# yyyyyxie/textflux

Hardware: AMD Instinct MI355X
Metric: images/sec (whole node), 1024x1024 30-step FLUX-Fill (higher is better)
Workload: dtype bf16

## Files before the change

### textflux_amd/csrc/attention.hip

```cpp
#include <atomic>
#include <type_traits>

#include "common.h"
#include "launch.h"

namespace tfx {

constexpr int KVBLK = 64, HD = 128;
#ifdef TFX_BENCH
constexpr int K_BYTES = KVBLK * HD * 2;
constexpr int ATT_LDS = 2 * 2 * K_BYTES;
constexpr int ATT_LDS2 = 2 * ATT_LDS;
constexpr int ATT_LDS_PP = 5 * K_BYTES;
#endif

typedef __attribute__((address_space(3))) s16x4 lds_s16x4;
__device__ unsigned long long* g_dbg_ptr = nullptr;

#define TFX_ATT_BARRIER()                                   \
  do {                                                      \
    __builtin_amdgcn_sched_barrier(0);                      \
    asm volatile("s_waitcnt lgkmcnt(0)" ::: "memory");      \
    __builtin_amdgcn_s_barrier();                           \
    __builtin_amdgcn_sched_barrier(0);                      \
// ... 391 lines not shown
  };
  for (int j = 0; j < nkv; j += 2) {
    tile(j, std::integral_constant<int, 0>{});
    if (j + 1 < nkv) tile(j + 1, std::integral_constant<int, 1>{});
  }

  const float inv = 1.0f / ol[0];
  if (qrow < N) {
    bf16_t* orow = Ob + (int64_t)qrow * ldo + 4 * hi;
#pragma unroll
    for (int db = 0; db < 4; ++db)
#pragma unroll
      for (int qd = 0; qd < 4; ++qd) {
        u32x2 w;
        w[0] = pack_bf2(o[db][qd * 4 + 0] * inv, o[db][qd * 4 + 1] * inv);
        w[1] = pack_bf2(o[db][qd * 4 + 2] * inv, o[db][qd * 4 + 3] * inv);
        *reinterpret_cast<u32x2*>(orow + db * 32 + qd * 8) = w;
      }
  }
}


template <bool TIMING>
__global__ __launch_bounds__(512, 2) void attn_pp_kernel(const bf16_t* Q, const bf16_t* __restrict__ Kp,
                                                         const bf16_t* __restrict__ Vp, bf16_t* O, int64_t ldq,
                                                         int64_t ldk, int64_t ldv, int64_t ldo, int64_t q_bs, int64_t k_bs,
                                                         int64_t v_bs, int64_t o_bs, int H, int N, int nqb,
                                                         float scale_log2e, unsigned long long* dbg) {
  extern __shared__ __attribute__((aligned(16))) char smem[];
  const int tid = threadIdx.x, lane = tid & 63;
  const int wave = __builtin_amdgcn_readfirstlane(tid >> 6);
  const int g = wave >> 2;
  unsigned long long t_pa = 0, t_b1 = 0, t_pb = 0, t_b2 = 0, tmark = 0;
#define ATM() do { if (TIMING) tmark = __builtin_readcyclecounter(); } while (0)
#define ATA(x) do { if (TIMING) { unsigned long long n_ = __builtin_readcyclecounter(); x += n_ - tmark; tmark = n_; } } while (0)
  const int hi = lane >> 5, l31 = lane & 31;
  int bid = blockIdx.x;
  {
    const int nwg = gridDim.x, q = nwg >> 3, r = nwg & 7, xcd = bid & 7, k = bid >> 3;
    bid = (xcd < r ? xcd * (q + 1) : r * (q + 1) + (xcd - r) * q) + k;
  }
  const int qb = bid % nqb;
  bid /= nqb;
  const int h = bid % H;
  const int b = bid / H;
  const bf16_t* Qb = Q + b * q_bs + h * HD;
  const bf16_t* Kb = Kp + b * k_bs + h * HD;
  const bf16_t* Vb = Vp + b * v_bs + h * HD;
  bf16_t* Ob = O + b * o_bs + h * HD;

  const int qrow = qb * 256 + wave * 32 + l31;
  const int qrow_c = qrow < N ? qrow : N - 1;
  bf16x8 qf[8];
#pragma unroll
  for (int s = 0; s < 8; ++s) qf[s] = *reinterpret_cast<const bf16x8*>(Qb + (int64_t)qrow_c * ldq + s * 16 + hi * 8);

  const int nkv = (N + KVBLK - 1) / KVBLK;
  char* kbuf = smem;
  char* vbuf = smem + 2 * K_BYTES;
  u32x4 kreg[2], vreg[2];
  auto opaque_tid = [&]() { int t_ = tid; asm volatile("" : "+v"(t_)); return t_; };
  auto load_rows = [&](const bf16_t* base, int64_t ld, int t, u32x4* reg) {
    const int te = opaque_tid();
#pragma unroll
    for (int i = 0; i < 2; ++i) {
      const int c = te + i * 512;
      int key = t * KVBLK + (c >> 4);
      if (key > N - 1) key = N - 1;
      reg[i] = *reinterpret_cast<const u32x4*>(base + (int64_t)key * ld + (c & 15) * 8);
    }
  };
  auto write_k = [&](int t) {
    char* kd = kbuf + (t & 1) * K_BYTES;
    const int te = opaque_tid();
#pragma unroll
    for (int i = 0; i < 2; ++i) {
      const int c = te + i * 512, key = c >> 4, ch = c & 15;
      *reinterpret_cast<u32x4*>(kd + key * 256 + ((ch ^ (key & 15)) << 4)) = kreg[i];
    }
  };
  auto write_v = [&](int t) {
    char* vd = vbuf + (t % 3) * K_BYTES;
    const int te = opaque_tid();
#pragma unroll
    for (int i = 0; i < 2; ++i) {
      const int c = te + i * 512, key = c >> 4, ch = c & 15;
      *reinterpret_cast<u32x4*>(vd + key * 256 + ((((ch >> 2) ^ (key & 3)) << 6) | ((ch & 3) << 4))) = vreg[i];
    }
  };

  uint32_t koff[8];
#pragma unroll
  for (int s = 0; s < 8; ++s) koff[s] = l31 * 256 + (((2 * s + hi) ^ (lane & 15)) << 4);
  const int vi = lane & 15;
  const uint32_t vrow = (4 * hi + (vi >> 2)) * 256 + 32 * ((lane >> 4) & 1) + (vi & 3) * 8;
  uint32_t voff[4];
#pragma unroll
  for (int db = 0; db < 4; ++db) voff[db] = vrow + ((db ^ ((vi >> 2) & 3)) << 6);

  f32x16 o[4], s0, s1;
#pragma unroll
  for (int db = 0; db < 4; ++db)
#pragma unroll
    for (int r = 0; r < 16; ++r) o[db][r] = 0.f;
  float m_run = -INFINITY, l_run = 0.f;
  bf16x8 pf[4];
  typedef __attribute__((ext_vector_type(8))) short s16x8;

  auto ldvf = [&](const char* vt, int i) -> bf16x8 {
    const char* va = vt + voff[i & 3] + (i >> 2) * 16 * 256;
    const s16x4 lo = __builtin_amdgcn_ds_read_tr16_b64_v4i16((lds_s16x4*)(va));
    const s16x4 hi4 = __builtin_amdgcn_ds_read_tr16_b64_v4i16((lds_s16x4*)(va + 8 * 256));
    return __builtin_bit_cast(bf16x8, (s16x8)__builtin_shufflevector(lo, hi4, 0, 1, 2, 3, 4, 5, 6, 7));
  };

  load_rows(Kb, ldk, 0, kreg);
  load_rows(Vb, ldv, 0, vreg);
  write_k(0);
  write_v(0);
  if (nkv > 1) {
    load_rows(Kb, ldk, 1, kreg);
    load_rows(Vb, ldv, 1, vreg);
    write_k(1);
    write_v(1);
    if (nkv > 2) {
      load_rows(Kb, ldk, 2, kreg);
      load_rows(Vb, ldv, 2, vreg);
    }
  }
  __syncthreads();
  {
#pragma unroll
    for (int r = 0; r < 16; ++r) { s0[r] = 0.f; s1[r] = 0.f; }
#pragma unroll
    for (int s = 0; s < 8; ++s) {
      const bf16x8 k0 = *reinterpret_cast<const bf16x8*>(kbuf + koff[s]);
      const bf16x8 k1 = *reinterpret_cast<const bf16x8*>(kbuf + koff[s] + 32 * 256);
      s0 = __builtin_amdgcn_mfma_f32_32x32x16_bf16(k0, qf[s], s0, 0, 0, 0);
      s1 = __builtin_amdgcn_mfma_f32_32x32x16_bf16(k1, qf[s], s1, 0, 0, 0);
    }
  }
  TFX_ATT_BARRIER();
  if (g == 1) TFX_ATT_BARRIER();

  int vslot = 0;
  for (int u = 0; u < nkv; ++u) {
    ATM();
    bf16x8 vf[16];
    {
      const char* vt = vbuf + vslot * K_BYTES;
#pragma unroll
      for (int i = 0; i < 16; ++i) vf[i] = ldvf(vt, i);
    }
    if (u == nkv - 1 && (N & (KVBLK - 1))) {
      const int kbase = u * KVBLK + 4 * hi;
#pragma unroll
      for (int r = 0; r < 16; ++r) {
        const int key = kbase + (r & 3) + 8 * (r >> 2);
        if (key >= N) s0[r] = -INFINITY;
        if (key + 32 >= N) s1[r] = -INFINITY;
      }
    }
    {
      float mx = s0[0];
#pragma unroll
      for (int r = 1; r < 16; ++r) mx = fmaxf(mx, s0[r]);
#pragma unroll
      for (int r = 0; r < 16; ++r) mx = fmaxf(mx, s1[r]);
      mx = fmaxf(mx, __shfl_xor(mx, 32, 64));
      const float m_new = fmaxf(m_run, mx);
      const float mc = m_new * scale_log2e;
      const float alpha = __builtin_amdgcn_exp2f(m_run * scale_log2e - mc);
      m_run = m_new;
      float psum = 0.f;
#pragma unroll
      for (int r = 0; r < 16; ++r) {
        s0[r] = __builtin_amdgcn_exp2f(s0[r] * scale_log2e - mc);
        s1[r] = __builtin_amdgcn_exp2f(s1[r] * scale_log2e - mc);
        psum += s0[r] + s1[r];
      }
      l_run = l_run * alpha + psum;
#pragma unroll
      for (int e = 0; e < 8; ++e) {
        pf[0][e] = (__bf16)s0[e];
        pf[1][e] = (__bf16)s0[8 + e];
        pf[2][e] = (__bf16)s1[e];
        pf[3][e] = (__bf16)s1[8 + e];
      }
      if (!__all(alpha == 1.0f)) {
#pragma unroll
        for (int db = 0; db < 4; ++db)
#pragma unroll
          for (int r = 0; r < 16; ++r) o[db][r] *= alpha;
      }
    }
    ATA(t_pa);
    TFX_ATT_BARRIER();
    ATA(t_b1);
    const char* kt = kbuf + ((u + 1) & 1) * K_BYTES;
    bf16x8 kf[8][2];
    uint32_t kofs[8];
    {
      int le = lane;
      asm volatile("" : "+v"(le));
#pragma unroll
      for (int s = 0; s < 8; ++s) kofs[s] = (le & 31) * 256 + (((2 * s + (le >> 5)) ^ (le & 15)) << 4);
    }
    __builtin_amdgcn_s_setprio(1);
#pragma unroll
    for (int ks = 0; ks < 4; ++ks) {
#pragma unroll
      for (int db = 0; db < 4; ++db) o[db] = __builtin_amdgcn_mfma_f32_32x32x16_bf16(vf[ks * 4 + db], pf[ks], o[db], 0, 0, 0);
      __builtin_amdgcn_sched_barrier(0);
#pragma unroll
      for (int s = 2 * ks; s < 2 * ks + 2; ++s) {
        kf[s][0] = *reinterpret_cast<const bf16x8*>(kt + kofs[s]);
        kf[s][1] = *reinterpret_cast<const bf16x8*>(kt + kofs[s] + 32 * 256);
      }
      __builtin_amdgcn_sched_barrier(0);
    }
#pragma unroll
    for (int db = 0; db < 4; ++db) asm volatile("" : "+v"(o[db]));
#pragma unroll
    for (int r = 0; r < 16; ++r) { s0[r] = 0.f; s1[r] = 0.f; }
#pragma unroll
    for (int s = 0; s < 8; ++s) {
      s0 = __builtin_amdgcn_mfma_f32_32x32x16_bf16(kf[s][0], qf[s], s0, 0, 0, 0);
      s1 = __builtin_amdgcn_mfma_f32_32x32x16_bf16(kf[s][1], qf[s], s1, 0, 0, 0);
    }
    asm volatile("" : "+v"(s0), "+v"(s1));
    __builtin_amdgcn_sched_barrier(0);
    __builtin_amdgcn_s_setprio(0);
    if (u + 2 < nkv) {
      write_k(u + 2);
      write_v(u + 2);
      if (u + 3 < nkv) {
        load_rows(Kb, ldk, u + 3, kreg);
        load_rows(Vb, ldv, u + 3, vreg);
      }
    }
    vslot = vslot == 2 ? 0 : vslot + 1;
    ATA(t_pb);
    TFX_ATT_BARRIER();
    ATA(t_b2);
  }
  if (g == 0) TFX_ATT_BARRIER();
  if (TIMING && lane == 0 && dbg) {
    unsigned long long* d = dbg + ((size_t)blockIdx.x * 8 + wave) * 4;
    d[0] = t_pa; d[1] = t_b1; d[2] = t_pb; d[3] = t_b2;
  }
#undef ATM
#undef ATA

  const float l_tot = l_run + __shfl_xor(l_run, 32, 64);
  const float inv = 1.0f / l_tot;
  if (qrow < N) {
    bf16_t* orow = Ob + (int64_t)qrow * ldo + 4 * hi;
#pragma unroll
    for (int db = 0; db < 4; ++db)
#pragma unroll
      for (int qd = 0; qd < 4; ++qd) {
        u32x2 w;
        w[0] = pack_bf2(o[db][qd * 4 + 0] * inv, o[db][qd * 4 + 1] * inv);
        w[1] = pack_bf2(o[db][qd * 4 + 2] * inv, o[db][qd * 4 + 3] * inv);
        *reinterpret_cast<u32x2*>(orow + db * 32 + qd * 8) = w;
      }
  }
}

#endif

static int g_attn_bound = 1;
void set_attention_use_bound(int v) { g_attn_bound = v; }
static std::atomic<int64_t> g_attn_mode_count[9];
void attention_note_streamk() { ++g_attn_mode_count[8]; }
int attention_mode_counts(int64_t* counts, int n, int reset) {
  n = n < 0 ? 0 : n > 9 ? 9 : n;
  for (int i = 0; i < n; ++i) counts[i] = g_attn_mode_count[i].load(std::memory_order_relaxed);
  if (reset) for (int i = 0; i < 9; ++i) g_attn_mode_count[i].store(0, std::memory_order_relaxed);
  return n;
}
static bool attn_bound_admissible(float score_bound, int N) {
  return score_bound > 0.f && score_bound * 1.4426950408889634f + log2f((float)N) + 24.0f <= 126.0f;
}
static int g_attn_waves = 30;
static unsigned long long* g_attn_dbg = nullptr;
void set_attention_debug(void* p) {
  g_attn_dbg = (unsigned long long*)p;
  (void)hipMemcpyToSymbol(HIP_SYMBOL(g_dbg_ptr), &p, sizeof(p));
}
static int g_attn_abl = 0;
void set_attention_ablation(int a) { g_attn_abl = a; }
void set_attention_waves(int nw) {
  if (nw == 0) { g_attn_waves = 30; return; }
  g_attn_waves = (nw == 4 || nw == 8 || nw == 9 || nw == 10 || nw == 12 || nw == 20 || (nw >= 30 && nw <= 34) || nw == 40) ? nw : 16;
}

int joint_attention(const AttnArgs& a, hipStream_t st) {
  if (a.B <= 0 || a.H <= 0 || a.N <= 0) return 0;
  if ((a.ldq | a.ldk | a.ldv | a.q_bstride | a.k_bstride | a.v_bstride) % 8 || (a.ldo | a.o_bstride) % 4)
    return fail("attention: strides must be multiples of 8 elements (q,k,v) / 4 (o)");
  if (((uintptr_t)a.q | (uintptr_t)a.k | (uintptr_t)a.v) % 16 || (uintptr_t)a.o % 8)
    return fail("attention: q/k/v must be 16-byte aligned, o 8-byte aligned");
#ifdef TFX_BENCH
  if (g_attn_waves == 20 && !g_attn_abl) {
    const bool prof = prof_on(st);
    if (prof) prof_begin(1, 4.0 * a.B * a.H * (double)a.N * a.N * HD, st);
    const int rc = joint_attention_hp(a, st);
    if (prof) prof_end(1, st);
    ++g_attn_mode_count[5];
    return rc ? rc : check_launch("joint_attention");
  }
#endif
  const uint64_t w4_rows = (uint64_t)((a.N + 63) / 64 + 3) * 64;
  const bool w4_ok = (a.ldo | a.o_bstride) % 8 == 0 && w4_rows * (uint64_t)a.ldk * 2 + 256 < (1ull << 32) &&
                     w4_rows * (uint64_t)a.ldv * 2 + 256 < (1ull << 32);
#ifdef TFX_BENCH
  if (g_attn_waves == 40 && w4_ok) {
    const bool prof = prof_on(st);
    if (prof) prof_begin(1, 4.0 * a.B * a.H * (double)a.N * a.N * HD, st);
    const int rc = joint_attention_w16(a, st);
    if (prof) prof_end(1, st);
    ++g_attn_mode_count[6];
    return rc ? rc : check_launch("joint_attention");
  }
#endif
#ifdef TFX_BENCH
  if (((g_attn_waves >= 30 && g_attn_waves <= 34) || g_attn_waves == 40) && w4_ok) {
#else
  if ((g_attn_waves == 30 || g_attn_waves == 34) && w4_ok) {
#endif
    const bool prof = prof_on(st);
    if (prof) prof_begin(1, 4.0 * a.B * a.H * (double)a.N * a.N * HD, st);
    const bool bounded = attn_bound_admissible(a.score_bound, a.N);
#ifdef TFX_BENCH
    const int mode = g_attn_waves == 34 ? (bounded ? 4 : 3) : g_attn_waves == 30 ? (bounded && g_attn_bound ? 4 : 0)
                   : g_attn_waves >= 31 && g_attn_waves <= 33 ? g_attn_waves - 30 : 0;
#else
    const int mode = bounded && (g_attn_bound || g_attn_waves == 34) ? 4 : 0;
#endif
    const int rc = joint_attention_w4(a, st, mode);
    if (prof) prof_end(1, st);
    ++g_attn_mode_count[mode];
    return rc ? rc : check_launch("joint_attention");
  }
#ifndef TFX_BENCH
  if (g_attn_waves != 30 && g_attn_waves != 34)
    return fail("attention: kernel variant %d is a bench-only schedule (libtextflux_hip_bench.so, `make bench`)", g_attn_waves);
  return fail("attention: output rows must be 16-byte aligned (ldo and o_bstride multiples of 8 elements) and one head's K / V rows "
              "addressable in 32 bits; got ldo %lld, o_bstride %lld, N %d, ldk %lld, ldv %lld", (long long)a.ldo, (long long)a.o_bstride,
              a.N, (long long)a.ldk, (long long)a.ldv);
#else
  const int NW = (g_attn_waves == 16 || g_attn_waves == 9 || g_attn_waves == 10 || g_attn_waves >= 30) ? 8 : g_attn_waves == 12 ? 4 : g_attn_waves;
  const int qblk = NW * 32;
  static bool attr_set = false;
  if (!attr_set) {
    const void* fns[] = {(const void*)attn_kernel<8>, (const void*)attn_mx_kernel<8>,
#ifdef TFX_BENCH
                         (const void*)attn_kernel<4>, (const void*)attn_mx_kernel<4>,
#endif
    };
    for (const void* fn : fns) {
      hipFuncAttributes fa;
      (void)hipFuncGetAttributes(&fa, fn);
      (void)hipGetLastError();
      if (hipFuncSetAttribute(fn, hipFuncAttributeMaxDynamicSharedMemorySize, ATT_LDS) != hipSuccess)
        return fail("attention: cannot raise dynamic LDS limit");
    }
#ifdef TFX_BENCH
    hipFuncAttributes fa;
    (void)hipFuncGetAttributes(&fa, (const void*)attn_kernel<8, 0, 2>);
    (void)hipFuncGetAttributes(&fa, (const void*)attn_pp_kernel<false>);
    (void)hipGetLastError();
    if (hipFuncSetAttribute((const void*)attn_kernel<8, 0, 2>, hipFuncAttributeMaxDynamicSharedMemorySize, ATT_LDS2) != hipSuccess ||
        hipFuncSetAttribute((const void*)attn_pp_kernel<false>, hipFuncAttributeMaxDynamicSharedMemorySize, ATT_LDS_PP) != hipSuccess)
      return fail("attention: cannot raise dynamic LDS limit (bench variants)");
#endif
    attr_set = true;
  }
  const int nqb = (a.N + qblk - 1) / qblk;
  const unsigned grid = (unsigned)(a.B * a.H * nqb);
  const bool prof = prof_on(st);
  if (prof) prof_begin(1, 4.0 * a.B * a.H * (double)a.N * a.N * HD, st);
  const float sl2 = a.scale * 1.4426950408889634f;
#define ATT_ARGS (const bf16_t*)a.q, (const bf16_t*)a.k, (const bf16_t*)a.v, (bf16_t*)a.o, a.ldq, a.ldk, a.ldv, a.ldo, a.q_bstride, \
                 a.k_bstride, a.v_bstride, a.o_bstride, a.H, a.N, nqb, sl2
#ifdef TFX_BENCH
  if (g_attn_abl) {
    (void)hipFuncSetAttribute((const void*)attn_kernel<8, 1>, hipFuncAttributeMaxDynamicSharedMemorySize, ATT_LDS);
    (void)hipFuncSetAttribute((const void*)attn_kernel<8, 2>, hipFuncAttributeMaxDynamicSharedMemorySize, ATT_LDS);
    (void)hipFuncSetAttribute((const void*)attn_kernel<8, 4>, hipFuncAttributeMaxDynamicSharedMemorySize, ATT_LDS);
    (void)hipFuncSetAttribute((const void*)attn_kernel<8, 8>, hipFuncAttributeMaxDynamicSharedMemorySize, ATT_LDS);
    (void)hipFuncSetAttribute((const void*)attn_kernel<8, 15>, hipFuncAttributeMaxDynamicSharedMemorySize, ATT_LDS);
    (void)hipFuncSetAttribute((const void*)attn_kernel<8, 16>, hipFuncAttributeMaxDynamicSharedMemorySize, ATT_LDS);
    switch (g_attn_abl) {
      case 1: attn_kernel<8, 1><<<grid, 512, ATT_LDS, st>>>(ATT_ARGS); break;
      case 2: attn_kernel<8, 2><<<grid, 512, ATT_LDS, st>>>(ATT_ARGS); break;
      case 4: attn_kernel<8, 4><<<grid, 512, ATT_LDS, st>>>(ATT_ARGS); break;
      case 8: attn_kernel<8, 8><<<grid, 512, ATT_LDS, st>>>(ATT_ARGS); break;
      case 16: attn_kernel<8, 16><<<grid, 512, ATT_LDS, st>>>(ATT_ARGS); break;
      default: attn_kernel<8, 15><<<grid, 512, ATT_LDS, st>>>(ATT_ARGS); break;
    }
  } else if (g_attn_waves == 16) {
    if (g_attn_dbg) {
      (void)hipFuncSetAttribute((const void*)attn_pp_kernel<true>, hipFuncAttributeMaxDynamicSharedMemorySize, ATT_LDS_PP);
      attn_pp_kernel<true><<<grid, 512, ATT_LDS_PP, st>>>(ATT_ARGS, g_attn_dbg);
    } else {
      attn_pp_kernel<false><<<grid, 512, ATT_LDS_PP, st>>>(ATT_ARGS, nullptr);
    }
  } else if (g_attn_waves == 12) {
    attn_mx_kernel<4><<<grid, 256, ATT_LDS, st>>>(ATT_ARGS);
  } else if (g_attn_waves == 9) {
    attn_kernel<8, 0, 2><<<grid, 512, ATT_LDS2, st>>>(ATT_ARGS);
  } else if (g_attn_waves == 4) {
    attn_kernel<4><<<grid, 256, ATT_LDS, st>>>(ATT_ARGS);
  } else
#endif
  if (g_attn_waves == 10 || (g_attn_waves >= 30 && g_attn_waves <= 34))
    attn_mx_kernel<8><<<grid, 512, ATT_LDS, st>>>(ATT_ARGS);
  else
    attn_kernel<8><<<grid, 512, ATT_LDS, st>>>(ATT_ARGS);
#undef ATT_ARGS
  if (prof) prof_end(1, st);
  ++g_attn_mode_count[7];
  return check_launch("joint_attention");
#endif
}

}
```

### textflux_amd/csrc/attention_w4.hip

```cpp
#include <mutex>
#include <type_traits>

#include "common.h"
#include "launch.h"

namespace tfx {

namespace {
constexpr int W4_KV = 64, W4_HD = 128;
constexpr int W4_VT = W4_KV * 256;
constexpr int W4_KROW = 272;
constexpr int W4_KT = W4_KV * W4_KROW;
constexpr int W4_NBUF = 3;
constexpr int W4_KBASE = W4_NBUF * W4_VT;
constexpr int W4_PROW = 132;
__device__ __forceinline__ int w4_part_off(int r, int col) {
  return ((((r >> 5) * 4 + (col >> 5)) * 4 + ((col >> 3) & 3)) * 64 + ((col >> 2) & 1) * 32 + (r & 31)) * 4;
}
constexpr int W4_PART_LM = 256 * 128;
constexpr float W4_THR = 4.0f;
constexpr float W4_BIG = 64.0f;
typedef __attribute__((address_space(3))) s16x4 lds_s16x4;
typedef __attribute__((ext_vector_type(8))) short s16x8;
typedef __attribute__((ext_vector_type(2))) __bf16 bf2_t;
template <int V>
using IC = std::integral_constant<int, V>;
}

constexpr int ATT_LDS_W4 = W4_NBUF * (W4_VT + W4_KT);

#define W4_GAP() __builtin_amdgcn_sched_barrier(0)
#ifndef W4_ABL
#define W4_ABL 0
#endif
#define W4_DRAIN_MFMA()                                                                                                 \
  asm volatile("s_nop 15\n\ts_nop 15\n\ts_nop 15\n\ts_nop 15\n\ts_nop 15\n\ts_nop 15\n\ts_nop 15\n\ts_nop 15\n\t"      \
               "s_nop 15\n\ts_nop 15\n\ts_nop 15\n\ts_nop 15\n\ts_nop 15\n\ts_nop 15\n\ts_nop 15\n\ts_nop 15\n\t"      \
               "s_nop 15\n\ts_nop 15\n\ts_nop 15\n\ts_nop 15\n\ts_nop 15\n\ts_nop 15\n\ts_nop 15\n\ts_nop 15" ::: "memory")

#ifndef W4_NO_TOUCH
#define W4_TOUCH(acc)                                                                  \
  do {                                                                                 \
    const int t_ = __builtin_amdgcn_readfirstlane(__float_as_int((acc)[0]));           \
    asm volatile("" ::"s"(t_));                                                        \
  } while (0)
#else
#define W4_TOUCH(acc) do { } while (0)
#endif

__device__ __forceinline__ void w4_mfma_s0(f32x16& d, const bf16x8& k, const bf16x8& q) {
  f32x16 z;
#pragma unroll
  for (int r = 0; r < 16; ++r) z[r] = 0.f;
  d = __builtin_amdgcn_mfma_f32_32x32x16_bf16(k, q, z, 0, 0, 0);
}
__device__ __forceinline__ void w4_mfma_s(f32x16& d, const bf16x8& k, const bf16x8& q) {
  d = __builtin_amdgcn_mfma_f32_32x32x16_bf16(k, q, d, 0, 0, 0);
}
__device__ __forceinline__ void w4_mfma_o(f32x16& d, const bf16x8& v, const u32x4& p) {
  d = __builtin_amdgcn_mfma_f32_32x32x16_bf16(v, __builtin_bit_cast(bf16x8, p), d, 0, 0, 0);
}
__device__ __forceinline__ void w4_mfma_l(f32x16& d, const bf16x8& ones, const u32x4& p) {
  d = __builtin_amdgcn_mfma_f32_32x32x16_bf16(ones, __builtin_bit_cast(bf16x8, p), d, 0, 0, 0);
}
__device__ __forceinline__ float w4_max7(float a, float b, float c, float d, float e, float f, float g) {
  float r;
  asm("v_max3_f32 %0, %1, %2, %3\n\tv_max3_f32 %0, %0, %4, %5\n\tv_max3_f32 %0, %0, %6, %7"
      : "=&v"(r) : "v"(a), "v"(b), "v"(c), "v"(d), "v"(e), "v"(f), "v"(g));
  return r;
}
__device__ __forceinline__ float w4_max4(float a, float b, float c, float d) {
  float r;
  asm("v_max3_f32 %0, %1, %2, %3\n\tv_max_f32 %0, %0, %4" : "=&v"(r) : "v"(a), "v"(b), "v"(c), "v"(d));
  return r;
}
__device__ __forceinline__ float w4_max(float a, float b) {
  float r;
  asm("v_max_f32 %0, %1, %2" : "=v"(r) : "v"(a), "v"(b));
  return r;
}
__device__ __forceinline__ void w4_dot2c(float& l, uint32_t p) {
  asm volatile("v_dot2c_f32_bf16 %0, 0x3f803f80, %1" : "+v"(l) : "v"(p));
}
__device__ __forceinline__ uint32_t w4_cvt_pk(float lo, float hi) {
  uint32_t r;
  asm volatile("v_cvt_pk_bf16_f32 %0, %1, %2" : "=v"(r) : "v"(lo), "v"(hi));
  return r;
}
#ifdef TFX_BENCH
__device__ unsigned long long* g_w4_timers = nullptr;
#define W4_STAMP(i) do { if (wave == 0) w4_stamp[i] = __builtin_amdgcn_s_memtime(); } while (0)
#else
#define W4_STAMP(i) ((void)0)
#endif
constexpr int W4_SK_MIN = 4;
__host__ __device__ __forceinline__ int w4_sk_bound(int c, int group, int share, int nkv, int total) {
  if (c >= group) return total;
  int p = c * share;
  if (p >= total) return total;
  const int r = p % nkv;
  if (r < W4_SK_MIN) p -= r;
  else if (r > nkv - W4_SK_MIN) p += nkv - r;
  return p < total ? p : total;
}

template <int MODE>
__global__ __launch_bounds__(256, 1) void attn_w4_kernel(const bf16_t* Q, const bf16_t* __restrict__ Kp,
                                                         const bf16_t* __restrict__ Vp, bf16_t* O, int64_t ldq, int64_t ldk,
                                                         int64_t ldv, int64_t ldo, int64_t q_bs, int64_t k_bs, int64_t v_bs,
                                                         int64_t o_bs, int H, int N, int nqb, float scale_log2e, int nfull,
                                                         int nparts, int nsplit, int xsplit, float* part, int T_items, int sk_group,
                                                         int sk_share) {
  extern __shared__ __attribute__((aligned(16))) char smem[];
  constexpr bool LV = MODE == 1 || MODE == 2, LZ = MODE >= 2, NOREF = MODE == 4, FT = LV || NOREF;
  const int tid = threadIdx.x, lane = tid & 63;
  const int wave = __builtin_amdgcn_readfirstlane(tid >> 6);
  const int hi = lane >> 5, l31 = lane & 31;
  int bid = blockIdx.x;
  int kpart = -1, ptile = 0, qblk, h, b;
  int item = 0, item_step = 0, item_end = 0;
  int sk_lo = 0, sk_hi = 0, sk_base = 0, sk_slot0 = 0, sk_u = 0, sk_nunits = 0, sk_nwhole = 0, sk_full = 0, sk_cu = 0, sk_tfirst = 0;
  const int nkv_all = (N + W4_KV - 1) / W4_KV;
  auto sk_unit = [&](int u, int& it, int& ts, int& te) __attribute__((always_inline)) {
    if (u < sk_nwhole) {
      it = sk_base + sk_cu + u * sk_group; ts = 0; te = nkv_all;
    } else {
      const int ti = sk_tfirst + (u - sk_nwhole);
      it = sk_base + sk_full + ti; ts = max(sk_lo - ti * nkv_all, 0); te = min(sk_hi - ti * nkv_all, nkv_all);
    }
  };
  int ts = 0, te = nkv_all;
  if (sk_share > 0) {
    const int L = (bid & 7) * (gridDim.x >> 3) + (bid >> 3);
    const int sample = L / sk_group;
    sk_cu = L - sample * sk_group;
    if (sample >= nfull) return;
    sk_full = (T_items / sk_group) * sk_group;
    sk_nwhole = sk_full / sk_group;
    const int total = (T_items - sk_full) * nkv_all;
    sk_lo = w4_sk_bound(sk_cu, sk_group, sk_share, nkv_all, total);
    sk_hi = w4_sk_bound(sk_cu + 1, sk_group, sk_share, nkv_all, total);
    sk_tfirst = sk_lo / nkv_all;
    sk_nunits = sk_nwhole + (sk_hi > sk_lo ? (sk_hi - 1) / nkv_all - sk_tfirst + 1 : 0);
    if (sk_nunits == 0) return;
    sk_base = sample * T_items;
    sk_slot0 = 2 * L;
    sk_unit(0, item, ts, te);
    qblk = item % nqb;
    h = (item / nqb) % H;
    b = item / (nqb * H);
  } else if (T_items > 0) {
    const int nwg = gridDim.x, q = T_items >> 3, r = T_items & 7, xcd = bid & 7, slot = bid >> 3;
    const int xs = xcd < r ? xcd * (q + 1) : r * (q + 1) + (xcd - r) * q, xc = q + (xcd < r ? 1 : 0);
    if (slot >= xc) return;
    item = xs + slot;
    item_step = nwg >> 3;
    item_end = xs + xc;
    qblk = item % nqb;
    h = (item / nqb) % H;
    b = item / (nqb * H);
  } else if (nsplit > 1) {
    const int fpad = (nfull + 7) & ~7, pf = H * nqb - xsplit;
    int pair;
    if (bid < fpad) {
      const int q = nfull >> 3, r = nfull & 7, xcd = bid & 7, k = bid >> 3;
      if (k >= q + (xcd < r ? 1 : 0)) return;
      const int fid = (xcd < r ? xcd * (q + 1) : r * (q + 1) + (xcd - r) * q) + k;
      b = fid / pf;
      pair = fid % pf;
    } else {
      const int pi = bid - fpad;
      if (pi >= nparts) return;
      kpart = pi % nsplit;
      ptile = pi / nsplit;
      b = ptile / xsplit;
      pair = pf + ptile % xsplit;
    }
    h = pair / nqb;
    qblk = pair % nqb;
  } else {
    const int nwg = gridDim.x, q = nwg >> 3, r = nwg & 7, xcd = bid & 7, k = bid >> 3;
    bid = (xcd < r ? xcd * (q + 1) : r * (q + 1) + (xcd - r) * q) + k;
    qblk = bid % nqb;
    bid /= nqb;
    h = bid % H;
    b = bid / H;
  }
  bf16x8 qn[2][8];
  bool have_pref = false;
  u32x4 kreg[4], vreg[4];
#ifdef TFX_BENCH
  unsigned long long w4_stamp[4] = {0, 0, 0, 0}, w4_sum[4] = {0, 0, 0, 0};
#endif
  for (;;) {
  W4_STAMP(0);
  bool has_next = item + item_step < item_end;
  int item2 = item + item_step, ts2 = 0;
  if (sk_share > 0) {
    int te2;
    has_next = sk_u + 1 < sk_nunits;
    if (has_next) sk_unit(sk_u + 1, item2, ts2, te2);
  }
  const int qblk2 = item2 % nqb, h2 = (item2 / nqb) % H, b2 = item2 / (nqb * H);
  const bf16_t* Qb = Q + b * q_bs + h * W4_HD;
  const bf16_t* Kb = Kp + b * k_bs + h * W4_HD;
  const bf16_t* Vb = Vp + b * v_bs + h * W4_HD;
  bf16_t* Ob = O + b * o_bs + h * W4_HD;
  int Nk = N;
  if (kpart >= 0) {
    const int nkv_all = (N + W4_KV - 1) / W4_KV;
    const int t0 = kpart * nkv_all / nsplit, t1 = (kpart + 1) * nkv_all / nsplit;
    Nk = min(N, t1 * W4_KV) - t0 * W4_KV;
    Kb += (int64_t)t0 * W4_KV * ldk;
    Vb += (int64_t)t0 * W4_KV * ldv;
  }
  int pslot = -1;
  if (sk_share > 0) {
    if (ts > 0) pslot = sk_slot0;
    else if (te < nkv_all) pslot = sk_slot0 + 1;
    Nk = min(N, te * W4_KV) - ts * W4_KV;
    Kb += (int64_t)ts * W4_KV * ldk;
    Vb += (int64_t)ts * W4_KV * ldv;
  }

  int qrow[2];
  bf16x8 qf[2][8];
#pragma unroll
  for (int qb = 0; qb < 2; ++qb) {
    qrow[qb] = qblk * 256 + wave * 64 + qb * 32 + l31;
    const int rc = qrow[qb] < N ? qrow[qb] : N - 1;
    if (have_pref) {
#pragma unroll
      for (int s = 0; s < 8; ++s) qf[qb][s] = qn[qb][s];
    } else {
#pragma unroll
      for (int s = 0; s < 8; ++s) qf[qb][s] = *reinterpret_cast<const bf16x8*>(Qb + (int64_t)rc * ldq + s * 16 + hi * 8);
    }
  }
  auto load_qn = [&]() __attribute__((always_inline)) {
    const bf16_t* Qb2 = Q + b2 * q_bs + h2 * W4_HD;
#pragma unroll
    for (int qb = 0; qb < 2; ++qb) {
      const int r2 = qblk2 * 256 + wave * 64 + qb * 32 + l31;
      const int rc = r2 < N ? r2 : N - 1;
#pragma unroll
      for (int s = 0; s < 8; ++s) qn[qb][s] = *reinterpret_cast<const bf16x8*>(Qb2 + (int64_t)rc * ldq + s * 16 + hi * 8);
    }
  };
  __builtin_amdgcn_sched_barrier(0);
  auto convert_q = [&]() __attribute__((always_inline)) {
    if constexpr (W4_ABL & 1024) {
      float cc = scale_log2e, sn = scale_log2e * 0.5f;
      uint32_t wlo = 0x3f80u, whi = 0x3f800000u;
      asm volatile("" : "+v"(cc), "+v"(sn), "+v"(wlo), "+v"(whi));
#pragma unroll
      for (int qb = 0; qb < 2; ++qb) {
        float ss = 0.f;
#pragma unroll
        for (int s = 0; s < 8; ++s) {
          const u32x4 pk = __builtin_bit_cast(u32x4, qf[qb][s]);
#pragma unroll
          for (int i = 0; i < 4; ++i) {
            const uint32_t pi = pk[i];
            ss = __builtin_amdgcn_fdot2_f32_bf16(__builtin_bit_cast(bf2_t, pi), __builtin_bit_cast(bf2_t, pi), ss, false);
          }
        }
        const auto sw = __builtin_amdgcn_permlane32_swap(__float_as_uint(ss), __float_as_uint(ss), false, false);
        const float rinv = rsqrtf((__uint_as_float(sw[0]) + __uint_as_float(sw[1])) * (1.0f / 128.0f) + 1e-6f);
#pragma unroll
        for (int s = 0; s < 8; ++s) {
          u32x4 pk = __builtin_bit_cast(u32x4, qf[qb][s]);
#pragma unroll
          for (int i = 0; i < 4; ++i) {
            const uint32_t a = pack_bf2(__uint_as_float(pk[i] << 16) * rinv, __uint_as_float(pk[i] & 0xffff0000u) * rinv);
            float y0, y1;
            y0 = __builtin_amdgcn_fdot2_f32_bf16(__builtin_bit_cast(bf2_t, a), __builtin_bit_cast(bf2_t, wlo), 0.0f, false);
            y1 = __builtin_amdgcn_fdot2_f32_bf16(__builtin_bit_cast(bf2_t, a), __builtin_bit_cast(bf2_t, whi), 0.0f, false);
            const uint32_t yp = pack_bf2(y0, y1);
            y0 = __uint_as_float(yp << 16);
            y1 = __uint_as_float(yp & 0xffff0000u);
            pk[i] = pack_bf2(y0 * cc + (-y1) * sn, y1 * cc + y0 * sn);
          }
          qf[qb][s] = __builtin_bit_cast(bf16x8, pk);
        }
      }
    }
#pragma unroll
    for (int qb = 0; qb < 2; ++qb)
#pragma unroll
      for (int s = 0; s < 8; ++s) {
#pragma unroll
        for (int e = 0; e < 8; ++e) qf[qb][s][e] = (__bf16)((float)qf[qb][s][e] * scale_log2e);
        asm volatile("" : "+a"(qf[qb][s]));
      }
  };

  const int nkv = (Nk + W4_KV - 1) / W4_KV;
  const int ldk2 = (int)ldk * 2, ldv2 = (int)ldv * 2;
  const auto rsK = __builtin_amdgcn_make_buffer_rsrc((void*)Kb, 0, (int)((uint32_t)(Nk - 1) * (uint32_t)ldk2 + 256u), 0x00020000);
  const auto rsV = __builtin_amdgcn_make_buffer_rsrc((void*)Vb, 0, (int)((uint32_t)(Nk - 1) * (uint32_t)ldv2 + 256u), 0x00020000);
  const auto rsK2 = __builtin_amdgcn_make_buffer_rsrc((void*)(Kp + b2 * k_bs + h2 * W4_HD + (int64_t)ts2 * W4_KV * ldk), 0,
                                                      (int)((uint32_t)(N - 1 - ts2 * W4_KV) * (uint32_t)ldk2 + 256u), 0x00020000);
  const auto rsV2 = __builtin_amdgcn_make_buffer_rsrc((void*)(Vp + b2 * v_bs + h2 * W4_HD + (int64_t)ts2 * W4_KV * ldv), 0,
                                                      (int)((uint32_t)(N - 1 - ts2 * W4_KV) * (uint32_t)ldv2 + 256u), 0x00020000);
  auto rsKs = rsK, rsVs = rsV;
  auto load_piece = [&](int j, int ko, int vo, auto Ic, bool k_side) __attribute__((always_inline)) {
    constexpr int i = decltype(Ic)::value;
    if (W4_ABL & 32) j = 0;
    if constexpr (W4_ABL & 256) {
      typedef __attribute__((address_space(3))) void lds_void_;
      __builtin_amdgcn_raw_ptr_buffer_load_lds(k_side ? rsKs : rsVs, (lds_void_*)(smem + ATT_LDS_W4 + (tid >> 6) * 1024), 16, k_side ? ko : vo,
                                               (j * W4_KV + 16 * i) * (k_side ? ldk2 : ldv2), 0, 0);
      return;
    }
    if (k_side)
      kreg[i] = __builtin_bit_cast(u32x4, __builtin_amdgcn_raw_buffer_load_b128(rsKs, ko, (j * W4_KV + 16 * i) * ldk2, 0));
    else
      vreg[i] = __builtin_bit_cast(u32x4, __builtin_amdgcn_raw_buffer_load_b128(rsVs, vo, (j * W4_KV + 16 * i) * ldv2, 0));
  };
  auto stage_offsets = [&](int& ko, int& vo) __attribute__((always_inline)) {
    int te = tid;
    asm volatile("" : "+v"(te));
    ko = (int)__umul24(te >> 4, ldk2) + (te & 15) * 16;
    vo = (int)__umul24(te >> 4, ldv2) + (te & 15) * 16;
  };
  auto load_tile = [&](int j) __attribute__((always_inline)) {
    int ko, vo;
    stage_offsets(ko, vo);
    load_piece(j, ko, vo, IC<0>{}, true); load_piece(j, ko, vo, IC<0>{}, false); load_piece(j, ko, vo, IC<1>{}, true); load_piece(j, ko, vo, IC<1>{}, false);
    load_piece(j, ko, vo, IC<2>{}, true); load_piece(j, ko, vo, IC<2>{}, false); load_piece(j, ko, vo, IC<3>{}, true); load_piece(j, ko, vo, IC<3>{}, false);
  };
  auto write_piece = [&](int buf, auto Ic, bool k_side) __attribute__((always_inline)) {
    constexpr int i = decltype(Ic)::value;
    const int kr = tid >> 4, ch = tid & 15;
    if (k_side)
      *reinterpret_cast<u32x4*>(smem + W4_KBASE + buf * W4_KT + kr * W4_KROW + ch * 16 + i * 16 * W4_KROW) = kreg[i];
    else
      *reinterpret_cast<u32x4*>(smem + buf * W4_VT + kr * 256 + ((((ch >> 2) ^ (kr & 3)) << 6) | ((ch & 3) << 4)) + i * 16 * 256) = vreg[i];
  };
  auto write_tile = [&](int buf) __attribute__((always_inline)) {
    write_piece(buf, IC<0>{}, true); write_piece(buf, IC<0>{}, false); write_piece(buf, IC<1>{}, true); write_piece(buf, IC<1>{}, false);
    write_piece(buf, IC<2>{}, true); write_piece(buf, IC<2>{}, false); write_piece(buf, IC<3>{}, true); write_piece(buf, IC<3>{}, false);
  };
  const char* rK = smem + W4_KBASE + l31 * W4_KROW + hi * 16;
  const int vi = lane & 15;
  const char* rV[4];
#pragma unroll
  for (int db = 0; db < 4; ++db)
    rV[db] = smem + (4 * hi + (vi >> 2)) * 256 + 32 * ((lane >> 4) & 1) + (vi & 3) * 8 + ((db ^ ((vi >> 2) & 3)) << 6);
  auto kread = [&](int koff, int s) __attribute__((always_inline)) -> bf16x8 {
    return *reinterpret_cast<const bf16x8*>(rK + koff + s * 32);
  };
  auto vread = [&](int voff, int ks, int db) __attribute__((always_inline)) -> bf16x8 {
    const char* va = rV[db] + voff + ks * 16 * 256;
    if constexpr (W4_ABL & 512) return *reinterpret_cast<const bf16x8*>(rK + voff + ks * 16 * 256 + db * 64);
    const s16x4 lo = __builtin_amdgcn_ds_read_tr16_b64_v4i16((lds_s16x4*)(va));
    const s16x4 hi4 = __builtin_amdgcn_ds_read_tr16_b64_v4i16((lds_s16x4*)(va + 8 * 256));
    return __builtin_bit_cast(bf16x8, (s16x8)__builtin_shufflevector(lo, hi4, 0, 1, 2, 3, 4, 5, 6, 7));
  };

  f32x16 o[2][4], ol[2], sc[2];
#pragma unroll
  for (int qb = 0; qb < 2; ++qb)
#pragma unroll
    for (int r = 0; r < 16; ++r) {
      ol[qb][r] = 0.f;
#pragma unroll
      for (int db = 0; db < 4; ++db) o[qb][db][r] = 0.f;
    }
  bf16x8 kone, vone, qm[2], kf[8], vf[2][4];
  u32x4 pf[2][2];
#pragma unroll
  for (int e = 0; e < 8; ++e) {
    kone[e] = (__bf16)0.f;
    vone[e] = (__bf16)1.0f;
    qm[0][e] = qm[1][e] = (__bf16)0.f;
  }
  if (hi == 0) kone[0] = (__bf16)1.0f;
  asm volatile("" : "+a"(kone), "+a"(vone));
  float m_ref[2] = {0.f, 0.f};
  float lsum[2] = {0.f, 0.f};
  bool any_ref = false;

#ifdef W4_DEBUG_CLEAR_LDS
  for (int i = tid * 16; i < ATT_LDS_W4; i += 256 * 16) *reinterpret_cast<u32x4*>(smem + i) = u32x4{0, 0, 0, 0};
  __syncthreads();
#endif
  if (!have_pref) load_tile(0);
  u32x4 k1[4], v1[4];
  {
    int ko, vo;
    stage_offsets(ko, vo);
#pragma unroll
    for (int i = 0; i < 4; ++i) {
      k1[i] = __builtin_bit_cast(u32x4, __builtin_amdgcn_raw_buffer_load_b128(rsK, ko, (W4_KV + 16 * i) * ldk2, 0));
      v1[i] = __builtin_bit_cast(u32x4, __builtin_amdgcn_raw_buffer_load_b128(rsV, vo, (W4_KV + 16 * i) * ldv2, 0));
    }
  }
  __builtin_amdgcn_sched_barrier(0);
  convert_q();
  __builtin_amdgcn_sched_barrier(0);
  write_tile(0);
  load_tile(2);
  {
    const int kr = tid >> 4, ch = tid & 15;
#pragma unroll
    for (int i = 0; i < 4; ++i) {
      *reinterpret_cast<u32x4*>(smem + W4_KBASE + W4_KT + kr * W4_KROW + ch * 16 + i * 16 * W4_KROW) = k1[i];
      *reinterpret_cast<u32x4*>(smem + W4_VT + kr * 256 + ((((ch >> 2) ^ (kr & 3)) << 6) | ((ch & 3) << 4)) + i * 16 * 256) = v1[i];
    }
  }
  __syncthreads();
#pragma unroll
  for (int s = 0; s < 8; ++s) kf[s] = kread(0, s);
  W4_GAP();
  if constexpr (LZ) {
    w4_mfma_s0(sc[0], kf[0], qf[0][0]);
#pragma unroll
    for (int s = 1; s < 8; ++s) w4_mfma_s(sc[0], kf[s], qf[0][s]);
  } else {
    w4_mfma_s0(sc[0], kone, qm[0]);
#pragma unroll
    for (int s = 0; s < 8; ++s) w4_mfma_s(sc[0], kf[s], qf[0][s]);
  }
#ifdef W4_KEEP_DRAINS
  W4_DRAIN_MFMA();
#endif
  W4_GAP();

  auto step = [&](auto QBc, auto PVc, auto FIRSTc, auto KNc, auto VNc, auto STGc, int jst, bool rag, int kb_abs) __attribute__((always_inline)) {
    constexpr int QB = decltype(QBc)::value, OQ = 1 - QB;
    constexpr bool EVEN = QB == 0, PV = decltype(PVc)::value != 0, FIRST = decltype(FIRSTc)::value != 0;
    constexpr int KN = decltype(KNc)::value, VN = decltype(VNc)::value, STG = decltype(STGc)::value;
    f32x16& cur = sc[QB];
    f32x16& nxt = sc[OQ];
    if (__builtin_expect_with_probability(rag, 0, 1.0)) {
      int kbase = kb_abs + 4 * hi;
      asm volatile("" : "+v"(kbase));
#pragma unroll
      for (int r = 0; r < 16; ++r)
        if (kbase + (r & 3) + 8 * (r >> 2) >= Nk) cur[r] = -INFINITY;
    }
    auto S = [&](auto Ic) __attribute__((always_inline)) {
      constexpr int i = decltype(Ic)::value;
      if constexpr (i == 0) {
        w4_mfma_s0(nxt, kone, qm[OQ]);
      } else if constexpr (i == 1 && LZ) {
        w4_mfma_s0(nxt, kf[0], qf[OQ][0]);
        if constexpr (!NOREF) {
          if (__builtin_expect_with_probability(any_ref, 0, 1.0)) w4_mfma_s(nxt, kone, qm[OQ]);
        }
      } else {
        w4_mfma_s(nxt, kf[i - 1], qf[OQ][i - 1]);
        if constexpr (EVEN && i >= 2 && !(W4_ABL & 2)) kf[i - 2] = kread(KN, i - 2);
      }
    };
    auto PL = [&](auto Ic) __attribute__((always_inline)) {
      constexpr int i = decltype(Ic)::value, ks = i / 4, db = i % 4;
      if constexpr (PV) w4_mfma_o(o[OQ][db], vf[ks][db], pf[OQ][ks]);
      if constexpr (EVEN && i >= 1 && !(W4_ABL & 2)) vf[(i - 1) / 4][(i - 1) % 4] = vread(VN, (i - 1) / 4, (i - 1) % 4);
    };
    auto RL = [&]() __attribute__((always_inline)) {
      if constexpr (EVEN && !(W4_ABL & 2)) {
        vf[1][3] = vread(VN, 1, 3);
        kf[7] = kread(KN, 7);
      }
    };
    auto DL = [&](auto Ic) __attribute__((always_inline)) {
      constexpr int c = decltype(Ic)::value;
      if constexpr (PV && !(W4_ABL & 1)) w4_dot2c(lsum[OQ], pf[OQ][c >> 2][c & 3]);
    };
    auto P = [&](auto Ic) __attribute__((always_inline)) {
      constexpr int i = decltype(Ic)::value, ks = i / 5, db = i % 5;
      if constexpr (PV) {
        if constexpr (db == 4) {
          w4_mfma_l(ol[OQ], vone, pf[OQ][ks]);
        } else {
          w4_mfma_o(o[OQ][db], vf[ks][db], pf[OQ][ks]);
        }
      }
      if constexpr (EVEN && i >= 1 && (i - 1) % 5 < 4 && !(W4_ABL & 2)) vf[(i - 1) / 5][(i - 1) % 5] = vread(VN, (i - 1) / 5, (i - 1) % 5);
      if constexpr (EVEN && i == 9 && !(W4_ABL & 2)) kf[7] = kread(KN, 7);
    };
    auto F = [&](auto Ic) __attribute__((always_inline)) {
      constexpr int k = decltype(Ic)::value;
      if constexpr (W4_ABL & 1) return;
      constexpr bool is_c = FT ? (k >= 22 || (k >= 3 && k <= 18 && k % 3 == 0)) : ((k == 23) || (k >= 3 && k < 22 && k % 3 == 0));
      if constexpr (is_c) {
        constexpr int c = FT ? (k >= 22 ? k - 16 : k / 3 - 1) : (k == 23 ? 7 : k / 3 - 1);
        pf[QB][c >> 2][c & 3] = w4_cvt_pk(cur[2 * c], cur[2 * c + 1]);
      } else {
        constexpr int e = FT ? (k < 3 ? k : k >= 19 ? k - 6 : k - (k / 3))
                             : (k < 3 ? k : k == 22 ? 15 : k - (k / 3));
        cur[e] = __builtin_amdgcn_exp2f(cur[e]);
      }
    };
    int stg_ko = 0, stg_vo = 0;
    if constexpr ((STG & 3) == 1 && !(W4_ABL & 4)) stage_offsets(stg_ko, stg_vo);
    auto G = [&](auto Ic) __attribute__((always_inline)) {
      constexpr int n = decltype(Ic)::value;
      if constexpr ((STG & 3) == 1 && !(W4_ABL & 4)) {
        constexpr bool is_w = n == 0 || n == 1 || (n < 15 && (n & 1));
        constexpr int g = n < 2 ? n : is_w ? (n + 1) / 2 : n == 15 ? 7 : n / 2 - 1;
        if constexpr (is_w) { if constexpr (!(W4_ABL & 64)) write_piece(STG >> 2, IC<g / 2>{}, (g & 1) == 0); }
        else { if constexpr (!(W4_ABL & 128)) load_piece(jst, stg_ko, stg_vo, IC<g / 2>{}, (g & 1) == 0); }
      }
    };
    float mx = 0.f;
    auto MX = [&](auto Ic) __attribute__((always_inline)) {
      constexpr int i = decltype(Ic)::value;
      if constexpr (W4_ABL & 8) return;
      if constexpr (i == 0) mx = w4_max7(cur[0], cur[1], cur[2], cur[3], cur[4], cur[5], cur[6]);
      if constexpr (i == 1) mx = w4_max7(mx, cur[7], cur[8], cur[9], cur[10], cur[11], cur[12]);
      if constexpr (i == 2) mx = w4_max4(mx, cur[13], cur[14], cur[15]);
      if constexpr (i == 3) {
        const auto sw = __builtin_amdgcn_permlane32_swap(__float_as_uint(mx), __float_as_uint(mx), false, false);
        mx = w4_max(__uint_as_float(sw[0]), __uint_as_float(sw[1]));
      }
    };
    auto MOVE = [&]() __attribute__((always_inline)) {
      bool take;
      if constexpr (LZ) take = !(W4_ABL & 8) && !__all(FIRST ? fabsf(mx) <= W4_BIG : mx <= W4_BIG);
      else take = FIRST || (!(W4_ABL & 8) && !__all(mx <= W4_THR));
      if (__builtin_expect_with_probability(take, FIRST && !LZ, 1.0)) {
        float m_new;
        if constexpr (LZ) {
          const bool mv = FIRST ? fabsf(mx) > W4_BIG : mx > W4_BIG;
          m_new = mv ? round_bf(m_ref[QB] + mx) : m_ref[QB];
        } else {
          m_new = round_bf(m_ref[QB] + (FIRST ? mx : fmaxf(mx, 0.f)));
        }
        const float d = m_new - m_ref[QB];
        m_ref[QB] = m_new;
        qm[QB][0] = (__bf16)(hi == 0 ? -m_new : 0.f);
        if constexpr (LZ) any_ref = __any(m_ref[0] != 0.f || m_ref[1] != 0.f);
#pragma unroll
        for (int r = 0; r < 16; ++r) cur[r] -= d;
        if constexpr (!FIRST) {
          const float f = __builtin_amdgcn_exp2f(-d);
          if constexpr (LV) lsum[QB] *= f;
#pragma unroll
          for (int r = 0; r < 16; ++r) {
            if constexpr (!LV) ol[QB][r] *= f;
#pragma unroll
            for (int db = 0; db < 4; ++db) o[QB][db][r] *= f;
          }
        }
      }
    };
    if constexpr (MODE == 0) {
    S(IC<0>{});
    W4_TOUCH(cur);
    MX(IC<0>{});
    W4_GAP();
    S(IC<1>{});
    MX(IC<1>{});
    W4_GAP();
    P(IC<0>{});
    MX(IC<2>{});
    W4_GAP();
    S(IC<2>{});
    MX(IC<3>{});
    W4_GAP();
    P(IC<1>{});
    W4_GAP();
    MOVE();
    W4_GAP();
    S(IC<3>{}); F(IC<0>{}); F(IC<1>{}); G(IC<0>{});
    W4_GAP();
    P(IC<2>{}); F(IC<2>{}); F(IC<3>{}); G(IC<1>{});
    W4_GAP();
    S(IC<4>{}); F(IC<4>{}); F(IC<5>{}); G(IC<2>{});
    W4_GAP();
    P(IC<3>{}); F(IC<6>{}); F(IC<7>{}); G(IC<3>{});
    W4_GAP();
    S(IC<5>{}); F(IC<8>{}); F(IC<9>{}); G(IC<4>{});
    W4_GAP();
    P(IC<4>{}); F(IC<10>{}); F(IC<11>{}); G(IC<5>{});
    W4_GAP();
    S(IC<6>{}); F(IC<12>{}); F(IC<13>{}); G(IC<6>{});
    W4_GAP();
    P(IC<5>{}); F(IC<14>{}); F(IC<15>{}); G(IC<7>{});
    W4_GAP();
    S(IC<7>{}); F(IC<16>{}); F(IC<17>{}); G(IC<8>{});
    W4_GAP();
    P(IC<6>{}); F(IC<18>{}); F(IC<19>{}); G(IC<9>{});
    W4_GAP();
    S(IC<8>{}); F(IC<20>{}); F(IC<21>{}); G(IC<10>{});
#ifdef W4_HAZARD_SELFTEST
    { const float t_ = w4_max(nxt[0], nxt[1]); asm volatile("" ::"v"(t_)); }
#endif
    W4_GAP();
    P(IC<7>{}); F(IC<22>{}); G(IC<11>{});
    W4_GAP();
    P(IC<8>{}); G(IC<12>{}); G(IC<13>{});
    W4_GAP();
    P(IC<9>{}); G(IC<14>{}); G(IC<15>{});
    W4_GAP();
    F(IC<23>{});
    W4_GAP();
    } else if constexpr (MODE == 1) {
    S(IC<0>{}); W4_TOUCH(cur); MX(IC<0>{}); G(IC<0>{});
    W4_GAP();
    S(IC<1>{}); MX(IC<1>{}); DL(IC<0>{}); G(IC<1>{});
    W4_GAP();
    PL(IC<0>{}); MX(IC<2>{}); DL(IC<1>{}); DL(IC<2>{}); G(IC<2>{});
    W4_GAP();
    S(IC<2>{}); MX(IC<3>{}); DL(IC<3>{}); DL(IC<4>{}); G(IC<3>{});
    W4_GAP();
    PL(IC<1>{}); DL(IC<5>{}); DL(IC<6>{}); DL(IC<7>{}); G(IC<4>{});
    W4_GAP();
    MOVE();
    W4_GAP();
    S(IC<3>{}); F(IC<0>{}); F(IC<1>{}); G(IC<5>{});
    W4_GAP();
    PL(IC<2>{}); F(IC<2>{}); F(IC<3>{}); G(IC<6>{});
    W4_GAP();
    S(IC<4>{}); F(IC<4>{}); F(IC<5>{}); G(IC<7>{});
    W4_GAP();
    PL(IC<3>{}); F(IC<6>{}); F(IC<7>{}); G(IC<8>{});
    W4_GAP();
    S(IC<5>{}); F(IC<8>{}); F(IC<9>{}); G(IC<9>{});
    W4_GAP();
    PL(IC<4>{}); F(IC<10>{}); F(IC<11>{}); G(IC<10>{});
    W4_GAP();
    S(IC<6>{}); F(IC<12>{}); F(IC<13>{}); G(IC<11>{});
    W4_GAP();
    PL(IC<5>{}); F(IC<14>{}); F(IC<15>{}); G(IC<12>{});
    W4_GAP();
    S(IC<7>{}); F(IC<16>{}); F(IC<17>{}); G(IC<13>{});
    W4_GAP();
    PL(IC<6>{}); F(IC<18>{}); F(IC<19>{}); G(IC<14>{});
    W4_GAP();
    S(IC<8>{}); F(IC<20>{}); F(IC<21>{}); G(IC<15>{});
#ifdef W4_HAZARD_SELFTEST
    { const float t_ = w4_max(nxt[0], nxt[1]); asm volatile("" ::"v"(t_)); }
#endif
    W4_GAP();
    PL(IC<7>{}); F(IC<22>{}); RL(); F(IC<23>{});
    W4_GAP();
    } else if constexpr (MODE == 3) {
    S(IC<1>{}); W4_TOUCH(cur); MX(IC<0>{});
    W4_GAP();
    P(IC<0>{}); MX(IC<1>{});
    W4_GAP();
    S(IC<2>{}); MX(IC<2>{});
    W4_GAP();
    P(IC<1>{}); MX(IC<3>{});
    W4_GAP();
    MOVE();
    W4_GAP();
    S(IC<3>{}); F(IC<0>{}); F(IC<1>{}); G(IC<0>{});
    W4_GAP();
    P(IC<2>{}); F(IC<2>{}); F(IC<3>{}); G(IC<1>{});
    W4_GAP();
    S(IC<4>{}); F(IC<4>{}); F(IC<5>{}); G(IC<2>{});
    W4_GAP();
    P(IC<3>{}); F(IC<6>{}); F(IC<7>{}); G(IC<3>{});
    W4_GAP();
    S(IC<5>{}); F(IC<8>{}); F(IC<9>{}); G(IC<4>{});
    W4_GAP();
    P(IC<4>{}); F(IC<10>{}); F(IC<11>{}); G(IC<5>{});
    W4_GAP();
    S(IC<6>{}); F(IC<12>{}); F(IC<13>{}); G(IC<6>{});
    W4_GAP();
    P(IC<5>{}); F(IC<14>{}); F(IC<15>{}); G(IC<7>{});
    W4_GAP();
    S(IC<7>{}); F(IC<16>{}); F(IC<17>{}); G(IC<8>{});
    W4_GAP();
    P(IC<6>{}); F(IC<18>{}); F(IC<19>{}); G(IC<9>{});
    W4_GAP();
    S(IC<8>{}); F(IC<20>{}); F(IC<21>{}); G(IC<10>{});
#ifdef W4_HAZARD_SELFTEST
    { const float t_ = w4_max(nxt[0], nxt[1]); asm volatile("" ::"v"(t_)); }
#endif
    W4_GAP();
    P(IC<7>{}); F(IC<22>{}); G(IC<11>{});
    W4_GAP();
    P(IC<8>{}); G(IC<12>{}); G(IC<13>{});
    W4_GAP();
    P(IC<9>{}); G(IC<14>{}); G(IC<15>{});
    W4_GAP();
    F(IC<23>{});
    W4_GAP();
    } else if constexpr (MODE == 4) {
    auto E = [&](auto Ic) __attribute__((always_inline)) {
      constexpr int e = decltype(Ic)::value;
      if constexpr (!(W4_ABL & 1)) cur[e] = __builtin_amdgcn_exp2f(cur[e]);
    };
    auto C2 = [&](auto Ic) __attribute__((always_inline)) {
      constexpr int c = decltype(Ic)::value;
      if constexpr (!(W4_ABL & 1)) pf[QB][c >> 2][c & 3] = w4_cvt_pk(cur[2 * c], cur[2 * c + 1]);
    };
    S(IC<1>{}); W4_TOUCH(cur); E(IC<0>{}); E(IC<1>{}); G(IC<0>{});
    W4_GAP();
    P(IC<0>{}); E(IC<2>{}); G(IC<1>{});
    W4_GAP();
    S(IC<2>{}); E(IC<3>{}); G(IC<2>{});
    W4_GAP();
    P(IC<1>{}); C2(IC<0>{}); E(IC<4>{}); G(IC<3>{});
    W4_GAP();
    S(IC<3>{}); E(IC<5>{}); G(IC<4>{});
    W4_GAP();
    P(IC<2>{}); C2(IC<1>{}); E(IC<6>{}); G(IC<5>{});
    W4_GAP();
    S(IC<4>{}); E(IC<7>{}); G(IC<6>{});
    W4_GAP();
    P(IC<3>{}); C2(IC<2>{}); E(IC<8>{}); G(IC<7>{});
    W4_GAP();
    S(IC<5>{}); E(IC<9>{}); G(IC<8>{});
    W4_GAP();
    P(IC<4>{}); C2(IC<3>{}); E(IC<10>{}); G(IC<9>{});
    W4_GAP();
    S(IC<6>{}); E(IC<11>{}); G(IC<10>{});
    W4_GAP();
    P(IC<5>{}); C2(IC<4>{}); E(IC<12>{}); G(IC<11>{});
    W4_GAP();
    S(IC<7>{}); E(IC<13>{}); G(IC<12>{});
    W4_GAP();
    P(IC<6>{}); C2(IC<5>{}); E(IC<14>{}); G(IC<13>{});
    W4_GAP();
    S(IC<8>{}); E(IC<15>{}); G(IC<14>{});
#ifdef W4_HAZARD_SELFTEST
    { const float t_ = w4_max(nxt[0], nxt[1]); asm volatile("" ::"v"(t_)); }
#endif
    W4_GAP();
    P(IC<7>{}); C2(IC<6>{}); G(IC<15>{});
    W4_GAP();
    P(IC<8>{});
    W4_GAP();
    P(IC<9>{}); C2(IC<7>{});
    W4_GAP();
    } else {
    S(IC<1>{}); W4_TOUCH(cur); MX(IC<0>{}); G(IC<0>{});
    W4_GAP();
    PL(IC<0>{}); MX(IC<1>{}); DL(IC<0>{}); G(IC<1>{});
    W4_GAP();
    S(IC<2>{}); MX(IC<2>{}); DL(IC<1>{}); DL(IC<2>{}); G(IC<2>{});
    W4_GAP();
    PL(IC<1>{}); MX(IC<3>{}); DL(IC<3>{}); DL(IC<4>{}); G(IC<3>{});
    W4_GAP();
    S(IC<3>{}); DL(IC<5>{}); DL(IC<6>{}); DL(IC<7>{}); G(IC<4>{});
    W4_GAP();
    MOVE();
    W4_GAP();
    PL(IC<2>{}); F(IC<0>{}); F(IC<1>{}); G(IC<5>{});
    W4_GAP();
    S(IC<4>{}); F(IC<2>{}); F(IC<3>{}); G(IC<6>{});
    W4_GAP();
    PL(IC<3>{}); F(IC<4>{}); F(IC<5>{}); G(IC<7>{});
    W4_GAP();
    S(IC<5>{}); F(IC<6>{}); F(IC<7>{}); G(IC<8>{});
    W4_GAP();
    PL(IC<4>{}); F(IC<8>{}); F(IC<9>{}); G(IC<9>{});
    W4_GAP();
    S(IC<6>{}); F(IC<10>{}); F(IC<11>{}); G(IC<10>{});
    W4_GAP();
    PL(IC<5>{}); F(IC<12>{}); F(IC<13>{}); G(IC<11>{});
    W4_GAP();
    S(IC<7>{}); F(IC<14>{}); F(IC<15>{}); G(IC<12>{});
    W4_GAP();
    PL(IC<6>{}); F(IC<16>{}); F(IC<17>{}); G(IC<13>{});
    W4_GAP();
    S(IC<8>{}); F(IC<18>{}); F(IC<19>{}); G(IC<14>{});
#ifdef W4_HAZARD_SELFTEST
    { const float t_ = w4_max(nxt[0], nxt[1]); asm volatile("" ::"v"(t_)); }
#endif
    W4_GAP();
    PL(IC<7>{}); F(IC<20>{}); F(IC<21>{}); G(IC<15>{}); RL();
    W4_GAP();
    F(IC<22>{}); F(IC<23>{});
    W4_GAP();
    }
  };

  const int j_rag = (Nk & (W4_KV - 1)) ? nkv - 1 : -1;
  auto tile = [&](int j, auto Bc, auto FIRSTc) __attribute__((always_inline)) {
    constexpr int B = decltype(Bc)::value, NB = (B + 1) % 3, WB = (B + 2) % 3;
    constexpr int FIRST = decltype(FIRSTc)::value;
    const bool rag = j == j_rag;
    step(IC<0>{}, IC<!FIRST>{}, IC<FIRST>{}, IC<B * W4_KT + 32 * W4_KROW>{}, IC<B * W4_VT>{}, IC<0>{}, 0, rag, j * W4_KV);
    step(IC<1>{}, IC<1>{}, IC<FIRST>{}, IC<0>{}, IC<0>{}, IC<1 + 4 * WB>{}, j + 3, rag, j * W4_KV);
    step(IC<0>{}, IC<1>{}, IC<0>{}, IC<NB * W4_KT>{}, IC<B * W4_VT + 2 * 16 * 256>{}, IC<0>{}, 0, rag, j * W4_KV + 32);
    step(IC<1>{}, IC<1>{}, IC<0>{}, IC<0>{}, IC<0>{}, IC<0>{}, 0, rag, j * W4_KV + 32);
    __builtin_amdgcn_sched_barrier(0);
    asm volatile("s_waitcnt lgkmcnt(0)" ::: "memory");
    if (!(W4_ABL & 16)) __builtin_amdgcn_s_barrier();
    __builtin_amdgcn_sched_barrier(0);
  };
  W4_STAMP(1);
  tile(0, IC<0>{}, IC<1>{});
  for (int j = 1; j < nkv; j += 3) {
    tile(j, IC<1>{}, IC<0>{});
    if (j + 1 < nkv) tile(j + 1, IC<2>{}, IC<0>{});
    if (j + 2 < nkv) tile(j + 2, IC<0>{}, IC<0>{});
  }
  W4_STAMP(2);
  asm volatile("s_waitcnt vmcnt(0)" ::: "memory");
  if (has_next) load_qn();
#pragma unroll
  for (int ks = 0; ks < 2; ++ks) {
#pragma unroll
    for (int db = 0; db < 4; ++db) w4_mfma_o(o[1][db], vf[ks][db], pf[1][ks]);
    if constexpr (!LV) w4_mfma_l(ol[1], vone, pf[1][ks]);
  }
  float ltot[2];
  if constexpr (LV) {
#pragma unroll
    for (int c = 0; c < 8; ++c) w4_dot2c(lsum[1], pf[1][c >> 2][c & 3]);
#pragma unroll
    for (int qb = 0; qb < 2; ++qb) ltot[qb] = lsum[qb] + __shfl_xor(lsum[qb], 32, 64);
  }
#ifdef W4_KEEP_DRAINS
  W4_DRAIN_MFMA();
#endif
  if constexpr (!LV) {
    ltot[0] = ol[0][0];
    ltot[1] = ol[1][0];
  }

  if (kpart >= 0 || pslot >= 0) {
    float* pp = part + (kpart >= 0 ? (int64_t)ptile * nsplit + kpart : (int64_t)pslot) * (256 * W4_PROW);
#pragma unroll
    for (int qb = 0; qb < 2; ++qb) {
      float* pr = pp + (wave * 2 + qb) * (16 * 256) + lane * 4;
#pragma unroll
      for (int db = 0; db < 4; ++db)
#pragma unroll
        for (int qd = 0; qd < 4; ++qd)
          *reinterpret_cast<f32x4*>(pr + (db * 4 + qd) * 256) =
              f32x4{o[qb][db][qd * 4 + 0], o[qb][db][qd * 4 + 1], o[qb][db][qd * 4 + 2], o[qb][db][qd * 4 + 3]};
      if (hi == 0) *reinterpret_cast<float2*>(pp + W4_PART_LM + (wave * 64 + qb * 32 + l31) * 2) = float2{ltot[qb], m_ref[qb]};
    }
    if (kpart >= 0) return;
  } else {
  constexpr int OROW = 272;
  char* ot = smem + wave * (64 * OROW);
#pragma unroll
  for (int qb = 0; qb < 2; ++qb) {
    const float inv = 1.0f / ltot[qb];
    char* orow = ot + (qb * 32 + l31) * OROW + 8 * hi;
#pragma unroll
    for (int db = 0; db < 4; ++db)
#pragma unroll
      for (int qd = 0; qd < 4; ++qd) {
        u32x2 w;
        w[0] = pack_bf2(o[qb][db][qd * 4 + 0] * inv, o[qb][db][qd * 4 + 1] * inv);
        w[1] = pack_bf2(o[qb][db][qd * 4 + 2] * inv, o[qb][db][qd * 4 + 3] * inv);
        *reinterpret_cast<u32x2*>(orow + db * 64 + qd * 16) = w;
      }
  }
  __builtin_amdgcn_fence(__ATOMIC_RELEASE, "wavefront");
  asm volatile("s_waitcnt lgkmcnt(0)" ::: "memory");
  const int row0 = qblk * 256 + wave * 64;
#pragma unroll
  for (int i = 0; i < 16; ++i) {
    const int c = lane + 64 * i, row = c >> 4, ch = c & 15;
    const u32x4 v = *reinterpret_cast<const u32x4*>(ot + row * OROW + ch * 16);
    if (row0 + row < N) *reinterpret_cast<u32x4*>(Ob + (int64_t)(row0 + row) * ldo + ch * 8) = v;
  }
  }
#ifdef TFX_BENCH
  W4_STAMP(3);
  w4_sum[0] += w4_stamp[1] - w4_stamp[0]; w4_sum[1] += w4_stamp[2] - w4_stamp[1]; w4_sum[2] += w4_stamp[3] - w4_stamp[2]; w4_sum[3] += 1;
  if (!has_next && g_w4_timers && tid == 0)
    for (int i = 0; i < 4; ++i) atomicAdd(g_w4_timers + i, w4_sum[i]);
#endif
  if (!has_next) break;
  rsKs = rsK2;
  rsVs = rsV2;
  load_tile(0);
  item = item2; b = b2; h = h2; qblk = qblk2;
  if (sk_share > 0) { ++sk_u; int it_; sk_unit(sk_u, it_, ts, te); }
  have_pref = true;
  __builtin_amdgcn_sched_barrier(0);
  asm volatile("s_waitcnt lgkmcnt(0)" ::: "memory");
  __builtin_amdgcn_s_barrier();
  __builtin_amdgcn_sched_barrier(0);
  }
}

__global__ __launch_bounds__(256) void attn_w4_merge_kernel(const float* part, bf16_t* O, int64_t ldo, int64_t o_bs, int H, int N,
                                                            int nqb, int xsplit, int nsplit) {
  const int rg = blockIdx.x * 8 + (threadIdx.x >> 5), c = (threadIdx.x & 31) * 4;
  const int ptile = rg >> 8, r = rg & 255;
  const int pair = H * nqb - xsplit + ptile % xsplit, b = ptile / xsplit, h = pair / nqb, qblk = pair % nqb;
  const int row = qblk * 256 + r;
  if (row >= N) return;
  const float* pr = part + (int64_t)ptile * nsplit * (256 * W4_PROW);
  const int po = w4_part_off(r, c), lo = W4_PART_LM + r * 2;
  float m = -INFINITY;
  for (int k = 0; k < nsplit; ++k) m = fmaxf(m, pr[(int64_t)k * 256 * W4_PROW + lo + 1]);
  f32x4 acc = {0.f, 0.f, 0.f, 0.f};
  float l = 0.f;
  for (int k = 0; k < nsplit; ++k) {
    const float* pk = pr + (int64_t)k * 256 * W4_PROW;
    const float w = __builtin_amdgcn_exp2f(pk[lo + 1] - m);
    const f32x4 v = *reinterpret_cast<const f32x4*>(pk + po);
    acc += v * w;
    l += pk[lo] * w;
  }
  const float inv = 1.0f / l;
  u32x2 o2;
  o2[0] = pack_bf2(acc[0] * inv, acc[1] * inv);
  o2[1] = pack_bf2(acc[2] * inv, acc[3] * inv);
  *reinterpret_cast<u32x2*>(O + b * o_bs + (int64_t)row * ldo + h * W4_HD + c) = o2;
}

__global__ __launch_bounds__(256) void attn_w4_merge_sk_kernel(const float* part, bf16_t* O, int64_t ldo, int64_t o_bs, int H, int N, int nqb,
                                                               int group, int share, int Tp) {
  __shared__ __attribute__((aligned(16))) unsigned short sm[32][128 + 8];
  const int bi = blockIdx.x >> 3, wq = blockIdx.x & 7;
  const int sample = bi / group, c = bi - sample * group;
  if (c == 0) return;
  const int nkv = (N + W4_KV - 1) / W4_KV, full = (Tp / group) * group, total = (Tp - full) * nkv;
  const int p = w4_sk_bound(c, group, share, nkv, total);
  if (p >= total || p % nkv == 0) return;
  const int il = p / nkv, istart = il * nkv, iend = istart + nkv;
  if (w4_sk_bound(c - 1, group, share, nkv, total) > istart) return;
  const int gi = full + il, h = gi / nqb, qblk = gi - h * nqb;
  if (qblk * 256 + wq * 32 >= N) return;
  int slots[8], np = 0;
  slots[np++] = 2 * (sample * group + c - 1) + 1;
  for (int j = c; j < group && np < 8; ++j) {
    const int lo = w4_sk_bound(j, group, share, nkv, total), hi = w4_sk_bound(j + 1, group, share, nkv, total);
    if (lo >= iend || lo >= total) break;
    if (hi > lo) slots[np++] = 2 * (sample * group + j);
  }
  const int tid = threadIdx.x, lane = tid & 63, w = tid >> 6, l31 = lane & 31, hi = lane >> 5;
  const int lmo = W4_PART_LM + (wq * 32 + l31) * 2, vo = ((wq * 4 + w) * 4 * 64 + lane) * 4;
  float2 lm[8];
  float m = -INFINITY;
#pragma unroll
  for (int k = 0; k < 8; ++k) {
    lm[k] = float2{0.f, -INFINITY};
    if (k < np) lm[k] = *reinterpret_cast<const float2*>(part + (int64_t)slots[k] * (256 * W4_PROW) + lmo);
  }
#pragma unroll
  for (int k = 0; k < 8; ++k) m = fmaxf(m, lm[k].y);
  f32x4 acc[4] = {{0.f, 0.f, 0.f, 0.f}, {0.f, 0.f, 0.f, 0.f}, {0.f, 0.f, 0.f, 0.f}, {0.f, 0.f, 0.f, 0.f}};
  float l = 0.f;
#pragma unroll
  for (int k = 0; k < 8; ++k)
    if (k < np) {
      const float* pk = part + (int64_t)slots[k] * (256 * W4_PROW) + vo;
      f32x4 v[4];
#pragma unroll
      for (int qd = 0; qd < 4; ++qd) v[qd] = *reinterpret_cast<const f32x4*>(pk + qd * 256);
      const float wgt = __builtin_amdgcn_exp2f(lm[k].y - m);
#pragma unroll
      for (int qd = 0; qd < 4; ++qd) acc[qd] += v[qd] * wgt;
      l += lm[k].x * wgt;
    }
  const float inv = 1.0f / l;
#pragma unroll
  for (int qd = 0; qd < 4; ++qd) {
    u32x2 o2;
    o2[0] = pack_bf2(acc[qd][0] * inv, acc[qd][1] * inv);
    o2[1] = pack_bf2(acc[qd][2] * inv, acc[qd][3] * inv);
    *reinterpret_cast<u32x2*>(&sm[l31][w * 32 + qd * 8 + hi * 4]) = o2;
  }
  __syncthreads();
  const int orow = tid >> 3, och = tid & 7, row = qblk * 256 + wq * 32 + orow;
  if (row < N) {
    bf16_t* dst = O + sample * o_bs + (int64_t)row * ldo + h * W4_HD + och * 16;
    *reinterpret_cast<u32x4*>(dst) = *reinterpret_cast<const u32x4*>(&sm[orow][och * 16]);
    *reinterpret_cast<u32x4*>(dst + 8) = *reinterpret_cast<const u32x4*>(&sm[orow][och * 16 + 8]);
  }
}

static constexpr int W4_PART_TILES = 1024;
static constexpr int W4_PART_SLOTS = 8;
struct W4Scratch { int dev; hipStream_t st; float* part; int cus; };
static W4Scratch g_w4_scr[W4_PART_SLOTS];
static int g_w4_nscr = 0;
static std::mutex g_w4_mu;
static int g_w4_split = 0;
void set_attention_tail_split(int v) { g_w4_split = v; }

static const W4Scratch* w4_scratch(hipStream_t st, bool may_alloc) {
  int dev = 0;
  (void)hipGetDevice(&dev);
  std::lock_guard<std::mutex> lk(g_w4_mu);
  for (int i = 0; i < g_w4_nscr; ++i)
    if (g_w4_scr[i].dev == dev && g_w4_scr[i].st == st) return &g_w4_scr[i];
  if (!may_alloc || g_w4_nscr == W4_PART_SLOTS) return nullptr;
  W4Scratch s{dev, st, nullptr, 256};
  if (hipDeviceGetAttribute(&s.cus, hipDeviceAttributeMultiprocessorCount, dev) != hipSuccess || s.cus < 8) s.cus = 256;
  if (hipMalloc((void**)&s.part, (size_t)W4_PART_TILES * 256 * W4_PROW * sizeof(float)) != hipSuccess) {
    (void)hipGetLastError();
    return nullptr;
  }
  g_w4_scr[g_w4_nscr] = s;
  return &g_w4_scr[g_w4_nscr++];
}

int attention_w4_release() {
  std::lock_guard<std::mutex> lk(g_w4_mu);
  if (g_w4_nscr == 0) return 0;
  (void)hipDeviceSynchronize();
  int cur = 0;
  (void)hipGetDevice(&cur);
  for (int i = 0; i < g_w4_nscr; ++i) {
    (void)hipSetDevice(g_w4_scr[i].dev);
    (void)hipDeviceSynchronize();
    (void)hipFree(g_w4_scr[i].part);
  }
  (void)hipSetDevice(cur);
  (void)hipGetLastError();
  g_w4_nscr = 0;
  return 0;
}

int attention_w4_prepare(hipStream_t st) {
  if (!g_w4_split) return 0;
  return w4_scratch(st, true) ? 0 : fail("attention: cannot allocate the tail-split scratch");
}

static int g_w4_streamk = 1;
void set_attention_streamk(int v) { g_w4_streamk = v; }
static int g_w4_persist = 1;
void set_attention_persistent(int v) { g_w4_persist = v; }
static int g_w4_grid() {
  static int grid = 0;
  if (!grid) {
    int dev = 0, cus = 0;
    (void)hipGetDevice(&dev);
    if (hipDeviceGetAttribute(&cus, hipDeviceAttributeMultiprocessorCount, dev) != hipSuccess || cus < 8) cus = 256;
    grid = cus & ~7;
  }
  return grid;
}

#ifdef TFX_BENCH
extern "C" void tfx_bench_attn_timers(unsigned long long* dev) {
  (void)hipMemcpyToSymbol(HIP_SYMBOL(g_w4_timers), &dev, sizeof(dev));
}
#endif

template <int MODE>
static int w4_launch(const AttnArgs& a, hipStream_t st, unsigned grid, int nqb, int nfull, int nparts, int nsplit, int xsplit, float* part,
                     int sk_group, int sk_share) {
  static bool attr_set = false;
  const void* fn = (const void*)attn_w4_kernel<MODE>;
  if (!attr_set) {
    hipFuncAttributes fa;
    if (hipFuncGetAttributes(&fa, fn) != hipSuccess) return fail("attention: no attn_w4_kernel<%d> in this build", MODE);
    (void)hipGetLastError();
    if (fa.localSizeBytes != 0)
      return fail("attention: attn_w4_kernel<%d> spills %zu bytes per lane -- attention_w4.hip must be compiled with "
                  "-mllvm -amdgpu-mfma-vgpr-form", MODE, (size_t)fa.localSizeBytes);
    if (hipFuncSetAttribute(fn, hipFuncAttributeMaxDynamicSharedMemorySize, ATT_LDS_W4 + ((W4_ABL & 256) ? 4096 : 0)) != hipSuccess)
      return fail("attention: cannot raise dynamic LDS limit to %d bytes", ATT_LDS_W4);
    attr_set = true;
  }
  int T_items = 0;
  if (sk_share > 0) {
    T_items = a.H * nqb;
    nfull = a.B;
    grid = (unsigned)g_w4_grid();
  } else if (g_w4_persist && nsplit == 1 && (int)grid > g_w4_grid()) {
    T_items = (int)grid;
    grid = (unsigned)g_w4_grid();
  }
  attn_w4_kernel<MODE><<<grid, 256, ATT_LDS_W4 + ((W4_ABL & 256) ? 4096 : 0), st>>>((const bf16_t*)a.q, (const bf16_t*)a.k, (const bf16_t*)a.v, (bf16_t*)a.o, a.ldq,
                                                       a.ldk, a.ldv, a.ldo, a.q_bstride, a.k_bstride, a.v_bstride, a.o_bstride, a.H,
                                                       a.N, nqb, a.scale * 1.4426950408889634f, nfull, nparts, nsplit, xsplit, part, T_items, sk_group, sk_share);
  return 0;
}

int joint_attention_w4(const AttnArgs& a, hipStream_t st, int mode) {
  const int nqb = (a.N + 255) / 256;
  const int T = a.B * a.H * nqb;
  int nfull = T, nsplit = 1, nparts = 0, xsplit = 0;
  float* part = nullptr;
  if (g_w4_split) {
    hipStreamCaptureStatus cs = hipStreamCaptureStatusNone;
    const bool capturing = !(hipStreamIsCapturing(st, &cs) == hipSuccess && cs == hipStreamCaptureStatusNone);
    (void)hipGetLastError();
    if (const W4Scratch* sc = w4_scratch(st, !capturing)) {
      const int C = sc->cus, tail = T % C, nkv = (a.N + W4_KV - 1) / W4_KV;
      const int m = (tail + a.B - 1) / a.B;
      if (tail && T >= C && m * a.B * 2 <= C + 8 && nkv >= 48 && m < a.H * nqb && m * a.B * 2 <= W4_PART_TILES) {
        xsplit = m; nsplit = 2; nfull = T - m * a.B; nparts = m * a.B * 2; part = sc->part;
      }
    }
  }
  int sk_group = 0, sk_share = 0;
  if (g_w4_streamk && g_w4_persist && nsplit == 1 && a.workspace && a.B <= g_w4_grid()) {
    const int C = g_w4_grid(), nkv = (a.N + W4_KV - 1) / W4_KV, Tp = a.H * nqb, group = C / a.B;
    const int full = (Tp / group) * group, R = Tp - full;
    const int share = R ? (R * nkv + group - 1) / group : 0;
    const int64_t need = (int64_t)2 * a.B * group * 256 * W4_PROW * (int64_t)sizeof(float);
    const float F = 7.f, M = 20.f;
    const float t_whole = (float)(full / group) * ((float)nkv + F);
    const float t_now = t_whole + (float)nkv + F, t_sk = t_whole + (float)share + ((float)share / (float)nkv + 1.f) * F + M;
    if (R > 0 && nkv >= 16 && share * 6 >= nkv && share >= 8 && need <= a.workspace_bytes && ((uintptr_t)a.workspace & 15) == 0 &&
        (g_w4_streamk >= 2 || t_sk < 0.99f * t_now)) {
      sk_group = group; sk_share = share; part = (float*)a.workspace;
    }
  }
  const unsigned grid = nsplit > 1 ? (unsigned)(((nfull + 7) & ~7) + nparts) : (unsigned)T;
#ifdef TFX_BENCH
  const int rc = mode == 4 ? w4_launch<4>(a, st, grid, nqb, nfull, nparts, nsplit, xsplit, part, sk_group, sk_share)
               : mode == 3 ? w4_launch<3>(a, st, grid, nqb, nfull, nparts, nsplit, xsplit, part, sk_group, sk_share)
               : mode == 2 ? w4_launch<2>(a, st, grid, nqb, nfull, nparts, nsplit, xsplit, part, sk_group, sk_share)
               : mode == 1 ? w4_launch<1>(a, st, grid, nqb, nfull, nparts, nsplit, xsplit, part, sk_group, sk_share)
                           : w4_launch<0>(a, st, grid, nqb, nfull, nparts, nsplit, xsplit, part, sk_group, sk_share);
#else
  if (mode != 4 && mode != 0) return fail("attention: attn_w4_kernel<%d> is bench-only (libtextflux_hip_bench.so)", mode);
  const int rc = mode == 4 ? w4_launch<4>(a, st, grid, nqb, nfull, nparts, nsplit, xsplit, part, sk_group, sk_share)
                           : w4_launch<0>(a, st, grid, nqb, nfull, nparts, nsplit, xsplit, part, sk_group, sk_share);
#endif
  if (rc) return rc;
  if (sk_share > 0) attention_note_streamk();
  if (sk_share > 0)
    attn_w4_merge_sk_kernel<<<(unsigned)(a.B * sk_group * 8), 256, 0, st>>>(part, (bf16_t*)a.o, a.ldo, a.o_bstride, a.H, a.N, nqb, sk_group,
                                                                             sk_share, a.H * nqb);
  if (nsplit > 1)
    attn_w4_merge_kernel<<<(unsigned)(xsplit * a.B * 32), 256, 0, st>>>(part, (bf16_t*)a.o, a.ldo, a.o_bstride, a.H, a.N, nqb,
                                                                              xsplit, nsplit);
  return 0;
}

}
```

### textflux_amd/csrc/capi.cpp

```cpp
#include "../../include/textflux_hip.h"

#include <cstring>

#include "launch.h"

using namespace tfx;

namespace {

inline hipStream_t S(tfx_stream s) { return (hipStream_t)s; }
inline const uint16_t* bf(const void* p) { return (const uint16_t*)p; }
inline uint16_t* bf(void* p) { return (uint16_t*)p; }

#define TRY(x)            \
  do {                    \
    if (int _e = (x)) return _e; \
  } while (0)

struct LoraCtx { const tfx_dit_desc* d; };
thread_local const LoraCtx* g_lora = nullptr;

struct Gemm {
  GemmArgs a;
  const tfx_linear* lin;
  const tfx_linear* lin2 = nullptr;
  Gemm(const void* A, int64_t lda, int64_t abs_, const tfx_linear& l, int64_t ldw, void* C, int64_t ldc, int64_t cbs,
       int M, int N, int K, int batch) : lin(&l) {
    a = GemmArgs();
    a.A = A; a.lda = lda; a.a_bstride = abs_;
    a.W = l.w; a.ldw = l.ldw > 0 ? l.ldw : ldw; a.bias = l.b;
    a.C = C; a.ldc = ldc; a.c_bstride = cbs;
    a.M = M; a.N = N; a.K = K; a.batch = batch;
    a.epilogue = EPI_BIAS;
  }
  Gemm& gelu(int from_col) { a.epilogue = EPI_BIAS_GELU; a.gelu_from_col = from_col; return *this; }
  Gemm& gate_res(const void* gate, int64_t gbs, const void* res, int64_t ldr, int64_t rbs) {
    a.epilogue = EPI_BIAS_GATE_RES; a.gate = gate; a.gate_bstride = gbs; a.res = res; a.ldr = ldr; a.r_bstride = rbs;
    return *this;
  }
  Gemm& scratch(void* ws, int64_t bytes) { a.workspace = ws; a.workspace_bytes = bytes; return *this; }
  Gemm& rowsplit(int split_row, const tfx_linear& l2, const void* gate2 = nullptr) {
    a.split_row = split_row; a.W2 = l2.w; a.bias2 = l2.b; a.gate2 = gate2; lin2 = &l2;
    return *this;
  }
  Gemm& qknorm2(const void* wq2, const void* wk2) { a.qkn_wq2 = wq2; a.qkn_wk2 = wk2; return *this; }
  bool rowsplit_ok() const { return gemm_rowsplit_ok(a); }
  Gemm& qknorm(const void* wq, const void* wk, const float* cs, int pos0, int D, float eps) {
    a.qkn_wq = wq; a.qkn_wk = wk; a.qkn_rope_cs = cs; a.qkn_pos0 = pos0;
    a.qkn_k0 = 0; a.qkn_k1 = D; a.qkn_q0 = 2 * D; a.qkn_q1 = 3 * D; a.qkn_eps = eps;
    if (a.epilogue == EPI_BIAS) { a.epilogue = EPI_BIAS_GELU; a.gelu_from_col = 1 << 30; }
    return *this;
  }
  bool qknorm_ok(const void* wq, const void* wk, const float* cs, int pos0, int D, float eps, bool fp8 = false) const {
    Gemm t = *this;
    t.qknorm(wq, wk, cs, pos0, D, eps);
    if (t.a.split_row > 0 && !(t.a.qkn_wq2 && t.a.qkn_wk2)) return false;
    return fp8 ? gemm_fp8_qkn_ok(t.a) : gemm_qkn_ok(t.a);
  }
  bool adapted() const { return lin->lora_a || (a.split_row > 0 && lin2 && lin2->lora_a); }
  int run_lora(hipStream_t st) const {
    if (!g_lora) return fail("dit_forward: adapted Linear outside a forward");
    const tfx_dit_desc& d = *g_lora->d;
    if (!d.lora_t_xn || !d.lora_t_y || !d.lora_scale)
      return fail("dit_forward: a block Linear carries a runtime LoRA adapter but lora_t_xn / lora_t_y / lora_scale are null");
    const tfx_linear* l2 = a.split_row > 0 ? lin2 : nullptr;
    const tfx_linear& ref = lin->lora_a ? *lin : *l2;
    const int R = ref.lora_r, nseg = ref.lora_nseg;
    if (R <= 0 || nseg <= 0 || nseg > 4) return fail("dit_forward: bad lora_r / lora_nseg on an adapted Linear");
    if (l2 && (l2->ldw != lin->ldw || (l2->lora_a && lin->lora_a && (l2->lora_r != R || l2->lora_nseg != nseg))))
      return fail("dit_forward: the [img; txt] Linears of a joint launch must share ldw, lora_r and lora_nseg");
    const int64_t hid_elems = (int64_t)d.B * (d.S + d.T) * d.D;
    const char* A = (const char*)a.A;
    const bool in_xn = A >= (const char*)d.xn && A < (const char*)d.xn + hid_elems * 2;
    const bool in_y = A >= (const char*)d.y && A < (const char*)d.y + hid_elems * 14;
    if (!in_xn && !in_y) return fail("dit_forward: adapted Linear whose input is neither xn nor y");
    char* T = const_cast<char*>(A) + (in_xn ? (const char*)d.lora_t_xn - (const char*)d.xn : (const char*)d.lora_t_y - (const char*)d.y);
    const bool planes = (int64_t)nseg * R > a.lda;
    if (planes && (!in_xn || d.D >= 1024)) return fail("dit_forward: lora_nseg * lora_r exceeds the input's row pitch");
    auto down = [&](const tfx_linear& l, int row0, int rows) -> int {
      if (!l.lora_a || rows <= 0) return 0;
      GemmArgs g = GemmArgs();
      g.A = A + (int64_t)row0 * a.lda * 2; g.lda = a.lda; g.a_bstride = a.a_bstride;
      g.ldw = a.K; g.bias = nullptr;
      g.ldc = a.lda; g.c_bstride = a.a_bstride;
      g.M = rows; g.K = a.K; g.batch = a.batch;
      g.epilogue = EPI_COLSCALE;
      g.workspace = a.workspace; g.workspace_bytes = a.workspace_bytes;
      for (int s = 0; s < (planes ? nseg : 1); ++s) {
        if (planes && !((l.lora_mask >> s) & 1)) continue;
        g.W = (const char*)l.lora_a + (int64_t)s * R * a.K * 2;
        g.C = T + (int64_t)row0 * a.lda * 2 + (int64_t)s * hid_elems * 2;
        g.N = planes ? R : nseg * R;
        g.cscale = d.lora_scale + l.lora_scale_off + s * R;
        if (int e = gemm_bf16(g, st)) return e;
      }
      return 0;
    };
    if (l2) {
      TRY(down(*l2, 0, a.split_row));
      TRY(down(*lin, a.split_row, a.M - a.split_row));
    } else {
      TRY(down(*lin, 0, a.M));
    }
    LoraArgs la{T, (const char*)a.W + (int64_t)a.K * 2, R, nseg > 1 ? d.D : a.N, nseg,
                (uint32_t)lin->lora_mask | (l2 ? (uint32_t)l2->lora_mask << 8 : 0u), planes ? hid_elems : 0};
    return gemm_bf16_lora(a, la, st);
  }
  int run(hipStream_t st) const { return adapted() ? run_lora(st) : gemm_bf16(a, st); }
  bool fp8_ready() const { return lin->w8 && lin->w8_scale && a.K % 256 == 0; }
  int run_pre(hipStream_t st, const void* q, int64_t qld, int64_t qbs, const float* qs, int64_t qs_bs) const {
    if (adapted()) return fail("dit_forward: runtime LoRA adapters and fp8 linears (flags bit 2) cannot be combined");
    GemmArgs f = a;
    f.A = q; f.lda = qld; f.a_bstride = qbs;
    f.W = lin->w8;
    f.a_scale = qs; f.a_scale_bstride = qs_bs; f.w_scale = lin->w8_scale;
    return gemm_fp8(f, st);
  }
  int run(hipStream_t st, void* q8, float* q8_scale) const {
    if (adapted()) return q8 ? fail("dit_forward: runtime LoRA adapters and fp8 linears (flags bit 2) cannot be combined") : run_lora(st);
    if (!q8 || !lin->w8 || !lin->w8_scale || a.K % 256) return gemm_bf16(a, st);
    if (int e = quantize_rows_fp8(a.A, a.lda, a.a_bstride, q8, a.K, (int64_t)a.M * a.K, q8_scale, a.M, a.M, a.batch, a.K, st))
      return e;
    GemmArgs f = a;
    f.A = q8; f.lda = a.K; f.a_bstride = (int64_t)a.M * a.K;
    f.W = lin->w8; f.ldw = a.ldw;
    f.a_scale = q8_scale; f.a_scale_bstride = a.M; f.w_scale = lin->w8_scale;
    return gemm_fp8(f, st);
  }
};

static int g_fp8_fuse_qkn = 1;
static int g_ln_joint = 1;
static int g_group_streams = 1;

int dit_forward(const tfx_dit_desc& d, hipStream_t st) {
  const int D = d.D, H = d.H, B = d.B, Sn = d.S, T = d.T, N = Sn + T;
  if (D != H * 128) return fail("dit_forward: inner dim %d != heads %d * 128", D, H);
  if (B <= 0 || Sn <= 0 || T < 0) return fail("dit_forward: bad B/S/T");
  const int64_t D7 = 7ll * D;
  const int64_t hid_bs = (int64_t)N * D, y_bs = (int64_t)N * D7;
  uint16_t* hid = bf(d.hid);
  uint16_t* xn = bf(d.xn);
  uint16_t* y = bf(d.y);
  uint16_t* hid_img = hid + (int64_t)T * D;
  uint16_t* xn_img = xn + (int64_t)T * D;
  uint16_t* y_img = y + (int64_t)T * D7;
  const uint16_t* mod = bf(d.mod);
  const int64_t mbs = d.mod_bstride;
  const float eps = 1e-6f;
  const float att_scale = 0.08838834764831845f;
  const int nblk = d.n_double + d.n_single;
  const int first = d.first_block < 0 ? 0 : d.first_block;
  const int last = (d.last_block < 0 || d.last_block > nblk) ? nblk : d.last_block;
  void* q8 = (d.flags & 4) ? d.q8 : nullptr;
  float* q8s = (d.flags & 4) ? d.q8_scale : nullptr;
  if ((d.flags & 4) && (!d.q8 || !d.q8_scale)) return fail("dit_forward: fp8 flag set but the q8 workspace is null");
  const LoraCtx lora_ctx{&d};
  struct LoraScope { LoraScope(const LoraCtx* c) { g_lora = c; } ~LoraScope() { g_lora = nullptr; } } lora_scope(&lora_ctx);

  if (!(d.flags & 1)) {
    TRY(Gemm(d.xin, d.in_channels, (int64_t)Sn * d.in_channels, d.x_embedder, d.in_channels, hid_img, D, hid_bs, Sn, D,
             d.in_channels, B).run(st));
    if (T > 0) TRY(copy_rows(d.ctx0, D, (int64_t)T * D, hid, D, hid_bs, T, D, B, st));
  }

  auto norm_rope_rows = [&](int row0, int rows, const void* nq, const void* nk) -> int {
    if (rows <= 0) return 0;
    return rmsnorm_rope(y + (int64_t)row0 * D7, D7, y_bs, 2 * D, 0, H, rows, 0, B, nq, nk, nq, nk, d.cos_tab + (int64_t)row0 * 128,
                        d.sin_tab + (int64_t)row0 * 128, eps, st);
  };
  auto attention = [&](float block_bound) -> int {
    AttnArgs a;
    a.q = y + 2 * D; a.k = y; a.v = y + D; a.o = y + 2 * D;
    a.ldq = a.ldk = a.ldv = a.ldo = D7;
    a.q_bstride = a.k_bstride = a.v_bstride = a.o_bstride = y_bs;
    a.B = B; a.H = H; a.N = N; a.scale = att_scale; a.score_bound = block_bound > 0.f ? block_bound : d.attn_score_bound;
    a.workspace = d.gemm_workspace; a.workspace_bytes = d.gemm_workspace_bytes;
    return joint_attention(a, st);
  };

  const bool may_fuse = d.rope_cs != nullptr;
  auto fused_here = [&](const Gemm& gm, int row0, const void* nq, const void* nk) -> bool {
    if (gm.adapted()) return may_fuse;
    Gemm t = gm;
    t.scratch(d.gemm_workspace, d.gemm_workspace_bytes);
    const bool f8 = q8 && gm.fp8_ready();
    if (f8 && !g_fp8_fuse_qkn) return false;
    return may_fuse && t.qknorm_ok(nq, nk, d.rope_cs, row0, D, eps, f8);
  };
  auto norm_gemm = [&](const uint16_t* src, int row0, int rows, const uint16_t* shift, const uint16_t* scale, Gemm gm) -> int {
    gm.scratch(d.gemm_workspace, d.gemm_workspace_bytes);
    if (q8 && gm.fp8_ready()) {
      uint8_t* q = (uint8_t*)q8 + (int64_t)row0 * D;
      float* qs = q8s + row0;
      TRY(ln_modulate_fp8(src, q, qs, shift, scale, mbs, rows, B, D, D, hid_bs, D, hid_bs, N, eps, st));
      return gm.run_pre(st, q, D, hid_bs, qs, N);
    }
    TRY(ln_modulate(src, xn + (int64_t)row0 * D, shift, scale, mbs, rows, B, D, D, hid_bs, D, hid_bs, eps, st));
    return gm.run(st, q8, q8s);
  };

  for (int blk = first; blk < last; ++blk) {
    if (blk < d.n_double) {
      const tfx_double_block& w = d.dbl[blk];
      const uint16_t* mi = mod + (int64_t)blk * 12 * D;
      const uint16_t* mt = mi + 6 * D;
      Gemm jq(xn, D, hid_bs, w.qkv_img, D, y, D7, y_bs, N, 3 * D, D, B);
      jq.rowsplit(T, w.qkv_txt).qknorm2(w.norm_added_q, w.norm_added_k).scratch(d.gemm_workspace, d.gemm_workspace_bytes);
      Gemm jo(y + 2 * D, D7, y_bs, w.out_img, D, hid, D, hid_bs, N, D, D, B);
      jo.gate_res(mi + 2 * D, mbs, hid, D, hid_bs).rowsplit(T, w.out_txt, mt + 2 * D).scratch(d.gemm_workspace, d.gemm_workspace_bytes);
      Gemm j1(xn, D, hid_bs, w.ff1_img, D, y + 3 * D, D7, y_bs, N, 4 * D, D, B);
      j1.gelu(0).rowsplit(T, w.ff1_txt).scratch(d.gemm_workspace, d.gemm_workspace_bytes);
      Gemm j2(y + 3 * D, D7, y_bs, w.ff2_img, 4 * D, hid, D, hid_bs, N, D, 4 * D, B);
      j2.gate_res(mi + 5 * D, mbs, hid, D, hid_bs).rowsplit(T, w.ff2_txt, mt + 5 * D).scratch(d.gemm_workspace, d.gemm_workspace_bytes);
      const bool joint = g_group_streams && T > 0 && !q8 && jq.rowsplit_ok() && jo.rowsplit_ok() && j1.rowsplit_ok() && j2.rowsplit_ok();
      if (joint) {
        if (g_ln_joint) {
          TRY(ln_modulate_split(hid, xn, mi, mi + D, mt, mt + D, T, mbs, N, B, D, D, hid_bs, D, hid_bs, eps, st));
        } else {
          TRY(ln_modulate(hid_img, xn_img, mi, mi + D, mbs, Sn, B, D, D, hid_bs, D, hid_bs, eps, st));
          TRY(ln_modulate(hid, xn, mt, mt + D, mbs, T, B, D, D, hid_bs, D, hid_bs, eps, st));
        }
        const bool fj = may_fuse && (jq.adapted() || jq.qknorm_ok(w.norm_q, w.norm_k, d.rope_cs, 0, D, eps));
        if (fj) jq.qknorm(w.norm_q, w.norm_k, d.rope_cs, 0, D, eps);
        TRY(jq.run(st));
        if (!fj)
          TRY(rmsnorm_rope(y, D7, y_bs, 2 * D, 0, H, N, T, B, w.norm_q, w.norm_k, w.norm_added_q, w.norm_added_k, d.cos_tab, d.sin_tab, eps, st));
        TRY(attention(w.attn_score_bound));
        TRY(jo.run(st));
        if (g_ln_joint) {
          TRY(ln_modulate_split(hid, xn, mi + 3 * D, mi + 4 * D, mt + 3 * D, mt + 4 * D, T, mbs, N, B, D, D, hid_bs, D, hid_bs, eps, st));
        } else {
          TRY(ln_modulate(hid_img, xn_img, mi + 3 * D, mi + 4 * D, mbs, Sn, B, D, D, hid_bs, D, hid_bs, eps, st));
          TRY(ln_modulate(hid, xn, mt + 3 * D, mt + 4 * D, mbs, T, B, D, D, hid_bs, D, hid_bs, eps, st));
        }
        TRY(j1.run(st));
        TRY(j2.run(st));
        continue;
      }
      {
        Gemm gi(xn_img, D, hid_bs, w.qkv_img, D, y_img, D7, y_bs, Sn, 3 * D, D, B);
        const bool fi = fused_here(gi, T, w.norm_q, w.norm_k);
        if (fi) gi.qknorm(w.norm_q, w.norm_k, d.rope_cs, T, D, eps);
        TRY(norm_gemm(hid_img, T, Sn, mi, mi + D, gi));
        if (!fi) TRY(norm_rope_rows(T, Sn, w.norm_q, w.norm_k));
        if (T > 0) {
          Gemm gt(xn, D, hid_bs, w.qkv_txt, D, y, D7, y_bs, T, 3 * D, D, B);
          const bool ft = fused_here(gt, 0, w.norm_added_q, w.norm_added_k);
          if (ft) gt.qknorm(w.norm_added_q, w.norm_added_k, d.rope_cs, 0, D, eps);
          TRY(norm_gemm(hid, 0, T, mt, mt + D, gt));
          if (!ft) TRY(norm_rope_rows(0, T, w.norm_added_q, w.norm_added_k));
        }
      }
      TRY(attention(w.attn_score_bound));
      TRY(Gemm(y_img + 2 * D, D7, y_bs, w.out_img, D, hid_img, D, hid_bs, Sn, D, D, B)
              .gate_res(mi + 2 * D, mbs, hid_img, D, hid_bs).scratch(d.gemm_workspace, d.gemm_workspace_bytes).run(st, q8, q8s));
      if (T > 0)
        TRY(Gemm(y + 2 * D, D7, y_bs, w.out_txt, D, hid, D, hid_bs, T, D, D, B)
                .gate_res(mt + 2 * D, mbs, hid, D, hid_bs).scratch(d.gemm_workspace, d.gemm_workspace_bytes).run(st, q8, q8s));
      TRY(norm_gemm(hid_img, T, Sn, mi + 3 * D, mi + 4 * D,
                    Gemm(xn_img, D, hid_bs, w.ff1_img, D, y_img + 3 * D, D7, y_bs, Sn, 4 * D, D, B).gelu(0)));
      if (T > 0)
        TRY(norm_gemm(hid, 0, T, mt + 3 * D, mt + 4 * D, Gemm(xn, D, hid_bs, w.ff1_txt, D, y + 3 * D, D7, y_bs, T, 4 * D, D, B).gelu(0)));
      TRY(Gemm(y_img + 3 * D, D7, y_bs, w.ff2_img, 4 * D, hid_img, D, hid_bs, Sn, D, 4 * D, B)
              .gate_res(mi + 5 * D, mbs, hid_img, D, hid_bs).scratch(d.gemm_workspace, d.gemm_workspace_bytes).run(st, q8, q8s));
      if (T > 0)
        TRY(Gemm(y + 3 * D, D7, y_bs, w.ff2_txt, 4 * D, hid, D, hid_bs, T, D, 4 * D, B)
                .gate_res(mt + 5 * D, mbs, hid, D, hid_bs).scratch(d.gemm_workspace, d.gemm_workspace_bytes).run(st, q8, q8s));
    } else {
      const int j = blk - d.n_double;
      const tfx_single_block& w = d.sgl[j];
      const uint16_t* ms = mod + (int64_t)d.n_double * 12 * D + (int64_t)j * 3 * D;
      {
        Gemm gs = Gemm(xn, D, hid_bs, w.qkv_mlp, D, y, D7, y_bs, N, 7 * D, D, B).gelu(3 * D);
        const bool fs = fused_here(gs, 0, w.norm_q, w.norm_k);
        if (fs) gs.qknorm(w.norm_q, w.norm_k, d.rope_cs, 0, D, eps);
        TRY(norm_gemm(hid, 0, N, ms, ms + D, gs));
        if (!fs) TRY(norm_rope_rows(0, N, w.norm_q, w.norm_k));
      }
      TRY(attention(w.attn_score_bound));
      TRY(Gemm(y + 2 * D, D7, y_bs, w.proj_out, 5 * D, hid, D, hid_bs, N, D, 5 * D, B)
              .gate_res(ms + 2 * D, mbs, hid, D, hid_bs).scratch(d.gemm_workspace, d.gemm_workspace_bytes).run(st, q8, q8s));
    }
  }

  if (!(d.flags & 2)) {
    const uint16_t* mo = mod + (int64_t)d.n_double * 12 * D + (int64_t)d.n_single * 3 * D;
    TRY(ln_modulate(hid_img, xn_img, mo + D, mo, mbs, Sn, B, D, D, hid_bs, D, hid_bs, eps, st));
    if (d.euler_gate) {
      void* lat = const_cast<void*>(d.xin);
      const int64_t xbs = (int64_t)Sn * d.in_channels;
      TRY(Gemm(xn_img, D, hid_bs, d.proj_out, D, lat, d.in_channels, xbs, Sn, d.out_channels, D, B)
              .gate_res(d.euler_gate, d.euler_gate_bstride, lat, d.in_channels, xbs).run(st));
    } else {
      TRY(Gemm(xn_img, D, hid_bs, d.proj_out, D, d.out, d.out_channels, (int64_t)Sn * d.out_channels, Sn, d.out_channels,
               D, B).run(st));
    }
  }
  return 0;
}

}

extern "C" {

const char* tfx_version(void) { return "textflux_hip 0.1 (gfx950)"; }
const char* tfx_last_error(void) { return last_error(); }
int tfx_abi_info(int32_t* out, int n) {
  const int32_t v[7] = {TFX_ABI_VERSION, (int32_t)sizeof(tfx_gemm_args), (int32_t)sizeof(tfx_attn_args), (int32_t)sizeof(tfx_dit_desc),
                        (int32_t)sizeof(tfx_step_desc), (int32_t)sizeof(tfx_double_block), (int32_t)sizeof(tfx_single_block)};
  for (int i = 0; i < 7 && i < n; ++i) out[i] = v[i];
  return 7;
}

int tfx_query_arch(char* buf, int buflen) {
  int dev = 0;
  if (hipGetDevice(&dev) != hipSuccess) return fail("tfx_query_arch: no HIP device");
  hipDeviceProp_t prop;
  if (hipGetDeviceProperties(&prop, dev) != hipSuccess) return fail("tfx_query_arch: hipGetDeviceProperties failed");
  if (buf && buflen > 0) {
    std::strncpy(buf, prop.gcnArchName, buflen - 1);
    buf[buflen - 1] = 0;
  }
  return 0;
}

#ifdef TFX_BENCH
static struct { const void* wq; const void* wk; const float* cs; int D; } g_bench_qkn = {nullptr, nullptr, nullptr, 0};
extern "C" void tfx_bench_gemm_qkn(const void* wq, const void* wk, const float* cs, int D) { g_bench_qkn = {wq, wk, cs, D}; }
#endif

int tfx_gemm_bf16(const tfx_gemm_args* g, int variant, tfx_stream stream) {
  if (!g) return fail("tfx_gemm_bf16: null args");
  GemmArgs a;
  a.A = g->A; a.lda = g->lda; a.a_bstride = g->a_bstride;
  a.W = g->W; a.ldw = g->ldw; a.bias = g->bias; a.w_bstride = g->w_bstride;
  a.C = g->C; a.ldc = g->ldc; a.c_bstride = g->c_bstride;
  a.M = g->M; a.N = g->N; a.K = g->K; a.batch = g->batch;
  a.epilogue = g->epilogue; a.gelu_from_col = g->gelu_from_col;
  a.gate = g->gate; a.gate_bstride = g->gate_bstride;
  a.res = g->res; a.ldr = g->ldr; a.r_bstride = g->r_bstride;
  a.workspace = g->workspace; a.workspace_bytes = g->workspace_bytes;
  a.cscale = g->cscale;
  if (!a.A || !a.W || !a.C) return fail("tfx_gemm_bf16: null matrix pointer");
#ifdef TFX_BENCH
  if (g_bench_qkn.cs) {
    const int D = g_bench_qkn.D;
    a.qkn_wq = g_bench_qkn.wq; a.qkn_wk = g_bench_qkn.wk; a.qkn_rope_cs = g_bench_qkn.cs; a.qkn_pos0 = 0;
    a.qkn_k0 = 0; a.qkn_k1 = D; a.qkn_q0 = 2 * D; a.qkn_q1 = 3 * D; a.qkn_eps = 1e-6f;
    if (!gemm_qkn_ok(a)) return fail("tfx_bench_gemm_qkn: shape cannot carry the fused epilogue");
  }
#endif
  return variant < 0 ? gemm_bf16(a, S(stream)) : gemm_bf16_variant(a, variant, S(stream));
}

int tfx_gemm_bf16_qkn(const tfx_gemm_args* g, const tfx_qkn_args* q, tfx_stream stream) {
  if (!g || !q) return fail("tfx_gemm_bf16_qkn: null args");
  if (!g->A || !g->W || !g->C) return fail("tfx_gemm_bf16_qkn: null matrix pointer");
  if (!q->norm_q || !q->norm_k || !q->rope_cs) return fail("tfx_gemm_bf16_qkn: norm weights and the rotary table are required");
  if ((uintptr_t)q->norm_q % 16 || (uintptr_t)q->norm_k % 16 || (uintptr_t)q->rope_cs % 16)
    return fail("tfx_gemm_bf16_qkn: norm weights and the rotary table must be 16-byte aligned");
  if (q->q0 < 0 || q->q1 < q->q0 || q->q1 > g->N || q->k0 < 0 || q->k1 < q->k0 || q->k1 > g->N || q->pos0 < 0)
    return fail("tfx_gemm_bf16_qkn: column ranges outside [0, N)");
  GemmArgs a;
  a.A = g->A; a.lda = g->lda; a.a_bstride = g->a_bstride;
  a.W = g->W; a.ldw = g->ldw; a.bias = g->bias; a.w_bstride = g->w_bstride;
  a.C = g->C; a.ldc = g->ldc; a.c_bstride = g->c_bstride;
  a.M = g->M; a.N = g->N; a.K = g->K; a.batch = g->batch;
  if (g->epilogue != EPI_BIAS && g->epilogue != EPI_BIAS_GELU) return fail("tfx_gemm_bf16_qkn: epilogue must be 0 (bias) or 1 (bias + GELU from a column)");
  a.epilogue = EPI_BIAS_GELU;
  a.gelu_from_col = g->epilogue == EPI_BIAS_GELU ? g->gelu_from_col : (g->N + 255) / 256 * 256;
  a.gate = nullptr; a.gate_bstride = 0; a.res = nullptr; a.ldr = 0; a.r_bstride = 0;
  a.workspace = g->workspace; a.workspace_bytes = g->workspace_bytes;
  a.qkn_wq = q->norm_q; a.qkn_wk = q->norm_k; a.qkn_rope_cs = q->rope_cs; a.qkn_pos0 = q->pos0;
  a.qkn_q0 = q->q0; a.qkn_q1 = q->q1; a.qkn_k0 = q->k0; a.qkn_k1 = q->k1; a.qkn_eps = q->eps;
  return gemm_bf16(a, S(stream));
}

int tfx_gemm_bf16_lora(const tfx_gemm_args* g, const tfx_qkn_args* q, const tfx_lora_args* l, tfx_stream stream) {
  if (!g || !l) return fail("tfx_gemm_bf16_lora: null args");
  if (!g->A || !g->W || !g->C) return fail("tfx_gemm_bf16_lora: null matrix pointer");
  if (!l->T || !l->Bm) return fail("tfx_gemm_bf16_lora: null adapter operand (T / Bm)");
  GemmArgs a;
  a.A = g->A; a.lda = g->lda; a.a_bstride = g->a_bstride;
  a.W = g->W; a.ldw = g->ldw; a.bias = g->bias; a.w_bstride = g->w_bstride;
  a.C = g->C; a.ldc = g->ldc; a.c_bstride = g->c_bstride;
  a.M = g->M; a.N = g->N; a.K = g->K; a.batch = g->batch;
  a.epilogue = g->epilogue; a.gelu_from_col = g->gelu_from_col;
  a.gate = g->gate; a.gate_bstride = g->gate_bstride;
  a.res = g->res; a.ldr = g->ldr; a.r_bstride = g->r_bstride;
  if (q) {
    if (!q->norm_q || !q->norm_k || !q->rope_cs) return fail("tfx_gemm_bf16_lora: norm weights and the rotary table are required");
    if ((uintptr_t)q->norm_q % 16 || (uintptr_t)q->norm_k % 16 || (uintptr_t)q->rope_cs % 16)
      return fail("tfx_gemm_bf16_lora: norm weights and the rotary table must be 16-byte aligned");
    if (q->q0 < 0 || q->q1 < q->q0 || q->q1 > g->N || q->k0 < 0 || q->k1 < q->k0 || q->k1 > g->N || q->pos0 < 0)
      return fail("tfx_gemm_bf16_lora: column ranges outside [0, N)");
    if (g->epilogue != EPI_BIAS && g->epilogue != EPI_BIAS_GELU) return fail("tfx_gemm_bf16_lora: with q/k norm the epilogue must be 0 (bias) or 1 (bias + GELU from a column)");
    a.epilogue = EPI_BIAS_GELU;
    a.gelu_from_col = g->epilogue == EPI_BIAS_GELU ? g->gelu_from_col : (g->N + 255) / 256 * 256;
    a.gate = nullptr; a.gate_bstride = 0; a.res = nullptr; a.ldr = 0; a.r_bstride = 0;
    a.qkn_wq = q->norm_q; a.qkn_wk = q->norm_k; a.qkn_rope_cs = q->rope_cs; a.qkn_pos0 = q->pos0;
    a.qkn_q0 = q->q0; a.qkn_q1 = q->q1; a.qkn_k0 = q->k0; a.qkn_k1 = q->k1; a.qkn_eps = q->eps;
  }
  if (l->split_row > 0) {
    if (!l->W2) return fail("tfx_gemm_bf16_lora: row-split weights need W2");
    if (q && ((uintptr_t)l->norm_q2 % 16 || (uintptr_t)l->norm_k2 % 16)) return fail("tfx_gemm_bf16_lora: norm_q2 / norm_k2 must be 16-byte aligned");
    a.split_row = l->split_row; a.W2 = l->W2; a.bias2 = l->bias2; a.gate2 = l->gate2; a.qkn_wq2 = l->norm_q2; a.qkn_wk2 = l->norm_k2;
  } else if (l->split_row < 0) {
    return fail("tfx_gemm_bf16_lora: split_row must not be negative");
  }
  if (l->t_seg_stride < 0) return fail("tfx_gemm_bf16_lora: t_seg_stride must not be negative");
  LoraArgs la{l->T, l->Bm, l->R, l->seg_cols, l->nseg, l->seg_mask, l->t_seg_stride};
  return gemm_bf16_lora(a, la, S(stream));
}

int tfx_gemm_bf16_f32(const tfx_gemm_args* g, tfx_stream stream) {
  if (!g) return fail("tfx_gemm_bf16_f32: null args");
  if (!g->A || !g->W || !g->C) return fail("tfx_gemm_bf16_f32: null matrix pointer");
  GemmArgs a;
  a.A = g->A; a.lda = g->lda; a.a_bstride = g->a_bstride;
  a.W = g->W; a.ldw = g->ldw; a.bias = g->bias; a.w_bstride = g->w_bstride;
  a.C = g->C; a.ldc = g->ldc; a.c_bstride = g->c_bstride;
  a.M = g->M; a.N = g->N; a.K = g->K; a.batch = g->batch;
  a.epilogue = g->epilogue; a.gelu_from_col = 0;
  a.gate = nullptr; a.gate_bstride = 0; a.res = nullptr; a.ldr = 0; a.r_bstride = 0;
  return gemm_bf16_f32out(a, S(stream));
}

int tfx_gemm_fp8(const tfx_gemm_args* g, const float* a_scale, int64_t a_scale_bstride, const float* w_scale,
                 tfx_stream stream) {
  if (!g) return fail("tfx_gemm_fp8: null args");
  GemmArgs a;
  a.A = g->A; a.lda = g->lda; a.a_bstride = g->a_bstride;
  a.W = g->W; a.ldw = g->ldw; a.bias = g->bias; a.w_bstride = g->w_bstride;
  a.C = g->C; a.ldc = g->ldc; a.c_bstride = g->c_bstride;
  a.M = g->M; a.N = g->N; a.K = g->K; a.batch = g->batch;
  a.epilogue = g->epilogue; a.gelu_from_col = g->gelu_from_col;
  a.gate = g->gate; a.gate_bstride = g->gate_bstride;
  a.res = g->res; a.ldr = g->ldr; a.r_bstride = g->r_bstride;
  a.a_scale = a_scale; a.a_scale_bstride = a_scale_bstride; a.w_scale = w_scale;
  a.workspace = g->workspace; a.workspace_bytes = g->workspace_bytes;
  if (!a.A || !a.W || !a.C) return fail("tfx_gemm_fp8: null matrix pointer");
  return gemm_fp8(a, S(stream));
}

int tfx_quantize_rows_fp8(const void* x, int64_t ldx, int64_t x_bstride, void* out, int64_t ldo, int64_t o_bstride,
                          float* scale, int64_t s_bstride, int32_t rows, int32_t batch, int32_t K, tfx_stream stream) {
  if (!x || !out || !scale) return fail("tfx_quantize_rows_fp8: null pointer");
  return quantize_rows_fp8(x, ldx, x_bstride, out, ldo, o_bstride, scale, s_bstride, rows, batch, K, S(stream));
}

int tfx_ln_modulate_fp8(const void* x, int64_t ldx, int64_t x_bstride, void* q8, int64_t ldq, int64_t q_bstride,
                        float* q8_scale, int64_t s_bstride, const void* shift, const void* scale, int64_t mod_bstride,
                        int32_t rows_per_batch, int32_t batch, int32_t D, float eps, tfx_stream stream) {
  if (!x || !q8 || !q8_scale || !shift || !scale) return fail("tfx_ln_modulate_fp8: null pointer");
  return ln_modulate_fp8(x, q8, q8_scale, shift, scale, mod_bstride, rows_per_batch, batch, D, ldx, x_bstride, ldq,
                         q_bstride, s_bstride, eps, S(stream));
}

int tfx_ln_modulate(const void* x, int64_t ldx, int64_t x_bstride, void* out, int64_t ldo, int64_t o_bstride,
                    const void* shift, const void* scale, int64_t mod_bstride, int32_t rows_per_batch, int32_t batch,
                    int32_t D, float eps, tfx_stream stream) {
  if (!x || !out || !shift || !scale) return fail("tfx_ln_modulate: null pointer");
  return ln_modulate(x, out, shift, scale, mod_bstride, rows_per_batch, batch, D, ldx, x_bstride, ldo, o_bstride, eps,
                     S(stream));
}

int tfx_layernorm(const void* x, int64_t ldx, void* out, int64_t ldo, const void* gamma, const void* beta, int64_t rows,
                  int32_t D, float eps, tfx_stream stream) {
  if (!x || !out || !gamma || !beta) return fail("tfx_layernorm: null pointer");
  if (ldx % 8 || ldo % 8) return fail("tfx_layernorm: row strides must be multiples of 8 elements");
  return layernorm_affine(x, out, gamma, beta, rows, D, ldx, ldo, eps, S(stream));
}

int tfx_rmsnorm_rope(void* buf, int64_t ld, int64_t bstride, int32_t q_off, int32_t k_off, int32_t H, int32_t Ntok,
                     int32_t T, int32_t B, const void* wq_img, const void* wk_img, const void* wq_txt,
                     const void* wk_txt, const float* cos_tab, const float* sin_tab, float eps, tfx_stream stream) {
  if (!buf || !wq_img || !wk_img || !wq_txt || !wk_txt || !cos_tab || !sin_tab) return fail("tfx_rmsnorm_rope: null pointer");
  if (ld % 8 || bstride % 8 || q_off % 8 || k_off % 8) return fail("tfx_rmsnorm_rope: offsets/strides must be multiples of 8");
  return rmsnorm_rope(buf, ld, bstride, q_off, k_off, H, Ntok, T, B, wq_img, wk_img, wq_txt, wk_txt, cos_tab, sin_tab,
                      eps, S(stream));
}

int tfx_rmsnorm_rope_qk(void* buf, int64_t ld, int64_t bstride, int32_t q_off, int32_t k_off, int32_t H, int32_t Ntok,
                        int32_t T, int32_t B, const void* wq_img, const void* wk_img, const void* wq_txt,
                        const void* wk_txt, const float* cos_tab, const float* sin_tab, float eps, tfx_stream stream) {
  return tfx_rmsnorm_rope(buf, ld, bstride, q_off, k_off, H, Ntok, T, B, wq_img, wk_img, wq_txt, wk_txt, cos_tab, sin_tab, eps, stream);
}

int tfx_gate_residual(const void* x, int64_t ldx, int64_t x_bstride, const void* gate, int64_t gate_bstride, const void* res,
                      int64_t ldr, int64_t r_bstride, void* out, int64_t ldo, int64_t o_bstride, int32_t rows_per_batch,
                      int32_t batch, int32_t D, tfx_stream stream) {
  if (!x || !gate || !res || !out) return fail("tfx_gate_residual: null pointer");
  if (D <= 0 || D % 8 || (ldx | x_bstride | ldr | r_bstride | ldo | o_bstride | gate_bstride) % 8)
    return fail("tfx_gate_residual: D and every stride must be multiples of 8 elements");
  if (((uintptr_t)x | (uintptr_t)gate | (uintptr_t)res | (uintptr_t)out) % 16) return fail("tfx_gate_residual: pointers must be 16-byte aligned");
  if (rows_per_batch < 0 || batch < 0) return fail("tfx_gate_residual: negative extent");
  return gate_residual(x, ldx, x_bstride, gate, gate_bstride, res, ldr, r_bstride, out, ldo, o_bstride, rows_per_batch, batch, D, S(stream));
}

int tfx_blend_edge_nhwc(const void* a, int64_t a_bstride, int64_t a_tstride, int64_t a_ustride, void* b, int64_t b_bstride,
                        int64_t b_tstride, int64_t b_ustride, int32_t batch, int32_t extent, int32_t len, int32_t C, tfx_stream stream) {
  if (!a || !b) return fail("tfx_blend_edge_nhwc: null pointer");
  if (C <= 0 || C % 8 || (a_bstride | a_tstride | a_ustride | b_bstride | b_tstride | b_ustride) % 8)
    return fail("tfx_blend_edge_nhwc: C and every stride must be multiples of 8 elements");
  if (((uintptr_t)a | (uintptr_t)b) % 16) return fail("tfx_blend_edge_nhwc: pointers must be 16-byte aligned");
  if (batch < 0 || extent < 0 || len < 0) return fail("tfx_blend_edge_nhwc: negative extent");
  return blend_edge(a, a_bstride, a_tstride, a_ustride, b, b_bstride, b_tstride, b_ustride, batch, extent, len, C, S(stream));
}

int tfx_release_scratch(void) { return attention_w4_release(); }

int tfx_attention_mode_counts(int64_t* counts, int32_t n, int32_t reset) {
  if (!counts && n > 0) return fail("tfx_attention_mode_counts: null pointer");
  return attention_mode_counts(counts, n, reset);
}

int tfx_joint_attention(const tfx_attn_args* g, tfx_stream stream) {
  if (!g || !g->q || !g->k || !g->v || !g->o) return fail("tfx_joint_attention: null pointer");
  AttnArgs a;
  a.q = g->q; a.k = g->k; a.v = g->v; a.o = g->o;
  a.ldq = g->ldq; a.ldk = g->ldk; a.ldv = g->ldv; a.ldo = g->ldo;
  a.q_bstride = g->q_bstride; a.k_bstride = g->k_bstride; a.v_bstride = g->v_bstride; a.o_bstride = g->o_bstride;
  a.B = g->B; a.H = g->H; a.N = g->N; a.scale = g->scale; a.score_bound = g->score_bound;
  a.workspace = g->workspace; a.workspace_bytes = g->workspace ? g->workspace_bytes : 0;
  return joint_attention(a, S(stream));
}

int tfx_euler_step(const void* v, void* x, void* xin, int64_t ldxin, int32_t C, int64_t rows, const float* coef,
                   const int32_t* step_ptr, int32_t step, tfx_stream stream) {
  if (!v || !x || !coef) return fail("tfx_euler_step: null pointer");
  return sched_step(false, v, x, xin, ldxin, C, rows, coef, step_ptr, step, nullptr, S(stream));
}
int tfx_amo_step(const void* v, void* x, void* xin, int64_t ldxin, int32_t C, int64_t rows, const float* coef,
                 const int32_t* step_ptr, int32_t step, const float* noise, tfx_stream stream) {
  if (!v || !x || !coef) return fail("tfx_amo_step: null pointer");
  return sched_step(true, v, x, xin, ldxin, C, rows, coef, step_ptr, step, noise, S(stream));
}

int tfx_timestep_embedding(const float* t, void* out, int32_t n, tfx_stream stream) {
  if (!t || !out) return fail("tfx_timestep_embedding: null pointer");
  return timestep_embedding(t, out, n, S(stream));
}
int tfx_silu(const void* a, void* out, int64_t n, tfx_stream stream) {
  if (!a || !out) return fail("tfx_silu: null pointer");
  return silu_bf16(a, out, n, S(stream));
}
int tfx_add(const void* a, const void* b, void* out, int64_t n, tfx_stream stream) {
  if (!a || !b || !out) return fail("tfx_add: null pointer");
  return add_bf16(a, b, out, n, S(stream));
}
int tfx_scatter_cols(const void* src, void* dst, int64_t rows, int32_t C, int64_t ld, int32_t col0, tfx_stream stream) {
  if (!src || !dst) return fail("tfx_scatter_cols: null pointer");
  return scatter_cols(src, dst, rows, C, ld, col0, S(stream));
}
int tfx_copy_rows(const void* src, int64_t src_ld, int64_t src_bstride, void* dst, int64_t dst_ld, int64_t dst_bstride,
                  int32_t rows, int32_t cols, int32_t batch, tfx_stream stream) {
  if (!src || !dst) return fail("tfx_copy_rows: null pointer");
  return copy_rows(src, src_ld, src_bstride, dst, dst_ld, dst_bstride, rows, cols, batch, S(stream));
}
int tfx_select_step(const void* table, void* cur, int64_t per_step_elems, int32_t* step_ptr, tfx_stream stream) {
  if (!table || !cur || !step_ptr) return fail("tfx_select_step: null pointer");
  return select_step(table, cur, per_step_elems, step_ptr, S(stream));
}
int tfx_advance_step(int32_t* step_ptr, tfx_stream stream) {
  if (!step_ptr) return fail("tfx_advance_step: null pointer");
  return advance_step(step_ptr, S(stream));
}

int tfx_conv3x3_nhwc(const void* x, int32_t B, int32_t inH, int32_t inW, int32_t Cin, const void* w, const void* bias,
                     void* out, int32_t H, int32_t W, int32_t Cout, int32_t stride, int32_t up, int32_t pad_lo,
                     const void* res, const void* zero_page, int variant, tfx_stream stream) {
  if (!x || !w || !out || !zero_page) return fail("tfx_conv3x3_nhwc: null pointer");
  if (up != 1 && up != 2) return fail("tfx_conv3x3_nhwc: up must be 1 or 2");
  GemmArgs a;
  std::memset(&a, 0, sizeof(a));
  const int K = Cin < 64 ? (9 * Cin + 63) / 64 * 64 : 9 * Cin;
  a.A = x; a.lda = Cin; a.W = w; a.ldw = K; a.bias = bias;
  a.C = out; a.ldc = Cout; a.M = B * H * W; a.N = Cout; a.K = K; a.batch = 1;
  a.epilogue = res ? EPI_BIAS_RES : EPI_BIAS;
  a.res = res; a.ldr = Cout;
  a.conv_cin = Cin; a.conv_inH = inH; a.conv_inW = inW; a.conv_H = H; a.conv_W = W;
  a.conv_stride = stride; a.conv_up_shift = up == 2 ? 1 : 0; a.conv_pad_lo = pad_lo; a.zero_page = zero_page;
  a.conv_kw = 3; a.conv_stride_x = 0; a.qkn_eps = 1e-6f;
  return variant < 0 ? gemm_bf16(a, S(stream)) : gemm_bf16_variant(a, variant, S(stream));
}

int tfx_conv3x3_pair_nhwc(const void* x, int32_t B, int32_t H, int32_t W, int32_t Cin, const void* w_pair, const void* bias_pair,
                          void* out, int32_t Cout, const void* res, const void* zero_page, tfx_stream stream) {
  if (!x || !w_pair || !out || !zero_page) return fail("tfx_conv3x3_pair_nhwc: null pointer");
  if (W % 2 || Cin % 64 || Cout % 4) return fail("tfx_conv3x3_pair_nhwc: W must be even, Cin a multiple of 64, Cout of 4");
  GemmArgs a;
  std::memset(&a, 0, sizeof(a));
  const int K = 12 * Cin;
  a.A = x; a.lda = Cin; a.W = w_pair; a.ldw = K; a.bias = bias_pair;
  a.C = out; a.ldc = 2 * Cout; a.M = B * H * (W / 2); a.N = 2 * Cout; a.K = K; a.batch = 1;
  a.epilogue = res ? EPI_BIAS_RES : EPI_BIAS;
  a.res = res; a.ldr = 2 * Cout;
  a.conv_cin = Cin; a.conv_inH = H; a.conv_inW = W; a.conv_H = H; a.conv_W = W / 2;
  a.conv_stride = 1; a.conv_up_shift = 0; a.conv_pad_lo = 1; a.zero_page = zero_page;
  a.conv_kw = 4; a.conv_stride_x = 2;
  return gemm_bf16(a, S(stream));
}

int tfx_groupnorm_nhwc(const void* x, void* out, const void* gamma, const void* beta, float* workspace, int32_t B,
                       int64_t HW, int32_t C, int32_t groups, float eps, int32_t silu, tfx_stream stream) {
  if (!x || !out || !gamma || !beta || !workspace) return fail("tfx_groupnorm_nhwc: null pointer");
  return groupnorm_silu_nhwc(x, out, gamma, beta, workspace, B, HW, C, groups, eps, silu != 0, S(stream));
}

int tfx_any_negative(const void* x, int32_t dtype, int64_t n, int32_t* flag, tfx_stream stream) {
  if (!x || !flag) return fail("tfx_any_negative: null pointer");
  return any_negative(x, dtype, n, flag, S(stream));
}
int tfx_prep_image(const void* img, int32_t img_dtype, const void* mask, int32_t mask_dtype, void* out, int32_t B, int32_t C,
                   int32_t H, int32_t W, int32_t mask_batch, int32_t norm_mode, int32_t binarize, const int32_t* neg_flag,
                   tfx_stream stream) {
  if (!img || !out) return fail("tfx_prep_image: null pointer");
  return prep_image(img, img_dtype, mask, mask_dtype, out, B, C, H, W, mask_batch, norm_mode, binarize, neg_flag, S(stream));
}
int tfx_compose_canvas(const void* glyph, const void* scene, const void* scene_mask_rgb, void* canvas, void* cmask, int32_t B,
                       int32_t gh, int32_t gw, int32_t sh, int32_t sw, int32_t direction, int32_t mask_rgb, tfx_stream stream) {
  if (!glyph || !scene || !scene_mask_rgb || !canvas || !cmask) return fail("tfx_compose_canvas: null pointer");
  return compose_canvas(glyph, scene, scene_mask_rgb, canvas, cmask, B, gh, gw, sh, sw, direction, mask_rgb, S(stream));
}
int tfx_rgb_to_grey_u8(const void* rgb, void* out, int64_t pixels, tfx_stream stream) {
  if (!rgb || !out) return fail("tfx_rgb_to_grey_u8: null pointer");
  return rgb_to_grey(rgb, out, pixels, S(stream));
}
int tfx_resample_u8(const void* in, void* out, const int32_t* bounds, const int32_t* coeffs, int32_t ksize, int64_t outer,
                    int32_t in_len, int32_t out_len, int32_t inner, tfx_stream stream) {
  if (!in || !out || !bounds || !coeffs) return fail("tfx_resample_u8: null pointer");
  return resample_u8(in, out, bounds, coeffs, ksize, outer, in_len, out_len, inner, S(stream));
}
int tfx_pack_mask(const void* mask, int32_t mask_dtype, void* out, int32_t B, int32_t H, int32_t W, int32_t mask_batch,
                  int32_t binarize, int64_t ld, int32_t col0, tfx_stream stream) {
  if (!mask || !out) return fail("tfx_pack_mask: null pointer");
  return pack_mask(mask, mask_dtype, out, B, H, W, mask_batch, binarize, ld, col0, S(stream));
}
int tfx_vae_sample_pack(const void* moments, const void* eps, int32_t eps_dtype, void* out, int32_t B, int32_t h, int32_t w,
                        int32_t L, float shift, float scale, int64_t ld, int32_t col0, tfx_stream stream) {
  if (!moments || !out) return fail("tfx_vae_sample_pack: null pointer");
  return sample_pack(moments, eps, eps_dtype, out, B, h, w, L, shift, scale, ld, col0, S(stream));
}
int tfx_unpack_latents(const void* latents, int64_t ld, void* out, int32_t B, int32_t h, int32_t w, int32_t L, float shift,
                       float scale, tfx_stream stream) {
  if (!latents || !out) return fail("tfx_unpack_latents: null pointer");
  return unpack_latents(latents, ld, out, B, h, w, L, shift, scale, S(stream));
}
int tfx_postprocess(const void* x, void* out, int32_t B, int32_t H, int32_t W, int32_t Cs, int32_t C, int32_t mode, int32_t denorm,
                    int32_t y0, int32_t x0, int32_t Hc, int32_t Wc, tfx_stream stream) {
  if (!x || !out) return fail("tfx_postprocess: null pointer");
  return postprocess(x, out, B, H, W, Cs, C, mode, denorm, y0, x0, Hc, Wc, S(stream));
}
int tfx_transpose(const void* in, int64_t ldi, int64_t in_bstride, void* out, int64_t ldo, int64_t out_bstride, int32_t N,
                  int32_t C, int32_t batch, tfx_stream stream) {
  if (!in || !out) return fail("tfx_transpose: null pointer");
  return transpose_bf16(in, ldi, in_bstride, out, ldo, out_bstride, N, C, batch, S(stream));
}
int tfx_row_softmax(const float* s, int64_t lds, void* p, int64_t ldp, int32_t rows, int32_t N, float scale, tfx_stream stream) {
  if (!s || !p) return fail("tfx_row_softmax: null pointer");
  return row_softmax(s, lds, p, ldp, rows, N, scale, S(stream));
}

int tfx_attention64(const tfx_attn_args* g, const float* rel_bias, int32_t causal, tfx_stream stream) {
  if (!g || !g->q || !g->k || !g->v || !g->o) return fail("tfx_attention64: null pointer");
  AttnArgs a;
  a.q = g->q; a.k = g->k; a.v = g->v; a.o = g->o;
  a.ldq = g->ldq; a.ldk = g->ldk; a.ldv = g->ldv; a.ldo = g->ldo;
  a.q_bstride = g->q_bstride; a.k_bstride = g->k_bstride; a.v_bstride = g->v_bstride; a.o_bstride = g->o_bstride;
  a.B = g->B; a.H = g->H; a.N = g->N; a.scale = g->scale;
  return attention64(a, rel_bias, causal, S(stream));
}
int tfx_rmsnorm(const void* x, int32_t x_dtype, int64_t ldx, const void* w, void* out, int64_t ldo, int64_t rows, int32_t D,
                float eps, tfx_stream stream) {
  if (!x || !w || !out) return fail("tfx_rmsnorm: null pointer");
  return rmsnorm(x, x_dtype, ldx, w, out, ldo, rows, D, eps, S(stream));
}
int tfx_gather_rows(const void* table, const int64_t* ids, void* out, int64_t n, int32_t D, int64_t vocab, tfx_stream stream) {
  if (!table || !ids || !out) return fail("tfx_gather_rows: null pointer");
  return gather_rows(table, ids, out, n, D, vocab, S(stream));
}
int tfx_add_into_f32(float* x, const void* y, int64_t n, int32_t mode, tfx_stream stream) {
  if (!x || !y) return fail("tfx_add_into_f32: null pointer");
  return add_into_f32(x, y, n, mode, S(stream));
}
int tfx_mul_act(const void* a, int64_t lda, const void* b, int64_t ldb, void* out, int64_t ldo, int64_t rows, int32_t cols,
                int32_t mode, tfx_stream stream) {
  if (!a || !out) return fail("tfx_mul_act: null pointer");
  return mul_act(a, lda, b, ldb, out, ldo, rows, cols, mode, S(stream));
}

int tfx_set_option(const char* name, int value) {
  if (!name) return fail("tfx_set_option: null name");
  if (!std::strcmp(name, "attention_waves")) {
    if (value == 0) { set_attention_waves(0); return 0; }
    if (value != 4 && value != 8 && value != 9 && value != 10 && value != 12 && value != 16 && value != 20 && !(value >= 30 && value <= 34) && value != 40)
      return fail("tfx_set_option: attention_waves must be 4, 8, 9 (128 keys per barrier), 10 / 12 (matrix-pipe softmax, 8 / 4 waves), 16 (ping-pong), 20 (half-tile pipelined), 30 .. 34 (one wave per SIMD, 32x32x16 MFMA: 30 bookkeeping on the matrix pipe -- or no reference at all when the call carries an admissible score bound -- / 31 row sums on the VALU / 32 = 31 + lazy reference offset / 33 = 30 + lazy reference offset / 34 = no reference with a score bound, else 33) or 40 (one wave per SIMD, 16x16x32 MFMA)");
#ifndef TFX_BENCH
    if (value != 30 && value != 34)
      return fail("tfx_set_option: attention_waves %d is a bench-only kernel (libtextflux_hip_bench.so, `make bench`); the product library "
                  "carries 30 (the default) and 34", value);
#endif
    set_attention_waves(value);
    return 0;
  }
  if (!std::strcmp(name, "gemm_group_m")) { set_gemm_group_m(value); return 0; }
  if (!std::strcmp(name, "attention_tail_split")) { set_attention_tail_split(value); return 0; }
  if (!std::strcmp(name, "attention_use_bound")) { set_attention_use_bound(value); return 0; }
  if (!std::strcmp(name, "attention_persistent")) { set_attention_persistent(value); return 0; }
  if (!std::strcmp(name, "attention_streamk")) { set_attention_streamk(value); return 0; }
  if (!std::strcmp(name, "gemm_place")) { set_gemm_place(value); return 0; }
  if (!std::strcmp(name, "gemm_waves")) {
#ifndef TFX_BENCH
    if (value != 8 && value != 0) return fail("tfx_set_option: gemm_waves 4 (gemm4w_kernel) is bench-only (libtextflux_hip_bench.so, `make bench`)");
#endif
    set_gemm_waves(value);
    return 0;
  }
  if (!std::strcmp(name, "gemm_group_streams")) { g_group_streams = value; return 0; }
  if (!std::strcmp(name, "ln_joint")) { g_ln_joint = value; return 0; }
  if (!std::strcmp(name, "ln_prefetch")) { set_ln_prefetch(value); return 0; }
  if (!std::strcmp(name, "fp8_fuse_qkn")) { g_fp8_fuse_qkn = value; return 0; }
  if (!std::strcmp(name, "gemm_splitk")) { set_gemm_splitk(value); return 0; }
  if (!std::strcmp(name, "attention_ablation")) { set_attention_ablation(value); return 0; }
  return fail("tfx_set_option: unknown option '%s'", name);
}

int tfx_debug_attention_timing(void* buf) { set_attention_debug(buf); return 0; }

int tfx_mfma_peak_probe(const void* operands, int64_t operand_bytes, int32_t fp8, int32_t ktiles, double* flops, tfx_stream stream) {
  return mfma_peak_probe(operands, operand_bytes, fp8, ktiles, flops, S(stream));
}

int tfx_prof_enable(int on) { prof_enable(on); return 0; }
int tfx_prof_collect(int kind, double* total_ms, double* total_flops, int* launches) {
  if (kind < 0 || kind > 2) return fail("tfx_prof_collect: kind must be 0 (gemm), 1 (attention) or 2 (fp8 gemm)");
  return prof_collect(kind, total_ms, total_flops, launches);
}

static inline int64_t align256(int64_t v) { return (v + 255) & ~(int64_t)255; }
int tfx_workspace_layout(int32_t B, int32_t Sn, int32_t T, int32_t D, int32_t flags, int64_t* off, int64_t* gemm_ws_bytes) {
  if (B <= 0 || Sn <= 0 || T < 0 || D <= 0 || !off) return fail("tfx_workspace_layout: bad arguments");
  const int64_t N = (int64_t)Sn + T, hid = align256(B * N * D * 2), y = align256(B * N * 7 * (int64_t)D * 2);
  const bool fp8 = (flags & 4) != 0;
  const int64_t q8 = fp8 ? align256(B * N * 5 * (int64_t)D) : 0, q8s = fp8 ? align256(B * N * 4) : 0, gws = 128ll << 20;
  int64_t o = 0;
  off[0] = o; o += hid;
  off[1] = o; o += hid;
  off[2] = o; o += y;
  off[3] = fp8 ? o : -1; o += q8;
  off[4] = fp8 ? o : -1; o += q8s;
  off[5] = o;
  if (flags & 8) {
    o += gws;
    off[6] = o; o += (D >= 1024 ? 1 : 4) * hid;
    off[7] = o;
  }
  if (gemm_ws_bytes) *gemm_ws_bytes = gws;
  return 0;
}
int64_t tfx_workspace_bytes(int32_t B, int32_t Sn, int32_t T, int32_t D, int32_t flags) {
  int64_t off[8], gws = 0;
  if (tfx_workspace_layout(B, Sn, T, D, flags, off, &gws)) return -1;
  if (flags & 8) return off[7] + ((off[3] >= 0 ? off[3] : off[5]) - off[2]);
  return off[5] + gws;
}

namespace {
struct StepGraph { hipGraph_t graph; hipGraphExec_t exec; };

int step_check(const tfx_step_desc* s) {
  if (!s) return fail("tfx_dit_step: null descriptor");
  if (!s->mod_table || !s->mod_cur || !s->step_ptr) return fail("tfx_dit_step: null pointer in descriptor");
  if (s->dit.mod != s->mod_cur) return fail("tfx_dit_step: dit.mod must point at mod_cur (the rows the step selects)");
  if (s->sampler < 0 || s->sampler > 2) return fail("tfx_dit_step: sampler must be 0 (Euler), 1 (AMO) or 2 (Euler fused into proj_out)");
  if (s->sampler == 2) {
    const char* g = (const char*)s->dit.euler_gate;
    if (!g || g < (const char*)s->mod_cur || g >= (const char*)s->mod_cur + s->mod_step_elems * 2)
      return fail("tfx_dit_step: sampler 2 needs dit.euler_gate inside mod_cur (the step's dsigma row is selected with its modulation rows)");
    return 0;
  }
  if (s->dit.euler_gate) return fail("tfx_dit_step: dit.euler_gate is set but sampler is not 2");
  if (!s->latents || !s->coef) return fail("tfx_dit_step: null pointer in descriptor");
  if (s->sampler == 1 && !s->noise) return fail("tfx_dit_step: the AMO sampler needs a noise buffer");
  if (!s->dit.out) return fail("tfx_dit_step: dit.out is null");
  return 0;
}

int step_enqueue(const tfx_step_desc& s, hipStream_t st) {
  TRY(select_step(s.mod_table, s.mod_cur, s.mod_step_elems, s.step_ptr, st));
  TRY(tfx_dit_forward(&s.dit, (tfx_stream)st));
  if (s.sampler == 2) return advance_step(s.step_ptr, st);
  const int64_t rows = (int64_t)s.dit.B * s.dit.S;
  TRY(sched_step(s.sampler == 1, s.dit.out, s.latents, const_cast<void*>(s.dit.xin), s.dit.in_channels, s.dit.out_channels, rows,
                 s.coef, s.step_ptr, 0, s.noise, st));
  return advance_step(s.step_ptr, st);
}
}

int tfx_dit_step_run(const tfx_step_desc* s, tfx_stream stream) {
  TRY(step_check(s));
  return step_enqueue(*s, S(stream));
}

int tfx_dit_step_capture(const tfx_step_desc* s, tfx_stream stream, tfx_graph* out) {
  TRY(step_check(s));
  if (!out) return fail("tfx_dit_step_capture: null output handle");
  if (!stream) return fail("tfx_dit_step_capture: the NULL stream cannot be captured; pass a created stream");
  hipStream_t st = S(stream);
  (void)attention_w4_prepare(st);
  hipError_t e = hipStreamBeginCapture(st, hipStreamCaptureModeThreadLocal);
  if (e != hipSuccess) return fail("tfx_dit_step_capture: hipStreamBeginCapture: %s", hipGetErrorString(e));
  const int rc = step_enqueue(*s, st);
  hipGraph_t g = nullptr;
  e = hipStreamEndCapture(st, &g);
  if (rc) { if (g) (void)hipGraphDestroy(g); return rc; }
  if (e != hipSuccess || !g) return fail("tfx_dit_step_capture: hipStreamEndCapture: %s", hipGetErrorString(e));
  hipGraphExec_t x = nullptr;
  e = hipGraphInstantiate(&x, g, nullptr, nullptr, 0);
  if (e != hipSuccess) { (void)hipGraphDestroy(g); return fail("tfx_dit_step_capture: hipGraphInstantiate: %s", hipGetErrorString(e)); }
  *out = new StepGraph{g, x};
  return 0;
}

int tfx_dit_step_replay(tfx_graph graph, tfx_stream stream) {
  if (!graph) return fail("tfx_dit_step_replay: null graph");
  const hipError_t e = hipGraphLaunch(((StepGraph*)graph)->exec, S(stream));
  if (e != hipSuccess) return fail("tfx_dit_step_replay: hipGraphLaunch: %s", hipGetErrorString(e));
  return 0;
}

int tfx_graph_destroy(tfx_graph graph) {
  if (!graph) return 0;
  StepGraph* g = (StepGraph*)graph;
  (void)hipGraphExecDestroy(g->exec);
  (void)hipGraphDestroy(g->graph);
  delete g;
  return 0;
}

int tfx_dit_forward(const tfx_dit_desc* d, tfx_stream stream) {
  if (!d) return fail("tfx_dit_forward: null descriptor");
  if (!d->xin || !d->mod || !d->hid || !d->xn || !d->y || !d->out || !d->cos_tab || !d->sin_tab)
    return fail("tfx_dit_forward: null buffer in descriptor");
  if ((d->n_double > 0 && !d->dbl) || (d->n_single > 0 && !d->sgl)) return fail("tfx_dit_forward: null block table");
  if (d->T > 0 && !d->ctx0) return fail("tfx_dit_forward: ctx0 is null");
  return dit_forward(*d, S(stream));
}

}
```

### textflux_amd/csrc/gemm.hip

```cpp
#include <algorithm>
#include <type_traits>

#include "common.h"
#include "launch.h"

namespace tfx {

struct GemmParams {
  const bf16_t* A; int64_t lda, a_bs;
  const bf16_t* W; int64_t ldw, w_bs;
  const bf16_t* bias;
  bf16_t* C; int64_t ldc, c_bs;
  int M, N, K, batch, tm, tn, gm;
  int gelu_from;
#ifdef TFX_BENCH
  unsigned long long* timers;
#endif
  const bf16_t* gate; int64_t gate_bs;
  const bf16_t* res; int64_t ldr, r_bs;
  int cin, inH, inW, oH, oW, cstride, cup, cpad;
  int ckw, cstride_x;
  int csh;
  const bf16_t* zero;
  const float* a_scale; int64_t as_bs; const float* w_scale;
// ... 1317 lines not shown
    for (int j = 0; j < 4; ++j) r += acc[i][j][0] + acc[i][j][1] + acc[i][j][2] + acc[i][j][3];
  if (r == 123456.789f) sink[0] = r;
}

int mfma_peak_probe(const void* operands, int64_t operand_bytes, int fp8, int ktiles, double* flops, hipStream_t st) {
  if (!operands || (uintptr_t)operands % 16 || operand_bytes < 16 * 64 * 16) return fail("mfma_peak_probe: operands must be a 16-byte aligned buffer of at least 16 KiB");
  if (ktiles < 48 || ktiles % 48) return fail("mfma_peak_probe: ktiles must be a positive multiple of 48");
  int dev = 0, cus = 0;
  (void)hipGetDevice(&dev);
  if (hipDeviceGetAttribute(&cus, hipDeviceAttributeMultiprocessorCount, dev) != hipSuccess || cus < 8) cus = 256;
  static float* sink = nullptr;
  if (!sink && hipMalloc((void**)&sink, 256) != hipSuccess) return fail("mfma_peak_probe: hipMalloc failed");
  const int nfrag = (int)std::min<int64_t>(operand_bytes / 16, 1 << 30);
  if (fp8) mfma_probe_kernel<true><<<cus, 512, 0, st>>>((const u32x4*)operands, nfrag, ktiles, sink);
  else mfma_probe_kernel<false><<<cus, 512, 0, st>>>((const u32x4*)operands, nfrag, ktiles, sink);
  if (flops) *flops = (double)cus * 8.0 * (double)ktiles * (fp8 ? 32.0 * 65536.0 : 64.0 * 16384.0);
  return check_launch("mfma_peak_probe");
}

static int g_gemm_splitk = 2;
void set_gemm_splitk(int v) { g_gemm_splitk = v; }
static int g_gemm_waves = 8;
void set_gemm_waves(int v) { g_gemm_waves = v == 4 ? 4 : 8; }
static int g_gemm_place = 2;
void set_gemm_place(int v) { g_gemm_place = v; }
#ifdef TFX_BENCH
static unsigned long long* g_gemm_timers = nullptr;
extern "C" void tfx_bench_gemm_timers(unsigned long long* dev) { g_gemm_timers = dev; }
#endif
static int g_gemm_group_m = 0;
void set_gemm_group_m(int gm) { g_gemm_group_m = gm < 0 ? 0 : gm; }

static GemmParams make_params(const GemmArgs& a) {
  GemmParams p;
  p.A = (const bf16_t*)a.A; p.lda = a.lda; p.a_bs = a.a_bstride;
  p.W = (const bf16_t*)a.W; p.ldw = a.ldw; p.w_bs = a.w_bstride;
  p.bias = (const bf16_t*)a.bias;
  p.C = (bf16_t*)a.C; p.ldc = a.ldc; p.c_bs = a.c_bstride;
  p.M = a.M; p.N = a.N; p.K = a.K; p.batch = a.batch;
  p.tm = (a.M + 255) / 256; p.tn = (a.N + 255) / 256;
  p.gm = g_gemm_group_m ? g_gemm_group_m : (p.tn <= 12 ? 1 : 4);
  p.gelu_from = a.gelu_from_col;
#ifdef TFX_BENCH
  p.timers = g_gemm_timers;
#endif
  p.gate = (const bf16_t*)a.gate; p.gate_bs = a.gate_bstride;
  p.res = (const bf16_t*)a.res; p.ldr = a.ldr; p.r_bs = a.r_bstride;
  p.cin = a.conv_cin; p.inH = a.conv_inH; p.inW = a.conv_inW; p.oH = a.conv_H; p.oW = a.conv_W;
  p.cstride = a.conv_stride; p.cup = a.conv_up_shift; p.cpad = a.conv_pad_lo; p.zero = (const bf16_t*)a.zero_page;
  p.ckw = a.conv_kw; p.cstride_x = a.conv_stride_x > 0 ? a.conv_stride_x : a.conv_stride;
  p.csh = a.conv_cin == 8 ? 3 : a.conv_cin == 16 ? 4 : a.conv_cin == 32 ? 5 : 0;
  p.a_scale = a.a_scale; p.as_bs = a.a_scale_bstride; p.w_scale = a.w_scale;
  p.ws = nullptr; p.sk = 1; p.u_full = 0; p.tail_r = 0; p.ws_ld = 0; p.ws_bs = 0;
  p.split_row = a.split_row; p.w2_off = 0;
  p.bias2 = (const bf16_t*)a.bias2; p.gate2 = (const bf16_t*)a.gate2; p.nq_w2 = (const bf16_t*)a.qkn_wq2; p.nk_w2 = (const bf16_t*)a.qkn_wk2;
  if (a.split_row > 0) p.w2_off = (uint32_t)((const char*)a.W2 - (const char*)a.W);
  p.nq_w = (const bf16_t*)a.qkn_wq; p.nk_w = (const bf16_t*)a.qkn_wk; p.rope_cs = a.qkn_rope_cs; p.rope_pos0 = a.qkn_pos0;
  p.nq0 = a.qkn_q0; p.nq1 = a.qkn_q1; p.nk0 = a.qkn_k0; p.nk1 = a.qkn_k1; p.n_eps = a.qkn_eps;
  p.t_off = 0; p.t_seg = 0; p.lora_rt = 0; p.seg_cols = 0; p.nseg = 0; p.seg_mask = 0;
  p.cscale = a.cscale;
  return p;
}

static bool conv_ok(const GemmArgs& a) {
  const bool wide = a.conv_cin % 64 == 0 && (a.conv_kw == 3 || a.conv_kw == 4) && a.K == 3 * a.conv_kw * a.conv_cin;
  const bool narrow = a.conv_kw == 3 && (a.conv_cin == 8 || a.conv_cin == 16 || a.conv_cin == 32) && a.K == (9 * a.conv_cin + 63) / 64 * 64;
  return (wide || narrow) && a.batch == 1 && a.zero_page && (uintptr_t)a.zero_page % 16 == 0 &&
         a.conv_H > 0 && a.conv_W > 0 && (a.conv_inH << a.conv_up_shift) < 32768 && (a.conv_inW << a.conv_up_shift) < 32768 &&
         (int64_t)a.M * 1 == (int64_t)a.conv_H * a.conv_W * (a.M / (a.conv_H * a.conv_W)) && a.M % (a.conv_H * a.conv_W) == 0;
}

static bool fast_ok(const GemmArgs& a) {
  if (a.conv_cin > 0 && !conv_ok(a)) return false;
  const bool al16 = ((uintptr_t)a.A % 16 == 0) && ((uintptr_t)a.W % 16 == 0) && ((uintptr_t)a.C % 16 == 0) &&
                    ((uintptr_t)a.bias % 8 == 0);
  return a.K % 64 == 0 && a.K >= 64 && a.N % 8 == 0 && a.lda % 8 == 0 && a.ldw % 8 == 0 && a.ldc % 8 == 0 && a.w_bstride % 8 == 0 && a.w_bstride >= 0 &&
         a.a_bstride % 8 == 0 && a.c_bstride % 8 == 0 && al16 && (int64_t)255 * a.lda < (1ll << 31) &&
         (int64_t)255 * a.ldw < (1ll << 31) &&
         ((a.epilogue != EPI_BIAS_GATE_RES && a.epilogue != EPI_BIAS_RES) || (a.ldr % 8 == 0 && a.r_bstride % 8 == 0 && a.gate_bstride % 4 == 0 &&
                                              (uintptr_t)a.res % 16 == 0 && (uintptr_t)a.gate % 8 == 0)) &&
         (a.epilogue != EPI_BIAS_GELU || a.gelu_from_col % 256 == 0);
}

static bool persist_ok(const GemmParams& p) {
  return p.cin == 0 && p.K % 128 == 0 &&
         ((int64_t)(p.batch - 1) * p.a_bs + (int64_t)p.tm * 256 * p.lda) * 2 < (1ll << 32) - 65536 &&
         ((int64_t)(p.batch - 1) * p.w_bs + (int64_t)p.tn * 256 * p.ldw) * 2 < (1ll << 32) - 65536;
}

struct SlicePlan { int sk, u_full, tail_r; };
static SlicePlan plan_slices(const GemmParams& p, int grid, int nt, void* ws, int64_t ws_bytes) {
  SlicePlan pl{1, 0, 0};
  if (!g_gemm_splitk || !ws || p.N % 8) return pl;
  const int per_batch = p.tm * p.tn, T = p.batch * per_batch;
  auto ok = [&](int units, int c) { return units * c <= grid && nt % (2 * c) == 0 && nt / c >= 8 && (int64_t)units * c * 262144 <= ws_bytes; };
  if (T < grid) {
    for (int c : {8, 6, 4, 3, 2})
      if (ok(T, c)) return SlicePlan{c, 0, per_batch};
    return pl;
  }
  const int R = T % grid;
  if (R == 0 || T / grid >= 8 || R % p.batch || g_gemm_splitk < 2) return pl;
  for (int c : {4, 3, 2})
    if (ok(R, c)) return SlicePlan{c, T - R, R / p.batch};
  return pl;
}

#ifdef TFX_BENCH
template <int ABL>
static int launch_ablation(const GemmParams& p, hipStream_t st) {
  (void)hipFuncSetAttribute((const void*)gemm8p_kernel<EPI_BIAS, ABL>, hipFuncAttributeMaxDynamicSharedMemorySize, LDS_TOTAL);
  gemm8p_kernel<EPI_BIAS, ABL><<<(unsigned)(p.batch * p.tm * p.tn), 512, LDS_TOTAL, st>>>(p);
  return check_launch("gemm_ablation");
}
#endif

template <int EPI>
static int launch_variant(const GemmParams& p, int variant, void* ws, int64_t ws_bytes, hipStream_t st) {
  if (variant >= 10) {
#ifndef TFX_BENCH
    return fail("gemm: ablation variants are bench-only (build with -DTFX_BENCH)");
#else
    switch (variant - 10) {
      case 1: return launch_ablation<1>(p, st);
      case 2: return launch_ablation<2>(p, st);
      case 3: return launch_ablation<3>(p, st);
      case 4: return launch_ablation<4>(p, st);
      case 7: return launch_ablation<7>(p, st);
      case 8: return launch_ablation<8>(p, st);
      case 16: return launch_ablation<16>(p, st);
      case 17: return launch_ablation<17>(p, st);
      case 18: return launch_ablation<18>(p, st);
      case 32768: return launch_ablation<32768>(p, st);
      case 65536: return launch_ablation<65536>(p, st);
      case 98304: return launch_ablation<98304>(p, st);
    }
    return fail("gemm: unknown ablation");
#endif
  }
  if ((variant == 1 || variant == 3) && persist_ok(p)) {
    static int grid = 0;
    if (!grid) {
      int dev = 0, cus = 0;
      (void)hipGetDevice(&dev);
      if (hipDeviceGetAttribute(&cus, hipDeviceAttributeMultiprocessorCount, dev) != hipSuccess || cus < 8) cus = 256;
      const void* fns[2] = {(const void*)gemm8pp_kernel<EPI, 1>, (const void*)gemm8pp_kernel<EPI, 2>};
      for (const void* fn : fns) {
        hipFuncAttributes fa;
        (void)hipFuncGetAttributes(&fa, fn);
        (void)hipGetLastError();
        const hipError_t e = hipFuncSetAttribute(fn, hipFuncAttributeMaxDynamicSharedMemorySize, PP_LDS_TOTAL);
        if (e != hipSuccess)
          return fail("gemm: cannot raise dynamic LDS limit to %d bytes: %s", PP_LDS_TOTAL, hipGetErrorString(e));
      }
      grid = cus & ~7;
    }
    const bool prof = prof_on(st);
    if (prof) prof_begin(0, 2.0 * p.M * (double)p.N * p.K * p.batch, st);
    const int nt = p.K >> 6;
    const SlicePlan pl = variant == 1 ? plan_slices(p, grid, nt, ws, ws_bytes) : SlicePlan{1, 0, 0};
    const int sk = pl.sk;
#ifdef TFX_BENCH
    if (g_gemm_waves == 4 && sk == 1 && p.K >= 256) {
      if (p.rope_cs && EPI != EPI_BIAS_GELU) return fail("gemm: the q/k norm + RoPE epilogue rides on the bias(+GELU) epilogue");
      static bool attr4[2] = {false, false};
      const int qi = p.rope_cs ? 1 : 0;
      const void* fn = qi ? (const void*)gemm4w_kernel<EPI_BIAS_GELU, true> : (const void*)gemm4w_kernel<EPI, false>;
      if (!attr4[qi]) {
        hipFuncAttributes fa;
        (void)hipFuncGetAttributes(&fa, fn);
        (void)hipGetLastError();
        if (hipFuncSetAttribute(fn, hipFuncAttributeMaxDynamicSharedMemorySize, W4G_LDS_TOTAL) != hipSuccess)
          return fail("gemm: cannot raise dynamic LDS limit for the 4-wave kernel");
        attr4[qi] = true;
      }
      if (qi) gemm4w_kernel<EPI_BIAS_GELU, true><<<grid, 256, W4G_LDS_TOTAL, st>>>(p);
      else gemm4w_kernel<EPI, false><<<grid, 256, W4G_LDS_TOTAL, st>>>(p);
    } else
#endif
    if (p.rope_cs) {
      if (sk > 1) return fail("gemm: the q/k norm + RoPE epilogue cannot ride on a K-sliced launch (gemm_qkn_ok)");
      if (EPI != EPI_BIAS_GELU) return fail("gemm: the q/k norm + RoPE epilogue rides on the bias(+GELU) epilogue");
      static bool attrq = false;
      const void* fn = (const void*)gemm8pp_kernel<EPI_BIAS_GELU, 2, false, false, true>;
      if (!attrq) {
        hipFuncAttributes fa;
        (void)hipFuncGetAttributes(&fa, fn);
        (void)hipGetLastError();
        if (hipFuncSetAttribute(fn, hipFuncAttributeMaxDynamicSharedMemorySize, PP_LDS_TOTAL) != hipSuccess)
          return fail("gemm: cannot raise dynamic LDS limit for the q/k-norm kernel");
        attrq = true;
      }
      gemm8pp_kernel<EPI_BIAS_GELU, 2, false, false, true><<<grid, 512, PP_LDS_TOTAL, st>>>(p);
    } else if (sk > 1) {
      static bool attr = false;
      if (!attr) {
        const void* fns[2] = {(const void*)gemm8pp_kernel<EPI_BIAS, 2, false, true>, (const void*)gemm8pp_kernel<EPI, 2, false, true>};
        for (const void* fn : fns) {
          hipFuncAttributes fa;
          (void)hipFuncGetAttributes(&fa, fn);
          (void)hipGetLastError();
          if (hipFuncSetAttribute(fn, hipFuncAttributeMaxDynamicSharedMemorySize, PP_LDS_TOTAL) != hipSuccess)
            return fail("gemm: cannot raise dynamic LDS limit for the K-sliced kernel");
        }
        attr = true;
      }
      GemmParams ps = p;
      ps.ws = (float*)ws; ps.sk = sk; ps.u_full = pl.u_full; ps.tail_r = pl.tail_r;
      if (pl.u_full == 0)
        gemm8pp_kernel<EPI_BIAS, 2, false, true><<<grid, 512, PP_LDS_TOTAL, st>>>(ps);
      else
        gemm8pp_kernel<EPI, 2, false, true><<<grid, 512, PP_LDS_TOTAL, st>>>(ps);
      tail_reduce_kernel<EPI><<<(unsigned)(p.batch * pl.tail_r * 32), 256, 0, st>>>(ps);
    } else if (g_gemm_place == 1) {
      gemm8pp_kernel<EPI, 1><<<grid, 512, PP_LDS_TOTAL, st>>>(p);
    } else {
      gemm8pp_kernel<EPI, 2><<<grid, 512, PP_LDS_TOTAL, st>>>(p);
    }
    if (prof) prof_end(0, st);
    return check_launch("gemm_bf16");
  }
  if (variant == 3) return fail("gemm: shape not eligible for the persistent kernel");
  if (variant == 1 || variant == 2) {
    const int conv = p.cin > 0 ? (p.csh ? 2 : 1) : 0;
    static bool attr_set[3] = {false, false, false};
    if (!attr_set[conv]) {
      const void* fn = conv == 2 ? (const void*)gemm8p_kernel<EPI, 0, 2> : conv == 1 ? (const void*)gemm8p_kernel<EPI, 0, 1>
                                                                                  : (const void*)gemm8p_kernel<EPI, 0, 0>;
      hipFuncAttributes fa;
      (void)hipFuncGetAttributes(&fa, fn);
      (void)hipGetLastError();
      const hipError_t e = hipFuncSetAttribute(fn, hipFuncAttributeMaxDynamicSharedMemorySize, LDS_TOTAL);
      if (e != hipSuccess)
        return fail("gemm: cannot raise dynamic LDS limit to %d bytes: %s", LDS_TOTAL, hipGetErrorString(e));
      attr_set[conv] = true;
    }
    const unsigned grid = (unsigned)(p.batch * p.tm * p.tn);
    const bool prof = prof_on(st) && !conv;
    if (prof) prof_begin(0, 2.0 * p.M * (double)p.N * p.K * p.batch, st);
    if (conv == 2)
      gemm8p_kernel<EPI, 0, 2><<<grid, 512, LDS_TOTAL, st>>>(p);
    else if (conv == 1)
      gemm8p_kernel<EPI, 0, 1><<<grid, 512, LDS_TOTAL, st>>>(p);
    else
      gemm8p_kernel<EPI, 0, 0><<<grid, 512, LDS_TOTAL, st>>>(p);
    if (prof) prof_end(0, st);
  } else {
    dim3 grid((p.N + 63) / 64, (p.M + 63) / 64, p.batch);
    gemm_generic_kernel<EPI><<<grid, 256, 0, st>>>(p);
  }
  return check_launch("gemm_bf16");
}

int gemm_bf16_variant(const GemmArgs& a, int variant, hipStream_t st) {
  if (a.M <= 0 || a.N <= 0 || a.batch <= 0) return 0;
  if (a.K <= 0) return fail("gemm: K must be positive");
  if (variant >= 1 && !fast_ok(a)) return fail("gemm: shape/alignment not supported by the MFMA kernel");
  if (a.epilogue == EPI_BIAS_GATE_RES && (!a.gate || !a.res)) return fail("gemm: gate/res pointers required");
  if (a.epilogue == EPI_BIAS_RES && !a.res) return fail("gemm: res pointer required");
  if (a.epilogue == EPI_COLSCALE && (!a.cscale || (uintptr_t)a.cscale % 16 || a.bias || a.split_row > 0))
    return fail("gemm: the column-scale epilogue needs a 16-byte aligned fp32 cscale vector and takes no bias / row-split weights");
  const GemmParams p = make_params(a);
  if (a.split_row > 0 && !((variant == 1 || variant == 3) && gemm_rowsplit_ok(a))) return fail("gemm: row-split weights need the persistent MFMA kernel");
  switch (a.epilogue) {
    case EPI_BIAS: return launch_variant<EPI_BIAS>(p, variant, a.workspace, a.workspace_bytes, st);
    case EPI_BIAS_GELU: return launch_variant<EPI_BIAS_GELU>(p, variant, a.workspace, a.workspace_bytes, st);
    case EPI_BIAS_GATE_RES: return launch_variant<EPI_BIAS_GATE_RES>(p, variant, a.workspace, a.workspace_bytes, st);
    case EPI_BIAS_RES: return launch_variant<EPI_BIAS_RES>(p, variant, a.workspace, a.workspace_bytes, st);
    case EPI_COLSCALE: return launch_variant<EPI_COLSCALE>(p, variant, a.workspace, a.workspace_bytes, st);
  }
  return fail("gemm: unknown epilogue %d", a.epilogue);
}

bool gemm_rowsplit_ok(const GemmArgs& a) {
  if (a.split_row <= 0 || a.split_row % 256 || a.split_row >= a.M || !fast_ok(a) || a.conv_cin > 0 || !a.W2 || a.w_bstride) return false;
  const GemmParams p = make_params(a);
  if (!persist_ok(p)) return false;
  const int64_t d = (const char*)a.W2 - (const char*)a.W;
  if (d <= 0 || d % 16 || d + (int64_t)p.tn * 256 * p.ldw * 2 >= (1ll << 32) - 65536) return false;
  if ((a.bias == nullptr) != (a.bias2 == nullptr) || (uintptr_t)a.bias2 % 8) return false;
  if (a.epilogue == EPI_BIAS_GATE_RES && (!a.gate2 || (uintptr_t)a.gate2 % 8)) return false;
  if (a.qkn_rope_cs && (!a.qkn_wq2 || !a.qkn_wk2)) return false;
  return true;
}

int gemm_bf16(const GemmArgs& a, hipStream_t st) {
  if (a.split_row > 0 && !gemm_rowsplit_ok(a)) return fail("gemm: shape / layout not eligible for row-split weights (gemm_rowsplit_ok)");
  if (a.qkn_rope_cs && !gemm_qkn_ok(a)) return fail("gemm: shape not eligible for the fused q/k norm + RoPE epilogue");
  return gemm_bf16_variant(a, fast_ok(a) ? 1 : 0, st);
}

bool gemm_qkn_ok(const GemmArgs& a) {
  if (!fast_ok(a) || a.conv_cin > 0 || (a.epilogue != EPI_BIAS_GELU && a.epilogue != EPI_BIAS)) return false;
  const GemmParams p = make_params(a);
  if (!persist_ok(p)) return false;
  if ((a.qkn_q0 | a.qkn_q1 | a.qkn_k0 | a.qkn_k1) % 256) return false;
  if (a.epilogue == EPI_BIAS_GELU && a.gelu_from_col < (a.qkn_q1 > a.qkn_k1 ? a.qkn_q1 : a.qkn_k1)) return false;
  int dev = 0, cus = 256;
  (void)hipGetDevice(&dev);
  if (hipDeviceGetAttribute(&cus, hipDeviceAttributeMultiprocessorCount, dev) != hipSuccess || cus < 8) cus = 256;
  return plan_slices(p, cus & ~7, p.K >> 6, a.workspace, a.workspace_bytes).sk == 1;
}

template <int EPI, bool QKN>
static int launch_lora(const GemmParams& p, hipStream_t st) {
  static int grid = 0;
  if (!grid) {
    int dev = 0, cus = 0;
    (void)hipGetDevice(&dev);
    if (hipDeviceGetAttribute(&cus, hipDeviceAttributeMultiprocessorCount, dev) != hipSuccess || cus < 8) cus = 256;
    const void* fn = (const void*)gemm8pp_kernel<EPI, 2, false, false, QKN, true>;
    hipFuncAttributes fa;
    (void)hipFuncGetAttributes(&fa, fn);
    (void)hipGetLastError();
    const hipError_t e = hipFuncSetAttribute(fn, hipFuncAttributeMaxDynamicSharedMemorySize, PP_LDS_TOTAL);
    if (e != hipSuccess) return fail("gemm_lora: cannot raise dynamic LDS limit to %d bytes: %s", PP_LDS_TOTAL, hipGetErrorString(e));
    grid = cus & ~7;
  }
  const bool prof = prof_on(st);
  if (prof) prof_begin(0, 2.0 * p.M * (double)p.N * (p.K + p.lora_rt * 64) * p.batch, st);
  gemm8pp_kernel<EPI, 2, false, false, QKN, true><<<grid, 512, PP_LDS_TOTAL, st>>>(p);
  if (prof) prof_end(0, st);
  return check_launch("gemm_bf16_lora");
}

int gemm_bf16_lora(const GemmArgs& a, const LoraArgs& l, hipStream_t st) {
  if (a.M <= 0 || a.N <= 0 || a.batch <= 0) return 0;
  if (a.K <= 0) return fail("gemm_lora: K must be positive");
  if (!fast_ok(a) || a.conv_cin > 0 || a.w_bstride) return fail("gemm_lora: shape/alignment not supported by the persistent MFMA kernel");
  if (a.epilogue == EPI_BIAS_GATE_RES && (!a.gate || !a.res)) return fail("gemm_lora: gate/res pointers required");
  if (a.epilogue == EPI_BIAS_RES && !a.res) return fail("gemm_lora: res pointer required");
  if (a.epilogue == EPI_COLSCALE) return fail("gemm_lora: the column-scale epilogue is the down projection's (tfx_gemm_bf16)");
  if (l.R < 128 || l.R % 128 || l.R > LORA_MAX_RANK) return fail("gemm_lora: R (the padded rank) must be 128 or 256");
  if (l.nseg < 1 || l.nseg > 4 || l.seg_cols <= 0 || l.seg_cols % 256) return fail("gemm_lora: 1..4 segments of seg_cols %% 256 == 0 output columns");
  if ((int64_t)(l.nseg - 1) * l.seg_cols >= a.N) return fail("gemm_lora: segment %d starts beyond N", l.nseg - 1);
  const uint32_t ok_bits = (1u << l.nseg) - 1u;
  if (l.seg_mask & ~(ok_bits | (a.split_row > 0 ? ok_bits << 8 : 0u))) return fail("gemm_lora: seg_mask has bits outside its %d segments", l.nseg);
  const int64_t d = (const char*)l.T - (const char*)a.A;
  if ((uintptr_t)l.T % 16 || d <= 0) return fail("gemm_lora: T must be 16-byte aligned and lie above A");
  const int64_t t_seg = l.t_seg > 0 ? l.t_seg : l.R;
  if (t_seg == l.R ? (int64_t)l.nseg * l.R > a.lda : (l.R > a.lda || t_seg % 8 || t_seg < (int64_t)(a.batch - 1) * a.a_bstride + (int64_t)(a.M - 1) * a.lda + l.R))
    return fail("gemm_lora: T's %d blocks of R columns do not fit A's row pitch (or overlap as separate matrices)", l.nseg);
  if ((const char*)l.Bm != (const char*)a.W + (int64_t)a.K * 2 || a.ldw < (int64_t)a.K + l.R) return fail("gemm_lora: Bm must be W + K with ldw >= K + R");
  if (a.split_row > 0 && !gemm_rowsplit_ok(a)) return fail("gemm_lora: shape / layout not eligible for row-split weights (gemm_rowsplit_ok)");
  GemmParams p = make_params(a);
  if (!persist_ok(p) || d + (l.nseg - 1) * t_seg * 2 + ((int64_t)(p.batch - 1) * p.a_bs + (int64_t)p.tm * 256 * p.lda) * 2 >= (1ll << 32) - 65536)
    return fail("gemm_lora: K %% 128 == 0 and A, T within one 32-bit byte range are required");
  p.t_off = (uint32_t)d; p.t_seg = (uint32_t)(t_seg * 2); p.lora_rt = l.R / 64; p.seg_cols = l.seg_cols; p.nseg = l.nseg; p.seg_mask = l.seg_mask;
  if (a.qkn_rope_cs) {
    if (a.epilogue != EPI_BIAS_GELU) return fail("gemm_lora: the q/k norm + RoPE epilogue rides on the bias(+GELU) epilogue");
    if ((a.qkn_q0 | a.qkn_q1 | a.qkn_k0 | a.qkn_k1) % 256 || a.gelu_from_col < (a.qkn_q1 > a.qkn_k1 ? a.qkn_q1 : a.qkn_k1))
      return fail("gemm_lora: q / k column ranges must be multiples of 256 in front of gelu_from_col");
    return launch_lora<EPI_BIAS_GELU, true>(p, st);
  }
  switch (a.epilogue) {
    case EPI_BIAS: return launch_lora<EPI_BIAS, false>(p, st);
    case EPI_BIAS_GELU: return launch_lora<EPI_BIAS_GELU, false>(p, st);
    case EPI_BIAS_GATE_RES: return launch_lora<EPI_BIAS_GATE_RES, false>(p, st);
    case EPI_BIAS_RES: return launch_lora<EPI_BIAS_RES, false>(p, st);
  }
  return fail("gemm_lora: unknown epilogue %d", a.epilogue);
}

bool gemm_fp8_qkn_ok(const GemmArgs& a) {
  if (a.conv_cin > 0 || (a.epilogue != EPI_BIAS_GELU && a.epilogue != EPI_BIAS) || a.split_row > 0) return false;
  if (a.K <= 0 || a.K % 256 || a.N % 8 || (a.qkn_q0 | a.qkn_q1 | a.qkn_k0 | a.qkn_k1) % 256) return false;
  if (a.epilogue == EPI_BIAS_GELU && (a.gelu_from_col % 256 || a.gelu_from_col < (a.qkn_q1 > a.qkn_k1 ? a.qkn_q1 : a.qkn_k1))) return false;
  int dev = 0, cus = 256;
  (void)hipGetDevice(&dev);
  if (hipDeviceGetAttribute(&cus, hipDeviceAttributeMultiprocessorCount, dev) != hipSuccess || cus < 8) cus = 256;
  const int64_t T = (int64_t)a.batch * ((a.M + 255) / 256) * ((a.N + 255) / 256);
  return T >= (cus & ~7);
}

int gemm_bf16_f32out(const GemmArgs& a, hipStream_t st) {
  if (a.M <= 0 || a.N <= 0 || a.batch <= 0) return 0;
  if (a.K <= 0) return fail("gemm_f32out: K must be positive");
  if (a.epilogue != EPI_BIAS || a.bias) return fail("gemm_f32out: raw accumulators only (no bias / epilogue)");
  if (a.conv_cin > 0) return fail("gemm_f32out: no convolution mode");
  if ((uintptr_t)a.C % 16 || a.ldc % 4 || a.c_bstride % 4) return fail("gemm_f32out: C must be 16-byte aligned, ldc / c_bstride multiples of 4");
  GemmParams p = make_params(a);
  p.ws = (float*)a.C; p.sk = 1; p.u_full = 0; p.tail_r = p.tm * p.tn; p.ws_ld = a.ldc; p.ws_bs = a.c_bstride;
  GemmArgs chk = a;
  chk.C = const_cast<void*>(a.A);
  chk.ldc = 8; chk.c_bstride = 8;
  if (fast_ok(chk) && persist_ok(p)) {
    static int grid = 0;
    if (!grid) {
      int dev = 0, cus = 0;
      (void)hipGetDevice(&dev);
      if (hipDeviceGetAttribute(&cus, hipDeviceAttributeMultiprocessorCount, dev) != hipSuccess || cus < 8) cus = 256;
      const void* fn = (const void*)gemm8pp_kernel<EPI_BIAS, 2, false, true>;
      hipFuncAttributes fa;
      (void)hipFuncGetAttributes(&fa, fn);
      (void)hipGetLastError();
      if (hipFuncSetAttribute(fn, hipFuncAttributeMaxDynamicSharedMemorySize, PP_LDS_TOTAL) != hipSuccess)
        return fail("gemm_f32out: cannot raise dynamic LDS limit");
      grid = cus & ~7;
    }
    const bool prof = prof_on(st);
    if (prof) prof_begin(0, 2.0 * p.M * (double)p.N * p.K * p.batch, st);
    gemm8pp_kernel<EPI_BIAS, 2, false, true><<<grid, 512, PP_LDS_TOTAL, st>>>(p);
    if (prof) prof_end(0, st);
  } else {
    dim3 grid((p.N + 63) / 64, (p.M + 63) / 64, p.batch);
    gemm_generic_kernel<EPI_BIAS><<<grid, 256, 0, st>>>(p);
  }
  return check_launch("gemm_f32out");
}

template <int EPI>
static int launch_fp8(const GemmParams& p, void* ws, int64_t ws_bytes, hipStream_t st) {
  static int grid = 0;
  if (!grid) {
    int dev = 0, cus = 0;
    (void)hipGetDevice(&dev);
    if (hipDeviceGetAttribute(&cus, hipDeviceAttributeMultiprocessorCount, dev) != hipSuccess || cus < 8) cus = 256;
    const void* fns[2] = {(const void*)gemm8pp_kernel<EPI, 2, true>, (const void*)gemm8pp_kernel<EPI_BIAS, 2, true, true>};
    for (const void* fn : fns) {
      hipFuncAttributes fa;
      (void)hipFuncGetAttributes(&fa, fn);
      (void)hipGetLastError();
      const hipError_t e = hipFuncSetAttribute(fn, hipFuncAttributeMaxDynamicSharedMemorySize, PP_LDS_TOTAL);
      if (e != hipSuccess) return fail("gemm_fp8: cannot raise dynamic LDS limit to %d bytes: %s", PP_LDS_TOTAL, hipGetErrorString(e));
    }
    grid = cus & ~7;
  }
  const bool prof = prof_on(st);
  if (prof) prof_begin(2, 2.0 * p.M * (double)p.N * p.K * p.batch, st);
  const int T = p.batch * p.tm * p.tn, nt = p.K >> 7;
  SlicePlan pl = T < grid ? plan_slices(p, grid, nt, ws, ws_bytes) : SlicePlan{1, 0, 0};
  if (p.rope_cs) {
    if (pl.sk > 1 || EPI != EPI_BIAS_GELU) {
      if (prof) prof_end(2, st);
      return fail("gemm_fp8: the q/k norm + RoPE epilogue needs an unsliced launch with the bias(+GELU) epilogue (gemm_fp8_qkn_ok)");
    }
    static bool attrq = false;
    const void* fn = (const void*)gemm8pp_kernel<EPI_BIAS_GELU, 2, true, false, true>;
    if (!attrq) {
      hipFuncAttributes fa;
      (void)hipFuncGetAttributes(&fa, fn);
      (void)hipGetLastError();
      if (hipFuncSetAttribute(fn, hipFuncAttributeMaxDynamicSharedMemorySize, PP_LDS_TOTAL) != hipSuccess) {
        if (prof) prof_end(2, st);
        return fail("gemm_fp8: cannot raise dynamic LDS limit for the q/k-norm kernel");
      }
      attrq = true;
    }
    gemm8pp_kernel<EPI_BIAS_GELU, 2, true, false, true><<<grid, 512, PP_LDS_TOTAL, st>>>(p);
  } else if (pl.sk > 1) {
    GemmParams ps = p;
    ps.ws = (float*)ws; ps.sk = pl.sk; ps.u_full = 0; ps.tail_r = pl.tail_r;
    gemm8pp_kernel<EPI_BIAS, 2, true, true><<<grid, 512, PP_LDS_TOTAL, st>>>(ps);
    tail_reduce_kernel<EPI, true><<<(unsigned)(p.batch * pl.tail_r * 32), 256, 0, st>>>(ps);
  } else {
    gemm8pp_kernel<EPI, 2, true><<<grid, 512, PP_LDS_TOTAL, st>>>(p);
  }
  if (prof) prof_end(2, st);
  return check_launch("gemm_fp8");
}

int gemm_fp8(const GemmArgs& a, hipStream_t st) {
  if (a.M <= 0 || a.N <= 0 || a.batch <= 0) return 0;
  if (!a.a_scale || !a.w_scale) return fail("gemm_fp8: scale pointers required");
  if (a.w_bstride) return fail("gemm_fp8: per-batch weights (w_bstride) are a bf16-path feature");
  if (a.conv_cin > 0) return fail("gemm_fp8: no convolution mode");
  const bool al = ((uintptr_t)a.A % 16 == 0) && ((uintptr_t)a.W % 16 == 0) && ((uintptr_t)a.C % 16 == 0) &&
                  ((uintptr_t)a.bias % 8 == 0) && ((uintptr_t)a.w_scale % 16 == 0);
  const int tm = (a.M + 255) / 256, tn = (a.N + 255) / 256;
  if (!(a.K > 0 && a.K % 256 == 0 && a.N % 8 == 0 && a.lda % 16 == 0 && a.ldw % 16 == 0 && a.a_bstride % 16 == 0 &&
        a.ldc % 8 == 0 && a.c_bstride % 8 == 0 && al && (int64_t)(a.batch - 1) * a.a_bstride + (int64_t)tm * 256 * a.lda < (1ll << 32) &&
        (int64_t)tn * 256 * a.ldw < (1ll << 32) && (int64_t)255 * a.lda < (1ll << 31) && (int64_t)255 * a.ldw < (1ll << 31)))
    return fail("gemm_fp8: shape/alignment not supported (K %% 256 == 0, N %% 8 == 0, 16-byte aligned rows)");
  if ((a.epilogue == EPI_BIAS_GATE_RES || a.epilogue == EPI_BIAS_RES) &&
      !(a.res && a.ldr % 8 == 0 && a.r_bstride % 8 == 0 && (uintptr_t)a.res % 16 == 0))
    return fail("gemm_fp8: residual pointer / alignment");
  if (a.epilogue == EPI_BIAS_GATE_RES && !(a.gate && a.gate_bstride % 4 == 0 && (uintptr_t)a.gate % 8 == 0))
    return fail("gemm_fp8: gate pointer / alignment");
  if (a.epilogue == EPI_BIAS_GELU && a.gelu_from_col % 256) return fail("gemm_fp8: gelu_from_col must be a multiple of 256");
  if (a.qkn_rope_cs) {
    if (!a.qkn_wq || !a.qkn_wk) return fail("gemm_fp8: the fused q/k norm + RoPE epilogue needs both norm weight vectors");
    if (!gemm_fp8_qkn_ok(a)) return fail("gemm_fp8: shape / column ranges not eligible for the fused q/k norm + RoPE epilogue (gemm_fp8_qkn_ok)");
  }
  const GemmParams p = make_params(a);
  switch (a.epilogue) {
    case EPI_BIAS: return launch_fp8<EPI_BIAS>(p, a.workspace, a.workspace_bytes, st);
    case EPI_BIAS_GELU: return launch_fp8<EPI_BIAS_GELU>(p, a.workspace, a.workspace_bytes, st);
    case EPI_BIAS_GATE_RES: return launch_fp8<EPI_BIAS_GATE_RES>(p, a.workspace, a.workspace_bytes, st);
    case EPI_BIAS_RES: return launch_fp8<EPI_BIAS_RES>(p, a.workspace, a.workspace_bytes, st);
  }
  return fail("gemm_fp8: unknown epilogue %d", a.epilogue);
}

}
```

### textflux_amd/csrc/launch.h

```cpp
#pragma once
#include <hip/hip_runtime.h>
#include <stdint.h>

namespace tfx {

int fail(const char* fmt, ...);
int check_launch(const char* what);
const char* last_error();

void prof_enable(int on);
bool prof_on();
bool prof_on(hipStream_t st);
void prof_begin(int kind, double flops, hipStream_t st);
void prof_end(int kind, hipStream_t st);
int prof_collect(int kind, double* total_ms, double* total_flops, int* launches);

enum Epilogue : int {
  EPI_BIAS = 0,
  EPI_BIAS_GELU = 1,
  EPI_BIAS_GATE_RES = 2,
  EPI_BIAS_RES = 3,
  EPI_COLSCALE = 4,
};

struct GemmArgs {
  const void* A; int64_t lda; int64_t a_bstride;
  const void* W;
  int64_t ldw;
  int64_t w_bstride = 0;
  const void* bias;
  void* C; int64_t ldc; int64_t c_bstride;
  int M, N, K, batch;
  int epilogue;
  int gelu_from_col;
  const void* gate; int64_t gate_bstride;
  const void* res; int64_t ldr; int64_t r_bstride;
  int conv_cin = 0, conv_inH = 0, conv_inW = 0, conv_H = 0, conv_W = 0, conv_stride = 1, conv_up_shift = 0, conv_pad_lo = 1;
  int conv_kw = 3, conv_stride_x = 0;
  const void* zero_page = nullptr;
  const float* a_scale = nullptr; int64_t a_scale_bstride = 0;
  const float* w_scale = nullptr;
  const void* qkn_wq = nullptr; const void* qkn_wk = nullptr; const float* qkn_rope_cs = nullptr;
  int qkn_pos0 = 0, qkn_q0 = 0, qkn_q1 = 0, qkn_k0 = 0, qkn_k1 = 0; float qkn_eps = 1e-6f;
  void* workspace = nullptr; int64_t workspace_bytes = 0;
  const float* cscale = nullptr;
  int split_row = 0;
  const void* W2 = nullptr; const void* bias2 = nullptr; const void* gate2 = nullptr; const void* qkn_wq2 = nullptr; const void* qkn_wk2 = nullptr;
};
bool gemm_rowsplit_ok(const GemmArgs& a);
void set_gemm_group_m(int gm);
void set_gemm_place(int v);
void set_gemm_waves(int v);
void set_gemm_splitk(int v);
int gemm_bf16(const GemmArgs& a, hipStream_t st);
bool gemm_qkn_ok(const GemmArgs& a);
bool gemm_fp8_qkn_ok(const GemmArgs& a);
constexpr int LORA_MAX_RANK = 256;
struct LoraArgs { const void* T; const void* Bm; int R, seg_cols, nseg; uint32_t seg_mask; int64_t t_seg = 0; };
int gemm_bf16_lora(const GemmArgs& a, const LoraArgs& l, hipStream_t st);
int gemm_bf16_variant(const GemmArgs& a, int variant, hipStream_t st);
int gemm_bf16_f32out(const GemmArgs& a, hipStream_t st);
int mfma_peak_probe(const void* operands, int64_t operand_bytes, int fp8, int ktiles, double* flops, hipStream_t st);
int gemm_fp8(const GemmArgs& a, hipStream_t st);
int ln_modulate_fp8(const void* x, void* q8, float* q8_scale, const void* shift, const void* scale, int64_t mod_bstride,
                    int rows_per_batch, int batch, int D, int64_t ldx, int64_t x_bstride, int64_t ldq, int64_t q_bstride,
                    int64_t s_bstride, float eps, hipStream_t st);
int quantize_rows_fp8(const void* x, int64_t ldx, int64_t x_bstride, void* out, int64_t ldo, int64_t o_bstride, float* scale,
                      int64_t s_bstride, int rows, int batch, int K, hipStream_t st);

struct AttnArgs {
  const void* q; const void* k; const void* v; void* o;
  int64_t ldq, ldk, ldv, ldo;
  int64_t q_bstride, k_bstride, v_bstride, o_bstride;
  int B, H, N;
  float scale;
  float score_bound = 0.f;
  void* workspace = nullptr;
  int64_t workspace_bytes = 0;
};
int joint_attention(const AttnArgs& a, hipStream_t st);
int joint_attention_hp(const AttnArgs& a, hipStream_t st);
int joint_attention_w16(const AttnArgs& a, hipStream_t st);
int attention_w4_release();
int attention_w4_prepare(hipStream_t st);
void set_attention_tail_split(int v);
int joint_attention_w4(const AttnArgs& a, hipStream_t st, int mode);
void set_attention_ablation(int a);
void set_attention_use_bound(int v);
int attention_mode_counts(int64_t* counts, int n, int reset);
void attention_note_streamk();
int blend_edge(const void* a, int64_t a_bs, int64_t a_ts, int64_t a_us, void* b, int64_t b_bs, int64_t b_ts, int64_t b_us, int batch,
               int extent, int len, int C, hipStream_t st);
int gate_residual(const void* x, int64_t ldx, int64_t x_bs, const void* gate, int64_t gate_bs, const void* res, int64_t ldr, int64_t r_bs,
                  void* out, int64_t ldo, int64_t o_bs, int rows, int batch, int D, hipStream_t st);
void set_attention_streamk(int v);
void set_attention_persistent(int v);
void set_attention_debug(void* p);
void set_attention_waves(int nw);

int groupnorm_silu_nhwc(const void* x, void* out, const void* gamma, const void* beta, float* stats_ws, int B,
                        int64_t HW, int C, int groups, float eps, bool silu, hipStream_t st);
void set_ln_prefetch(int v);
int ln_modulate_split(const void* x, void* out, const void* shift, const void* scale, const void* shift2, const void* scale2,
                      int split_row, int64_t mod_bstride, int rows_per_batch, int batch, int D, int64_t ldx, int64_t x_bstride, int64_t ldo,
                      int64_t o_bstride, float eps, hipStream_t st);
int ln_modulate(const void* x, void* out, const void* shift, const void* scale, int64_t mod_bstride,
                int rows_per_batch, int batch, int D, int64_t ldx, int64_t x_bstride, int64_t ldo,
                int64_t o_bstride, float eps, hipStream_t st);
int layernorm_affine(const void* x, void* out, const void* gamma, const void* beta, int64_t rows, int D, int64_t ldx, int64_t ldo,
                     float eps, hipStream_t st);
int rmsnorm_rope(void* buf, int64_t ld, int64_t bstride, int q_off, int k_off, int H, int Ntok, int T, int B,
                 const void* wq_img, const void* wk_img, const void* wq_txt, const void* wk_txt, const float* cosT,
                 const float* sinT, float eps, hipStream_t st);
int sched_step(bool amo, const void* v, void* x, void* xin, int64_t ldxin, int C, int64_t rows, const float* coef,
               const int* step_ptr, int step, const float* noise, hipStream_t st);
int timestep_embedding(const float* t, void* out, int n, hipStream_t st);
int silu_bf16(const void* a, void* out, int64_t n, hipStream_t st);
int add_bf16(const void* a, const void* b, void* out, int64_t n, hipStream_t st);
int scatter_cols(const void* src, void* dst, int64_t rows, int C, int64_t ld, int col0, hipStream_t st);
int copy_rows(const void* src, int64_t sld, int64_t sbs, void* dst, int64_t dld, int64_t dbs, int rows, int cols,
              int batch, hipStream_t st);
int any_negative(const void* x, int dtype, int64_t n, int* flag, hipStream_t st);
int prep_image(const void* img, int img_dtype, const void* mask, int mask_dtype, void* out, int B, int C, int H, int W,
               int mask_b, int norm_mode, int binarize, const int* neg_flag, hipStream_t st);
int compose_canvas(const void* glyph, const void* scene, const void* smask, void* canvas, void* cmask, int B, int gh, int gw, int sh,
                   int sw, int dir, int mask_rgb, hipStream_t st);
int rgb_to_grey(const void* rgb, void* out, int64_t n, hipStream_t st);
int resample_u8(const void* in, void* out, const int* bounds, const int* coeffs, int ksize, int64_t outer, int in_len, int out_len,
                int inner, hipStream_t st);
int pack_mask(const void* mask, int mask_dtype, void* out, int B, int H, int W, int mask_b, int binarize, int64_t ld, int col0,
              hipStream_t st);
int sample_pack(const void* moments, const void* eps, int eps_dtype, void* out, int B, int h, int w, int L, float shift,
                float scale, int64_t ld, int col0, hipStream_t st);
int unpack_latents(const void* lat, int64_t ld, void* out, int B, int h, int w, int L, float shift, float scale, hipStream_t st);
int postprocess(const void* x, void* out, int B, int H, int W, int Cs, int C, int mode, int denorm, int y0, int x0, int Hc, int Wc,
                hipStream_t st);
int transpose_bf16(const void* in, int64_t ldi, int64_t ibs, void* out, int64_t ldo, int64_t obs, int N, int C, int batch,
                   hipStream_t st);
int row_softmax(const float* s, int64_t lds, void* p, int64_t ldp, int rows, int N, float scale, hipStream_t st);
int attention64(const AttnArgs& a, const float* rel_bias, int causal, hipStream_t st);
int rmsnorm(const void* x, int x_dtype, int64_t ldx, const void* w, void* out, int64_t ldo, int64_t rows, int D, float eps,
            hipStream_t st);
int gather_rows(const void* table, const int64_t* ids, void* out, int64_t n, int D, int64_t vocab, hipStream_t st);
int add_into_f32(float* x, const void* y, int64_t n, int mode, hipStream_t st);
int mul_act(const void* a, int64_t lda, const void* b, int64_t ldb, void* out, int64_t ldo, int64_t rows, int cols, int mode,
            hipStream_t st);
int select_step(const void* table, void* cur, int64_t per_step_elems, int* step_ptr, hipStream_t st);
int advance_step(int* step_ptr, hipStream_t st);

}
```

Measured before the change: 0.5867.

## Compute only image rows in last single block and defer attention output stores

For the final single-stream block, only the image-token rows feed the output. So the QKV/MLP GEMM for text rows is cut to the Q/K/V columns, attention runs only over query rows past the text tokens via a new Nq range, and the output projection runs only on image rows. Separately, the persistent attention kernel now stages a finished tile's normalized output in extra LDS and writes it to global memory spread across the next tile's steps, so the store tail overlaps compute. The deferred store adds LDS usage (a 256x240 staging area) and extra code in the hot loop, which could affect scheduling.

```diff
diff --git a/textflux_amd/csrc/attention.hip b/textflux_amd/csrc/attention.hip
--- a/textflux_amd/csrc/attention.hip
+++ b/textflux_amd/csrc/attention.hip
@@ -717,7 +717,11 @@
     return fail("attention: strides must be multiples of 8 elements (q,k,v) / 4 (o)");
   if (((uintptr_t)a.q | (uintptr_t)a.k | (uintptr_t)a.v) % 16 || (uintptr_t)a.o % 8)
     return fail("attention: q/k/v must be 16-byte aligned, o 8-byte aligned");
+  const bool qsub = a.Nq > 0 && a.Nq != a.N;
+  const double qfrac = qsub ? (double)a.Nq / a.N : 1.0;
 #ifdef TFX_BENCH
+  if (qsub && (g_attn_waves == 20 || g_attn_waves == 40))
+    return fail("attention: kernel variant %d takes no query-row range (AttnArgs::Nq)", g_attn_waves);
   if (g_attn_waves == 20 && !g_attn_abl) {
     const bool prof = prof_on(st);
     if (prof) prof_begin(1, 4.0 * a.B * a.H * (double)a.N * a.N * HD, st);
@@ -746,7 +750,7 @@
   if ((g_attn_waves == 30 || g_attn_waves == 34) && w4_ok) {
 #endif
     const bool prof = prof_on(st);
-    if (prof) prof_begin(1, 4.0 * a.B * a.H * (double)a.N * a.N * HD, st);
+    if (prof) prof_begin(1, 4.0 * a.B * a.H * (double)a.N * a.N * HD * qfrac, st);
     const bool bounded = attn_bound_admissible(a.score_bound, a.N);
 #ifdef TFX_BENCH
     const int mode = g_attn_waves == 34 ? (bounded ? 4 : 3) : g_attn_waves == 30 ? (bounded && g_attn_bound ? 4 : 0)
@@ -759,6 +763,7 @@
     ++g_attn_mode_count[mode];
     return rc ? rc : check_launch("joint_attention");
   }
+  if (qsub) return fail("attention: a query-row range (AttnArgs::Nq) needs the one-wave-per-SIMD kernel (attention_waves 30 .. 34, 16-byte aligned output rows)");
 #ifndef TFX_BENCH
   if (g_attn_waves != 30 && g_attn_waves != 34)
     return fail("attention: kernel variant %d is a bench-only schedule (libtextflux_hip_bench.so, `make bench`)", g_attn_waves);
diff --git a/textflux_amd/csrc/attention_w4.hip b/textflux_amd/csrc/attention_w4.hip
--- a/textflux_amd/csrc/attention_w4.hip
+++ b/textflux_amd/csrc/attention_w4.hip
@@ -28,11 +28,14 @@
 }
 
 constexpr int ATT_LDS_W4 = W4_NBUF * (W4_VT + W4_KT);
+constexpr int W4_DROW = 240;
+constexpr int ATT_LDS_W4_ALL = ATT_LDS_W4 + 256 * W4_DROW;
 
 #define W4_GAP() __builtin_amdgcn_sched_barrier(0)
 #ifndef W4_ABL
 #define W4_ABL 0
 #endif
+constexpr int W4_LDS_LAUNCH = (W4_ABL & 256) ? ATT_LDS_W4 + 4096 : ATT_LDS_W4_ALL;
 #define W4_DRAIN_MFMA()                                                                                                 \
   asm volatile("s_nop 15\n\ts_nop 15\n\ts_nop 15\n\ts_nop 15\n\ts_nop 15\n\ts_nop 15\n\ts_nop 15\n\ts_nop 15\n\t"      \
                "s_nop 15\n\ts_nop 15\n\ts_nop 15\n\ts_nop 15\n\ts_nop 15\n\ts_nop 15\n\ts_nop 15\n\ts_nop 15\n\t"      \
@@ -110,9 +113,10 @@
                                                          int64_t ldv, int64_t ldo, int64_t q_bs, int64_t k_bs, int64_t v_bs,
                                                          int64_t o_bs, int H, int N, int nqb, float scale_log2e, int nfull,
                                                          int nparts, int nsplit, int xsplit, float* part, int T_items, int sk_group,
-                                                         int sk_share) {
+                                                         int sk_share, int Nq, int defer_out) {
   extern __shared__ __attribute__((aligned(16))) char smem[];
   constexpr bool LV = MODE == 1 || MODE == 2, LZ = MODE >= 2, NOREF = MODE == 4, FT = LV || NOREF;
+  constexpr bool DEFER = MODE == 4;
   const int tid = threadIdx.x, lane = tid & 63;
   const int wave = __builtin_amdgcn_readfirstlane(tid >> 6);
   const int hi = lane >> 5, l31 = lane & 31;
@@ -188,6 +192,8 @@
   }
   bf16x8 qn[2][8];
   bool have_pref = false;
+  bool have_def = false;
+  uint32_t def_vo = 0;
   u32x4 kreg[4], vreg[4];
 #ifdef TFX_BENCH
   unsigned long long w4_stamp[4] = {0, 0, 0, 0}, w4_sum[4] = {0, 0, 0, 0};
@@ -228,7 +234,7 @@
 #pragma unroll
   for (int qb = 0; qb < 2; ++qb) {
     qrow[qb] = qblk * 256 + wave * 64 + qb * 32 + l31;
-    const int rc = qrow[qb] < N ? qrow[qb] : N - 1;
+    const int rc = qrow[qb] < Nq ? qrow[qb] : Nq - 1;
     if (have_pref) {
 #pragma unroll
       for (int s = 0; s < 8; ++s) qf[qb][s] = qn[qb][s];
@@ -242,7 +248,7 @@
 #pragma unroll
     for (int qb = 0; qb < 2; ++qb) {
       const int r2 = qblk2 * 256 + wave * 64 + qb * 32 + l31;
-      const int rc = r2 < N ? r2 : N - 1;
+      const int rc = r2 < Nq ? r2 : Nq - 1;
 #pragma unroll
       for (int s = 0; s < 8; ++s) qn[qb][s] = *reinterpret_cast<const bf16x8*>(Qb2 + (int64_t)rc * ldq + s * 16 + hi * 8);
     }
@@ -428,10 +434,10 @@
 #endif
   W4_GAP();
 
-  auto step = [&](auto QBc, auto PVc, auto FIRSTc, auto KNc, auto VNc, auto STGc, int jst, bool rag, int kb_abs) __attribute__((always_inline)) {
+  auto step = [&](auto QBc, auto PVc, auto FIRSTc, auto KNc, auto VNc, auto STGc, int jst, bool rag, int kb_abs, auto DGc) __attribute__((always_inline)) {
     constexpr int QB = decltype(QBc)::value, OQ = 1 - QB;
     constexpr bool EVEN = QB == 0, PV = decltype(PVc)::value != 0, FIRST = decltype(FIRSTc)::value != 0;
-    constexpr int KN = decltype(KNc)::value, VN = decltype(VNc)::value, STG = decltype(STGc)::value;
+    constexpr int KN = decltype(KNc)::value, VN = decltype(VNc)::value, STG = decltype(STGc)::value, DG = decltype(DGc)::value;
     f32x16& cur = sc[QB];
     f32x16& nxt = sc[OQ];
     if (__builtin_expect_with_probability(rag, 0, 1.0)) {
@@ -497,6 +503,7 @@
     };
     int stg_ko = 0, stg_vo = 0;
     if constexpr ((STG & 3) == 1 && !(W4_ABL & 4)) stage_offsets(stg_ko, stg_vo);
+    u32x4 def_t = {0, 0, 0, 0};
     auto G = [&](auto Ic) __attribute__((always_inline)) {
       constexpr int n = decltype(Ic)::value;
       if constexpr ((STG & 3) == 1 && !(W4_ABL & 4)) {
@@ -504,6 +511,18 @@
         constexpr int g = n < 2 ? n : is_w ? (n + 1) / 2 : n == 15 ? 7 : n / 2 - 1;
         if constexpr (is_w) { if constexpr (!(W4_ABL & 64)) write_piece(STG >> 2, IC<g / 2>{}, (g & 1) == 0); }
         else { if constexpr (!(W4_ABL & 128)) load_piece(jst, stg_ko, stg_vo, IC<g / 2>{}, (g & 1) == 0); }
+      }
+      if constexpr (DEFER && DG > 0 && (STG & 3) == 0) {
+        constexpr int i = (DG - 1) * 8 + n / 2;
+        if constexpr ((n & 1) == 0) {
+          int dl = lane;
+          asm volatile("" : "+v"(dl));
+          dl = dl < 60 ? dl : dl - 60;
+          const int dr = (dl * 2185) >> 15;
+          def_t = *reinterpret_cast<const u32x4*>(smem + ATT_LDS_W4 + (wave * 64 + i * 4) * W4_DROW + dr * W4_DROW + (dl - dr * 15) * 16);
+        }
+        else if (__builtin_expect_with_probability(have_def, 1, 1.0))
+          *reinterpret_cast<u32x4*>(reinterpret_cast<char*>(O) + (def_vo + (uint32_t)(i * 4 * (int)ldo * 2))) = def_t;
       }
     };
     float mx = 0.f;
@@ -775,25 +794,27 @@
   };
 
   const int j_rag = (Nk & (W4_KV - 1)) ? nkv - 1 : -1;
-  auto tile = [&](int j, auto Bc, auto FIRSTc) __attribute__((always_inline)) {
+  auto tile = [&](int j, auto Bc, auto FIRSTc, auto DTc) __attribute__((always_inline)) {
     constexpr int B = decltype(Bc)::value, NB = (B + 1) % 3, WB = (B + 2) % 3;
     constexpr int FIRST = decltype(FIRSTc)::value;
+    constexpr int DT = decltype(DTc)::value;
     const bool rag = j == j_rag;
-    step(IC<0>{}, IC<!FIRST>{}, IC<FIRST>{}, IC<B * W4_KT + 32 * W4_KROW>{}, IC<B * W4_VT>{}, IC<0>{}, 0, rag, j * W4_KV);
-    step(IC<1>{}, IC<1>{}, IC<FIRST>{}, IC<0>{}, IC<0>{}, IC<1 + 4 * WB>{}, j + 3, rag, j * W4_KV);
-    step(IC<0>{}, IC<1>{}, IC<0>{}, IC<NB * W4_KT>{}, IC<B * W4_VT + 2 * 16 * 256>{}, IC<0>{}, 0, rag, j * W4_KV + 32);
-    step(IC<1>{}, IC<1>{}, IC<0>{}, IC<0>{}, IC<0>{}, IC<0>{}, 0, rag, j * W4_KV + 32);
+    step(IC<0>{}, IC<!FIRST>{}, IC<FIRST>{}, IC<B * W4_KT + 32 * W4_KROW>{}, IC<B * W4_VT>{}, IC<0>{}, 0, rag, j * W4_KV, IC<0>{});
+    step(IC<1>{}, IC<1>{}, IC<FIRST>{}, IC<0>{}, IC<0>{}, IC<1 + 4 * WB>{}, j + 3, rag, j * W4_KV, IC<0>{});
+    step(IC<0>{}, IC<1>{}, IC<0>{}, IC<NB * W4_KT>{}, IC<B * W4_VT + 2 * 16 * 256>{}, IC<0>{}, 0, rag, j * W4_KV + 32, IC<DT ? 1 : 0>{});
+    step(IC<1>{}, IC<1>{}, IC<0>{}, IC<0>{}, IC<0>{}, IC<0>{}, 0, rag, j * W4_KV + 32, IC<DT ? 2 : 0>{});
     __builtin_amdgcn_sched_barrier(0);
     asm volatile("s_waitcnt lgkmcnt(0)" ::: "memory");
     if (!(W4_ABL & 16)) __builtin_amdgcn_s_barrier();
     __builtin_amdgcn_sched_barrier(0);
   };
   W4_STAMP(1);
-  tile(0, IC<0>{}, IC<1>{});
+  tile(0, IC<0>{}, IC<1>{}, IC<1>{});
+  have_def = false;
   for (int j = 1; j < nkv; j += 3) {
-    tile(j, IC<1>{}, IC<0>{});
-    if (j + 1 < nkv) tile(j + 1, IC<2>{}, IC<0>{});
-    if (j + 2 < nkv) tile(j + 2, IC<0>{}, IC<0>{});
+    tile(j, IC<1>{}, IC<0>{}, IC<0>{});
+    if (j + 1 < nkv) tile(j + 1, IC<2>{}, IC<0>{}, IC<0>{});
+    if (j + 2 < nkv) tile(j + 2, IC<0>{}, IC<0>{}, IC<0>{});
   }
   W4_STAMP(2);
   asm volatile("s_waitcnt vmcnt(0)" ::: "memory");
@@ -833,6 +854,28 @@
       if (hi == 0) *reinterpret_cast<float2*>(pp + W4_PART_LM + (wave * 64 + qb * 32 + l31) * 2) = float2{ltot[qb], m_ref[qb]};
     }
     if (kpart >= 0) return;
+  } else if (DEFER && defer_out && has_next && (qblk + 1) * 256 <= Nq) {
+  const int orow0 = qblk * 256 + wave * 64;
+#pragma unroll
+  for (int qb = 0; qb < 2; ++qb) {
+    const float inv = 1.0f / ltot[qb];
+    char* orow = smem + ATT_LDS_W4 + (wave * 64 + qb * 32 + l31) * W4_DROW + 8 * hi;
+#pragma unroll
+    for (int db = 0; db < 4; ++db)
+#pragma unroll
+      for (int qd = 0; qd < 4; ++qd) {
+        u32x2 w;
+        w[0] = pack_bf2(o[qb][db][qd * 4 + 0] * inv, o[qb][db][qd * 4 + 1] * inv);
+        w[1] = pack_bf2(o[qb][db][qd * 4 + 2] * inv, o[qb][db][qd * 4 + 3] * inv);
+        if (db * 4 + qd < 15) *reinterpret_cast<u32x2*>(orow + db * 64 + qd * 16) = w;
+        else *reinterpret_cast<u32x2*>(Ob + (int64_t)(orow0 + qb * 32 + l31) * ldo + 120 + 4 * hi) = w;
+      }
+  }
+  {
+    const int dl = lane < 60 ? lane : lane - 60;
+    def_vo = (uint32_t)(b * o_bs + h * W4_HD) * 2u + (uint32_t)(orow0 + dl / 15) * (uint32_t)((int)ldo * 2) + (uint32_t)(dl % 15) * 16u;
+  }
+  have_def = true;
   } else {
   constexpr int OROW = 272;
   char* ot = smem + wave * (64 * OROW);
@@ -857,7 +900,7 @@
   for (int i = 0; i < 16; ++i) {
     const int c = lane + 64 * i, row = c >> 4, ch = c & 15;
     const u32x4 v = *reinterpret_cast<const u32x4*>(ot + row * OROW + ch * 16);
-    if (row0 + row < N) *reinterpret_cast<u32x4*>(Ob + (int64_t)(row0 + row) * ldo + ch * 8) = v;
+    if (row0 + row < Nq) *reinterpret_cast<u32x4*>(Ob + (int64_t)(row0 + row) * ldo + ch * 8) = v;
   }
   }
 #ifdef TFX_BENCH
@@ -880,13 +923,13 @@
   }
 }
 
-__global__ __launch_bounds__(256) void attn_w4_merge_kernel(const float* part, bf16_t* O, int64_t ldo, int64_t o_bs, int H, int N,
+__global__ __launch_bounds__(256) void attn_w4_merge_kernel(const float* part, bf16_t* O, int64_t ldo, int64_t o_bs, int H, int Nq,
                                                             int nqb, int xsplit, int nsplit) {
   const int rg = blockIdx.x * 8 + (threadIdx.x >> 5), c = (threadIdx.x & 31) * 4;
   const int ptile = rg >> 8, r = rg & 255;
   const int pair = H * nqb - xsplit + ptile % xsplit, b = ptile / xsplit, h = pair / nqb, qblk = pair % nqb;
   const int row = qblk * 256 + r;
-  if (row >= N) return;
+  if (row >= Nq) return;
   const float* pr = part + (int64_t)ptile * nsplit * (256 * W4_PROW);
   const int po = w4_part_off(r, c), lo = W4_PART_LM + r * 2;
   float m = -INFINITY;
@@ -908,7 +951,7 @@
 }
 
 __global__ __launch_bounds__(256) void attn_w4_merge_sk_kernel(const float* part, bf16_t* O, int64_t ldo, int64_t o_bs, int H, int N, int nqb,
-                                                               int group, int share, int Tp) {
+                                                               int group, int share, int Tp, int Nq) {
   __shared__ __attribute__((aligned(16))) unsigned short sm[32][128 + 8];
   const int bi = blockIdx.x >> 3, wq = blockIdx.x & 7;
   const int sample = bi / group, c = bi - sample * group;
@@ -919,7 +962,7 @@
   const int il = p / nkv, istart = il * nkv, iend = istart + nkv;
   if (w4_sk_bound(c - 1, group, share, nkv, total) > istart) return;
   const int gi = full + il, h = gi / nqb, qblk = gi - h * nqb;
-  if (qblk * 256 + wq * 32 >= N) return;
+  if (qblk * 256 + wq * 32 >= Nq) return;
   int slots[8], np = 0;
   slots[np++] = 2 * (sample * group + c - 1) + 1;
   for (int j = c; j < group && np < 8; ++j) {
@@ -962,7 +1005,7 @@
   }
   __syncthreads();
   const int orow = tid >> 3, och = tid & 7, row = qblk * 256 + wq * 32 + orow;
-  if (row < N) {
+  if (row < Nq) {
     bf16_t* dst = O + sample * o_bs + (int64_t)row * ldo + h * W4_HD + och * 16;
     *reinterpret_cast<u32x4*>(dst) = *reinterpret_cast<const u32x4*>(&sm[orow][och * 16]);
     *reinterpret_cast<u32x4*>(dst + 8) = *reinterpret_cast<const u32x4*>(&sm[orow][och * 16 + 8]);
@@ -1019,6 +1062,8 @@
 
 static int g_w4_streamk = 1;
 void set_attention_streamk(int v) { g_w4_streamk = v; }
+static int g_w4_defer = 1;
+void set_attention_deferred_output(int v) { g_w4_defer = v; }
 static int g_w4_persist = 1;
 void set_attention_persistent(int v) { g_w4_persist = v; }
 static int g_w4_grid() {
@@ -1050,8 +1095,8 @@
     if (fa.localSizeBytes != 0)
       return fail("attention: attn_w4_kernel<%d> spills %zu bytes per lane -- attention_w4.hip must be compiled with "
                   "-mllvm -amdgpu-mfma-vgpr-form", MODE, (size_t)fa.localSizeBytes);
-    if (hipFuncSetAttribute(fn, hipFuncAttributeMaxDynamicSharedMemorySize, ATT_LDS_W4 + ((W4_ABL & 256) ? 4096 : 0)) != hipSuccess)
-      return fail("attention: cannot raise dynamic LDS limit to %d bytes", ATT_LDS_W4);
+    if (hipFuncSetAttribute(fn, hipFuncAttributeMaxDynamicSharedMemorySize, W4_LDS_LAUNCH) != hipSuccess)
+      return fail("attention: cannot raise dynamic LDS limit to %d bytes", W4_LDS_LAUNCH);
     attr_set = true;
   }
   int T_items = 0;
@@ -1063,14 +1108,18 @@
     T_items = (int)grid;
     grid = (unsigned)g_w4_grid();
   }
-  attn_w4_kernel<MODE><<<grid, 256, ATT_LDS_W4 + ((W4_ABL & 256) ? 4096 : 0), st>>>((const bf16_t*)a.q, (const bf16_t*)a.k, (const bf16_t*)a.v, (bf16_t*)a.o, a.ldq,
+  const int Nq = a.Nq > 0 ? a.Nq : a.N;
+  const int defer = g_w4_defer && !(W4_ABL & 256) && T_items > 0 &&
+                    ((uint64_t)(a.B - 1) * (uint64_t)a.o_bstride + (uint64_t)Nq * (uint64_t)a.ldo) * 2 < (1ull << 32);
+  attn_w4_kernel<MODE><<<grid, 256, W4_LDS_LAUNCH, st>>>((const bf16_t*)a.q, (const bf16_t*)a.k, (const bf16_t*)a.v, (bf16_t*)a.o, a.ldq,
                                                        a.ldk, a.ldv, a.ldo, a.q_bstride, a.k_bstride, a.v_bstride, a.o_bstride, a.H,
-                                                       a.N, nqb, a.scale * 1.4426950408889634f, nfull, nparts, nsplit, xsplit, part, T_items, sk_group, sk_share);
+                                                       a.N, nqb, a.scale * 1.4426950408889634f, nfull, nparts, nsplit, xsplit, part, T_items, sk_group, sk_share, Nq, defer);
   return 0;
 }
 
 int joint_attention_w4(const AttnArgs& a, hipStream_t st, int mode) {
-  const int nqb = (a.N + 255) / 256;
+  const int Nq = a.Nq > 0 ? a.Nq : a.N;
+  const int nqb = (Nq + 255) / 256;
   const int T = a.B * a.H * nqb;
   int nfull = T, nsplit = 1, nparts = 0, xsplit = 0;
   float* part = nullptr;
@@ -1116,9 +1165,9 @@
   if (sk_share > 0) attention_note_streamk();
   if (sk_share > 0)
     attn_w4_merge_sk_kernel<<<(unsigned)(a.B * sk_group * 8), 256, 0, st>>>(part, (bf16_t*)a.o, a.ldo, a.o_bstride, a.H, a.N, nqb, sk_group,
-                                                                             sk_share, a.H * nqb);
+                                                                             sk_share, a.H * nqb, Nq);
   if (nsplit > 1)
-    attn_w4_merge_kernel<<<(unsigned)(xsplit * a.B * 32), 256, 0, st>>>(part, (bf16_t*)a.o, a.ldo, a.o_bstride, a.H, a.N, nqb,
+    attn_w4_merge_kernel<<<(unsigned)(xsplit * a.B * 32), 256, 0, st>>>(part, (bf16_t*)a.o, a.ldo, a.o_bstride, a.H, Nq, nqb,
                                                                               xsplit, nsplit);
   return 0;
 }
diff --git a/textflux_amd/csrc/capi.cpp b/textflux_amd/csrc/capi.cpp
--- a/textflux_amd/csrc/capi.cpp
+++ b/textflux_amd/csrc/capi.cpp
@@ -131,6 +131,7 @@
 
 static int g_fp8_fuse_qkn = 1;
 static int g_ln_joint = 1;
+static int g_last_block_rows = 1;
 static int g_group_streams = 1;
 
 int dit_forward(const tfx_dit_desc& d, hipStream_t st) {
@@ -169,9 +170,10 @@
     return rmsnorm_rope(y + (int64_t)row0 * D7, D7, y_bs, 2 * D, 0, H, rows, 0, B, nq, nk, nq, nk, d.cos_tab + (int64_t)row0 * 128,
                         d.sin_tab + (int64_t)row0 * 128, eps, st);
   };
-  auto attention = [&](float block_bound) -> int {
+  auto attention = [&](float block_bound, int q_row0 = 0) -> int {
     AttnArgs a;
-    a.q = y + 2 * D; a.k = y; a.v = y + D; a.o = y + 2 * D;
+    a.q = y + (int64_t)q_row0 * D7 + 2 * D; a.k = y; a.v = y + D; a.o = y + (int64_t)q_row0 * D7 + 2 * D;
+    a.Nq = N - q_row0;
     a.ldq = a.ldk = a.ldv = a.ldo = D7;
     a.q_bstride = a.k_bstride = a.v_bstride = a.o_bstride = y_bs;
     a.B = B; a.H = H; a.N = N; a.scale = att_scale; a.score_bound = block_bound > 0.f ? block_bound : d.attn_score_bound;
@@ -271,6 +273,28 @@
       const int j = blk - d.n_double;
       const tfx_single_block& w = d.sgl[j];
       const uint16_t* ms = mod + (int64_t)d.n_double * 12 * D + (int64_t)j * 3 * D;
+      if (g_last_block_rows && blk == nblk - 1 && !(d.flags & 2) && T > 0 && T % 256 == 0 && !q8 && !w.qkv_mlp.lora_a && !w.proj_out.lora_a) {
+        auto ws = [&](Gemm g) -> Gemm { return g.scratch(d.gemm_workspace, d.gemm_workspace_bytes); };
+        Gemm gi = ws(Gemm(xn_img, D, hid_bs, w.qkv_mlp, D, y_img, D7, y_bs, Sn, 7 * D, D, B).gelu(3 * D));
+        Gemm gt(xn, D, hid_bs, w.qkv_mlp, D, y, D7, y_bs, T, 2 * D, D, B);
+        Gemm go = ws(Gemm(y_img + 2 * D, D7, y_bs, w.proj_out, 5 * D, hid_img, D, hid_bs, Sn, D, 5 * D, B).gate_res(ms + 2 * D, mbs, hid_img, D, hid_bs));
+        const Gemm all_in = ws(Gemm(xn, D, hid_bs, w.qkv_mlp, D, y, D7, y_bs, N, 7 * D, D, B).gelu(3 * D));
+        const Gemm all_out = ws(Gemm(y + 2 * D, D7, y_bs, w.proj_out, 5 * D, hid, D, hid_bs, N, D, 5 * D, B).gate_res(ms + 2 * D, mbs, hid, D, hid_bs));
+        if (!gemm_k_sliced(gi.a) && !gemm_k_sliced(go.a) && !gemm_k_sliced(all_in.a) && !gemm_k_sliced(all_out.a)) {
+          TRY(ln_modulate(hid, xn, ms, ms + D, mbs, N, B, D, D, hid_bs, D, hid_bs, eps, st));
+          const bool fi = fused_here(gi, T, w.norm_q, w.norm_k);
+          if (fi) gi.qknorm(w.norm_q, w.norm_k, d.rope_cs, T, D, eps);
+          TRY(gi.run(st));
+          if (!fi) TRY(norm_rope_rows(T, Sn, w.norm_q, w.norm_k));
+          const bool ft = may_fuse && gt.qknorm_ok(w.norm_q, w.norm_k, d.rope_cs, 0, D, eps);
+          if (ft) gt.qknorm(w.norm_q, w.norm_k, d.rope_cs, 0, D, eps);
+          TRY(gt.run(st));
+          if (!ft) TRY(norm_rope_rows(0, T, w.norm_q, w.norm_k));
+          TRY(attention(w.attn_score_bound, T));
+          TRY(go.run(st));
+          continue;
+        }
+      }
       {
         Gemm gs = Gemm(xn, D, hid_bs, w.qkv_mlp, D, y, D7, y_bs, N, 7 * D, D, B).gelu(3 * D);
         const bool fs = fused_here(gs, 0, w.norm_q, w.norm_k);
@@ -709,6 +733,7 @@
   if (!std::strcmp(name, "attention_tail_split")) { set_attention_tail_split(value); return 0; }
   if (!std::strcmp(name, "attention_use_bound")) { set_attention_use_bound(value); return 0; }
   if (!std::strcmp(name, "attention_persistent")) { set_attention_persistent(value); return 0; }
+  if (!std::strcmp(name, "attention_deferred_output")) { set_attention_deferred_output(value); return 0; }
   if (!std::strcmp(name, "attention_streamk")) { set_attention_streamk(value); return 0; }
   if (!std::strcmp(name, "gemm_place")) { set_gemm_place(value); return 0; }
   if (!std::strcmp(name, "gemm_waves")) {
@@ -719,6 +744,7 @@
     return 0;
   }
   if (!std::strcmp(name, "gemm_group_streams")) { g_group_streams = value; return 0; }
+  if (!std::strcmp(name, "last_block_rows")) { g_last_block_rows = value; return 0; }
   if (!std::strcmp(name, "ln_joint")) { g_ln_joint = value; return 0; }
   if (!std::strcmp(name, "ln_prefetch")) { set_ln_prefetch(value); return 0; }
   if (!std::strcmp(name, "fp8_fuse_qkn")) { g_fp8_fuse_qkn = value; return 0; }
diff --git a/textflux_amd/csrc/gemm.hip b/textflux_amd/csrc/gemm.hip
--- a/textflux_amd/csrc/gemm.hip
+++ b/textflux_amd/csrc/gemm.hip
@@ -1643,6 +1643,16 @@
   return plan_slices(p, cus & ~7, p.K >> 6, a.workspace, a.workspace_bytes).sk == 1;
 }
 
+bool gemm_k_sliced(const GemmArgs& a) {
+  if (!fast_ok(a) || a.conv_cin > 0) return false;
+  const GemmParams p = make_params(a);
+  if (!persist_ok(p)) return false;
+  int dev = 0, cus = 256;
+  (void)hipGetDevice(&dev);
+  if (hipDeviceGetAttribute(&cus, hipDeviceAttributeMultiprocessorCount, dev) != hipSuccess || cus < 8) cus = 256;
+  return plan_slices(p, cus & ~7, p.K >> 6, a.workspace, a.workspace_bytes).sk != 1;
+}
+
 template <int EPI, bool QKN>
 static int launch_lora(const GemmParams& p, hipStream_t st) {
   static int grid = 0;
diff --git a/textflux_amd/csrc/launch.h b/textflux_amd/csrc/launch.h
--- a/textflux_amd/csrc/launch.h
+++ b/textflux_amd/csrc/launch.h
@@ -54,6 +54,7 @@
 void set_gemm_splitk(int v);
 int gemm_bf16(const GemmArgs& a, hipStream_t st);
 bool gemm_qkn_ok(const GemmArgs& a);
+bool gemm_k_sliced(const GemmArgs& a);
 bool gemm_fp8_qkn_ok(const GemmArgs& a);
 constexpr int LORA_MAX_RANK = 256;
 struct LoraArgs { const void* T; const void* Bm; int R, seg_cols, nseg; uint32_t seg_mask; int64_t t_seg = 0; };
@@ -77,6 +78,7 @@
   float score_bound = 0.f;
   void* workspace = nullptr;
   int64_t workspace_bytes = 0;
+  int Nq = 0;
 };
 int joint_attention(const AttnArgs& a, hipStream_t st);
 int joint_attention_hp(const AttnArgs& a, hipStream_t st);
@@ -94,6 +96,7 @@
 int gate_residual(const void* x, int64_t ldx, int64_t x_bs, const void* gate, int64_t gate_bs, const void* res, int64_t ldr, int64_t r_bs,
                   void* out, int64_t ldo, int64_t o_bs, int rows, int batch, int D, hipStream_t st);
 void set_attention_streamk(int v);
+void set_attention_deferred_output(int v);
 void set_attention_persistent(int v);
 void set_attention_debug(void* p);
 void set_attention_waves(int nw);
```

Measured after the change: 0.5866. About the same (-0.0%).
